# yoozzeek/zk-lisp

Measured on AMD Instinct MI355X. Metric: segment-proofs/sec at 65536 rows, blowup=16; proof bytes bit-exact vs CPU ref, higher is better.
Workload: dtype f128 (u128 mod 2^128-45*2^40+1)

## Files before the change

### zk-lisp_amd/csrc/kernels.h

```cpp
#pragma once
#include <hip/hip_runtime.h>
#include <stdint.h>

#include <stdexcept>
#include <string>
#include "air_host.h"
#include "field.h"

namespace zkl {

struct DeviceError : std::runtime_error { using std::runtime_error::runtime_error; };
#define ZKL_HIPCHECK(x)                                                                       \
  do {                                                                                        \
    hipError_t e_ = (x);                                                                      \
    if (e_ != hipSuccess) throw ::zkl::DeviceError(std::string(#x) + ": " + hipGetErrorString(e_)); \
  } while (0)
inline void check_launch(const char* what) {
  const hipError_t e = hipGetLastError();
  if (e != hipSuccess) throw DeviceError(std::string("kernel launch failed (") + what + "): " + hipGetErrorString(e));
}

struct HasherConsts {
  fe mds[144];
  fe rc[27 * 12];
  fe dom[2];
  fe dom_elems, dom_merge, dom_many, dom_int;
};

struct HasherMont {
  uint32_t mds[12][12][5];
  uint32_t rc[27][12][5];
  uint32_t dom[2][5];
  uint32_t r2[5];
  uint32_t dfe[4][5];
  uint32_t dom130[2][5];
  uint32_t r2_130[5];
  uint32_t dfe130[4][5];
  uint32_t mdsl[12][12][5][5];
  uint32_t rc130[27][12][5];
  uint32_t pmk0[5];
  uint32_t pmkt[2][5];
};
HasherMont make_hasher_mont(const HasherConsts& h);
void upload_hasher_mont(const HasherMont& m, hipStream_t s);
void upload_pm_tables(const HasherConsts& h, hipStream_t s);
int hash_engine();
void set_hash_policy(int engine, size_t min_items);
void set_row_digest_rule(int rule);
int row_digest_rule();
void set_ntt_lazy(bool on);
const char* poseidon_build_config();
const char* kernels_build_config();
void launch_permute(fe* d_states, size_t n, int engine, hipStream_t s);
struct CeParams;
struct DerivedConsts;
struct ProofConsts;
void upload_air_consts(ProofConsts* dK, const AirDevice& a, hipStream_t s);
void upload_alphas_from_device(ProofConsts* dK, const fe* d_alphas, int n, hipStream_t s);
void launch_pose_k(const ProofConsts* dK, DerivedConsts* dD, int n_tc, bool pose, hipStream_t s);
void launch_deep_coeffs(const fe* d_gam, uint32_t W, uint32_t C, const fe* d_frame, DerivedConsts* dD, hipStream_t s);

void launch_hash_rows(const fe* d_mat, uint32_t n_cols, size_t n_rows, uint32_t num_partitions,
                      uint32_t hash_rate, fe* d_tmp, fe* d_out, hipStream_t s, int tag = 0, int split = 0);
constexpr uint32_t COL_GENERAL = 0xFFFFFFFFu;
constexpr uint32_t COL_P_MAX = 128;
bool column_structure_enabled();
void set_column_structure(bool on);
void launch_scan_columns(const fe* d_mat, uint32_t n_cols, size_t n_rows, uint32_t* d_bits, hipStream_t s,
                         bool clear = true);
void decode_column_scan(const uint32_t* bits, uint32_t n_cols, size_t n_rows, uint32_t* period);
struct RowPrefixPlan {
  uint32_t np = 0;
  uint32_t lead[16] = {0};
  uint32_t q[16] = {0};
  bool any() const {
    for (uint32_t p = 0; p < np; p++)
      if (lead[p]) return true;
    return false;
  }
};
RowPrefixPlan plan_row_prefix(const uint32_t* period, uint32_t n_cols, size_t n_rows, uint32_t blowup,
                              uint32_t num_partitions, uint32_t hash_rate, size_t rows_per_entry = 64);
size_t row_prefix_table_bytes(const RowPrefixPlan& plan);
bool launch_hash_rows_prefix(const fe* d_mat, uint32_t n_cols, size_t n_rows, uint32_t num_partitions,
                             uint32_t hash_rate, const RowPrefixPlan& plan, uint32_t* d_table, fe* d_tmp, fe* d_out,
                             hipStream_t s, int split = 0);
void launch_merkle(fe* d_nodes, size_t n_leaves, hipStream_t s, fe* d_coin = nullptr, fe* d_root_out = nullptr,
                   int coin_mode = 0);
void launch_draws(fe seed, uint64_t base, size_t k, fe* d_out, hipStream_t s, const fe* d_seed = nullptr);
void launch_grind(fe seed, uint64_t base, uint32_t count, uint32_t bits, unsigned long long* d_best, hipStream_t s,
                  const fe* d_seed = nullptr);
void launch_fri_remainder(const fe* d_ev, uint32_t Nr, uint32_t rlen, const fe* wk, const fe* sk, fe* d_coin,
                          fe* d_rem, hipStream_t s);
void launch_query_seed(fe* d_coin, const unsigned long long* d_best, hipStream_t s);

struct MontTab {
  const uint4* l4;
  const uint32_t* l1;
};
void build_mont_table(const fe* h_w, size_t N, void* d_buf, hipStream_t s);
inline MontTab mont_tab(const void* d_buf, size_t N) {
  return MontTab{(const uint4*)d_buf, (const uint32_t*)((const char*)d_buf + N * 16)};
}
void launch_ntt_stages(fe* d_data, size_t n_cols, size_t N, bool dif, int lo_log, int hi_log,
                       MontTab roots, size_t Ntab, hipStream_t s);
void launch_intt_scaled(const fe* d_src, fe* d_data, size_t n_cols, size_t n, MontTab iroots, size_t Ntab,
                        const fe* d_scale, hipStream_t s);
int launch_lde_from_coeffs(const fe* d_coef, size_t n_cols, size_t n, size_t N, MontTab roots, size_t Ntab, fe* d_out,
                           hipStream_t s, bool want_split = false);
__host__ __device__ inline size_t lde_pos(size_t r, size_t N, int split) {
  if (!split) return r;
  const int logS = __builtin_ctzll((unsigned long long)N) - 8;
  const size_t S = (size_t)1 << logS;
  const size_t L = r & (S - 1), t = r >> logS, l = L & 7;
  return (L - l) + (l >> 1) + ((t & 1) << 2) + (((t >> 1) + ((l & 1) << 7)) << logS);
}
__host__ __device__ inline size_t lde_row(size_t q, size_t N, int split) {
  if (!split) return q;
  const int logS = __builtin_ctzll((unsigned long long)N) - 8;
  const size_t S = (size_t)1 << logS;
  const size_t Lp = q & (S - 1), tp = q >> logS, m = Lp & 7;
  const size_t l = ((m & 3) << 1) | (tp >> 7), t = ((tp & 127) << 1) | (m >> 2);
  return (Lp - m) + l + (t << logS);
}
void launch_broadcast(const fe* d_in, size_t in_col_stride, size_t in_elem_stride, size_t in_offset,
                      size_t n_cols, size_t n, size_t N, const fe* d_scale, fe mult, bool reverse, fe* d_out, hipStream_t s);
void launch_scale_bitrev(fe* d_data, size_t n_cols, size_t n, const fe* d_scale, hipStream_t s);

struct CeParams {
  size_t n, N, ce;
  uint32_t blowup;
  fe gl;
  fe inv_n;
  fe xn_inv[64];
  fe xn_m1[64];
  fe lagr;
  uint32_t n_bcols;
  uint32_t bcol[64];
};
struct ProofConsts {
  AirDevice air;
  CeParams ce;
  fe alpha[1024];
};
struct DerivedConsts {
  fe pose_k[27];
  fe apre[1025];
  fe deep[512];
  uint32_t deep_m[512][5];
  fe deep_sz[2];
};
void launch_constraint_eval(const fe* d_lde, const fe* d_roots, size_t Ntab, const fe* d_pertab,
                            const fe* d_bm , const CeParams& p, ProofConsts* dK,
                            const DerivedConsts* dD, bool pose_block, bool ram_merkle,
                            fe* d_xinv , bool xinv_ready, fe* d_out,
                            hipStream_t s, int split = 0, fe* d_pose_part  = nullptr);
void launch_boundary_scatter(const uint32_t* d_slot, const uint32_t* d_step, const fe* d_beta, size_t n_assert,
                             size_t n, fe* d_vecs, hipStream_t s);
void launch_boundary_w(const uint32_t* d_row_start, const fe* d_beta, const fe* d_val, size_t n, fe* d_w, hipStream_t s);
void launch_check_zero_range_bitrev(const fe* d_data, size_t N, size_t lo, size_t hi, unsigned* d_flag, hipStream_t s);

struct OodArgs {
  const fe* coef;
  size_t col_stride, elem_stride, n;
  const fe* pw1;
  const fe* pw2;
  uint32_t ncols, chunks, use_off;
  uint32_t off[16];
};
void launch_ood(const OodArgs& a, fe* d_partial, hipStream_t s);
void launch_ood_frame(const fe* d_partial_trace, const fe* d_partial_comp, uint32_t W, uint32_t C, uint32_t chunks,
                      const fe* mult , fe* d_frame, hipStream_t s);
struct DeepParams {
  size_t N;
  uint32_t W, C;
  fe z, zg;
};
void launch_deep_denoms(const fe* d_roots, size_t Ntab, size_t N, fe z, fe zg, fe* d_dinv, hipStream_t s);
void launch_deep(const fe* d_lde, const fe* d_clde, const fe* d_roots, size_t Ntab, const DeepParams& p,
                 const DerivedConsts* dD, const fe* d_dinv , fe* d_out, hipStream_t s,
                 int split = 0);
void launch_fri_leaves(const fe* d_ev, size_t Nd, fe* d_leaves, hipStream_t s);
void launch_fri_fold(const fe* d_ev, size_t Nd, const fe* d_alpha, const fe* d_iroots, size_t Ntab, fe* d_out,
                     hipStream_t s);
void launch_gather(const uint64_t* d_addrs, size_t k, fe* d_out, hipStream_t s);

}
```

### zk-lisp_amd/csrc/kernels.hip

```cpp
#include <hip/hip_runtime.h>

#include <algorithm>
#include <atomic>
#include <cstdlib>
#include <cstring>
#include <map>
#include <mutex>
#include <set>
#include <stdexcept>
#include <vector>

#include "kernels.h"
#include "air_eval.h"
#include "mont26.h"

namespace zkl {


void upload_air_consts(ProofConsts* dK, const AirDevice& a, hipStream_t s) {
  ZKL_HIPCHECK(hipMemcpyAsync(&dK->air, &a, sizeof a, hipMemcpyHostToDevice, s));
}
void upload_alphas_from_device(ProofConsts* dK, const fe* d, int n, hipStream_t s) {
  if (n > 1024) throw std::invalid_argument("more than 1024 transition constraints");
  ZKL_HIPCHECK(hipMemcpyAsync(dK->alpha, d, sizeof(fe) * n, hipMemcpyDeviceToDevice, s));
}
__global__ __launch_bounds__(1024) void pose_k_kernel(const ProofConsts* K, DerivedConsts* D, int n_tc, int pose) {
  const int j = (int)threadIdx.x;
  if (pose && j < 27) {
    uint32_t acc[9] = {0, 0, 0, 0, 0, 0, 0, 0, 0};
    for (int i = 0; i < 12; i++) mul_acc(K->alpha[12 * j + i], K->air.pose_rc[j][i], acc);
    D->pose_k[j] = reduce288(acc);
  }
  __shared__ fe sc[1024];
  sc[j] = j < n_tc ? K->alpha[j] : fe_zero();
  __syncthreads();
  for (int d = 1; d < 1024; d <<= 1) {
    const fe add = j >= d ? sc[j - d] : fe_zero();
    __syncthreads();
    sc[j] = fe_add(sc[j], add);
    __syncthreads();
  }
  D->apre[j + 1] = sc[j];
  if (j == 0) D->apre[0] = fe_zero();
}
void launch_pose_k(const ProofConsts* dK, DerivedConsts* dD, int n_tc, bool pose, hipStream_t s) {
  if (n_tc < 0 || n_tc > 1024) throw std::invalid_argument("launch_pose_k: more than 1024 transition constraints");
  pose_k_kernel<<<1, 1024, 0, s>>>(dK, dD, n_tc, pose ? 1 : 0);
}

#ifndef NTT_ELEMS_CFG
#define NTT_ELEMS_CFG 1024
#endif
#ifndef NTT_THREADS_CFG
#define NTT_THREADS_CFG 256
#endif
constexpr int NTT_ELEMS = NTT_ELEMS_CFG;
constexpr int NTT_THREADS = NTT_THREADS_CFG;

__device__ __forceinline__ uint32_t bitrev(uint32_t x, int logn) { return logn ? (__brev(x) >> (32 - logn)) : 0; }

__host__ __device__ __forceinline__ fe mul_tw(fe a, MontTab t, size_t e) {
  const uint4 q = t.l4[e];
  const uint32_t wm[5] = {q.x, q.y, q.z, q.w, t.l1[e]};
  uint32_t l[5], o[5];
  to26(a, l);
  mont_mul(l, wm, o);
  typedef unsigned __int128 u128;
  const u128 v = (u128)o[0] + ((u128)o[1] << 26) + ((u128)o[2] << 52) + ((u128)o[3] << 78) + ((u128)o[4] << 104);
  const u128 P = ((u128)P_HI << 64) | P_LO;
  const u128 r = (o[4] >> 24) ? v + C_RED : (v >= P ? v - P : v);
#ifdef NTT_CHECK
  {
    uint64_t cc[10] = {wm[0], wm[1], wm[2], wm[3], wm[4], 0, 0, 0, 0, 0};
    uint32_t wl[5];
    redc(cc, wl);
    u128 wv = (u128)wl[0] + ((u128)wl[1] << 26) + ((u128)wl[2] << 52) + ((u128)wl[3] << 78) + ((u128)wl[4] << 104);
    if (wv >= P) wv -= P;
    fe want = fe_mul(a, fe{(uint64_t)wv, (uint64_t)(wv >> 64)});
    if (want.lo != (uint64_t)r || want.hi != (uint64_t)(r >> 64))
      printf("mul_tw mismatch e=%lu a=%016lx%016lx got=%016lx%016lx want=%016lx%016lx o=%x %x %x %x %x\n", (unsigned long)e,
             (unsigned long)a.hi, (unsigned long)a.lo, (unsigned long)(uint64_t)(r >> 64), (unsigned long)(uint64_t)r,
             (unsigned long)want.hi, (unsigned long)want.lo, o[0], o[1], o[2], o[3], o[4]);
  }
#endif
  return fe{(uint64_t)r, (uint64_t)(r >> 64)};
}

void build_mont_table(const fe* w, size_t N, void* d_buf, hipStream_t s) {
  const fe R = fe_pow64(fe{2, 0}, 156);
  std::vector<uint32_t> l4(4 * N, 0), l1(N, 0);
  for (size_t H = 1; H < N; H *= 2) {
    const size_t step = N / (2 * H);
    for (size_t j = 0; j < H; j++) {
      uint32_t l[5];
      limbs26(fe_mul(w[j * step], R), l);
      for (int t = 0; t < 4; t++) l4[4 * (H + j) + t] = l[t];
      l1[H + j] = l[4];
    }
  }
  ZKL_HIPCHECK(hipMemcpyAsync(d_buf, l4.data(), N * 16, hipMemcpyHostToDevice, s));
  ZKL_HIPCHECK(hipMemcpyAsync((char*)d_buf + N * 16, l1.data(), N * 4, hipMemcpyHostToDevice, s));
  ZKL_HIPCHECK(hipStreamSynchronize(s));
}

template <bool DIF>
__global__ __launch_bounds__(NTT_THREADS) void ntt_pass_kernel(fe* __restrict__ data, size_t ncols, int logN, int r,
                                                       int logS, MontTab roots, int logTab, const fe* __restrict__ src,
                                                       int src_logb, const fe* __restrict__ scale = nullptr) {
  __shared__ fe buf[NTT_ELEMS + NTT_ELEMS / 16];
  const int R = 1 << r;
  const int G = NTT_ELEMS >> r;
  const size_t S = (size_t)1 << logS;
  const int log_gpc = logN - r;
  const size_t gpc = (size_t)1 << log_gpc;
  const bool gfast = S >= (size_t)G;
  const int pitch = R >= 16 ? R + 1 : R;
  size_t col_fixed = 0, qbase = 0;
  const bool whole = gpc >= (size_t)G;
  if (whole) {
    col_fixed = blockIdx.x % (unsigned)ncols;
    qbase = (size_t)(blockIdx.x / (unsigned)ncols) * G;
  }
  auto locate = [&](int g, size_t& col, size_t& q) -> bool {
    if (whole) {
      col = col_fixed;
      q = qbase + g;
      return true;
    }
    const size_t qg = (size_t)blockIdx.x * G + g;
    col = qg >> log_gpc;
    q = qg & (gpc - 1);
    return col < ncols;
  };
  auto addr = [&](int g, int t, bool& ok) -> size_t {
    size_t col, q;
    ok = locate(g, col, q);
    const size_t L = q & (S - 1), Hb = q >> logS;
    return (col << logN) + ((Hb << logS) << r) + (size_t)t * S + L;
  };
  const size_t Nmask = ((size_t)1 << logN) - 1;
  for (int e = threadIdx.x; e < NTT_ELEMS; e += NTT_THREADS) {
    int g = gfast ? (e % G) : (e >> r);
    int t = gfast ? (e / G) : (e & (R - 1));
    bool ok;
    size_t a = addr(g, t, ok);
    fe v = fe_zero();
    if (ok) v = src ? src[((a >> logN) << (logN - src_logb)) + ((a & Nmask) >> src_logb)] : data[a];
    buf[g * pitch + t] = v;
  }
  __syncthreads();
  for (int st = 0; st < r; st++) {
    const int lh = DIF ? (r - 1 - st) : st;
    const int h = 1 << lh;
    const size_t Hs = (size_t)h << logS;
    constexpr int BPT = NTT_ELEMS / 2 / NTT_THREADS;
    fe x0[BPT], x1[BPT];
    size_t te[BPT];
    int o0[BPT];
#pragma unroll
    for (int i = 0; i < BPT; i++) {
      const int u = threadIdx.x + NTT_THREADS * i;
      const int g = u % G;
      const int w = u / G;
      const int k = w & (h - 1);
      const int t0 = ((w >> lh) << (lh + 1)) + k;
      size_t colx, q;
      locate(g, colx, q);
      const size_t L = q & (S - 1);
      te[i] = Hs + ((size_t)k << logS) + L;
      o0[i] = g * pitch + t0;
      x0[i] = buf[o0[i]];
      x1[i] = buf[o0[i] + h];
    }
#pragma unroll
    for (int i = 0; i < BPT; i++) {
      if (DIF) {
        buf[o0[i]] = fe_add(x0[i], x1[i]);
        buf[o0[i] + h] = mul_tw(fe_sub(x0[i], x1[i]), roots, te[i]);
      } else {
        const fe v = mul_tw(x1[i], roots, te[i]);
        buf[o0[i]] = fe_add(x0[i], v);
        buf[o0[i] + h] = fe_sub(x0[i], v);
      }
    }
    __syncthreads();
  }
  for (int e = threadIdx.x; e < NTT_ELEMS; e += NTT_THREADS) {
    int g = gfast ? (e % G) : (e >> r);
    int t = gfast ? (e / G) : (e & (R - 1));
    bool ok;
    size_t a = addr(g, t, ok);
    if (ok) data[a] = scale ? fe_mul(buf[g * pitch + t], scale[bitrev((uint32_t)(a & Nmask), logN)]) : buf[g * pitch + t];
  }
}

constexpr uint32_t NTT_Q[5] = {67108872u, 128319487u, 134217726u, 134217726u, 134217726u};

__device__ __forceinline__ fe ntt_canon(const uint32_t l[5]) {
  typedef unsigned __int128 u128;
  const u128 lo = (u128)l[0] + ((u128)l[1] << 26) + ((u128)l[2] << 52) + ((u128)l[3] << 78);
  const u128 v = lo + ((u128)(l[4] & 0xFFFFFFu) << 104);
  const uint32_t t = (l[4] >> 24) + (v < lo ? 1u : 0u);
  const u128 P = ((u128)P_HI << 64) | P_LO;
  u128 r = v + (u128)t * C_RED;
  if (r < v) r += C_RED;
  if (r >= P) r -= P;
  return fe{(uint64_t)r, (uint64_t)(r >> 64)};
}

template <int ELEMS, int THREADS>
__global__ __launch_bounds__(THREADS) void ntt_dit_lazy_kernel(fe* __restrict__ data, size_t ncols, int logN, int r,
                                                                  int logS, MontTab roots, const fe* __restrict__ src,
                                                                  int src_logb) {
  constexpr int PITCHED = ELEMS + ELEMS / 16;
  __shared__ uint4 bufA[PITCHED];
  __shared__ uint32_t bufB[PITCHED];
  const int R = 1 << r;
  const int G = ELEMS >> r;
  const size_t S = (size_t)1 << logS;
  const int log_gpc = logN - r;
  const size_t gpc = (size_t)1 << log_gpc;
  const bool gfast = S >= (size_t)G;
  const int pitch = R >= 16 ? R + 1 : R;
  size_t col_fixed = 0, qbase = 0;
  const bool whole = gpc >= (size_t)G;
  if (whole) {
    col_fixed = blockIdx.x % (unsigned)ncols;
    qbase = (size_t)(blockIdx.x / (unsigned)ncols) * G;
  }
  auto locate = [&](int g, size_t& col, size_t& q) -> bool {
    if (whole) {
      col = col_fixed;
      q = qbase + g;
      return true;
    }
    const size_t qg = (size_t)blockIdx.x * G + g;
    col = qg >> log_gpc;
    q = qg & (gpc - 1);
    return col < ncols;
  };
  auto addr = [&](int g, int t, bool& ok) -> size_t {
    size_t col, q;
    ok = locate(g, col, q);
    const size_t L = q & (S - 1), Hb = q >> logS;
    return (col << logN) + ((Hb << logS) << r) + (size_t)t * S + L;
  };
  const size_t Nmask = ((size_t)1 << logN) - 1;
  for (int e = threadIdx.x; e < ELEMS; e += THREADS) {
    const int g = gfast ? (e % G) : (e >> r);
    const int t = gfast ? (e / G) : (e & (R - 1));
    bool ok;
    const size_t a = addr(g, t, ok);
    fe v = fe_zero();
    if (ok) v = src ? src[((a >> logN) << (logN - src_logb)) + ((a & Nmask) >> src_logb)] : data[a];
    uint32_t l[5];
    to26(v, l);
    bufA[g * pitch + t] = make_uint4(l[0], l[1], l[2], l[3]);
    bufB[g * pitch + t] = l[4];
  }
  __syncthreads();
  auto ld = [&](int o, uint32_t x[5]) {
    const uint4 a = bufA[o];
    x[0] = a.x; x[1] = a.y; x[2] = a.z; x[3] = a.w; x[4] = bufB[o];
  };
  auto st = [&](int o, const uint32_t x[5]) {
    bufA[o] = make_uint4(x[0], x[1], x[2], x[3]);
    bufB[o] = x[4];
  };
  auto tw = [&](size_t e, uint32_t wm[5]) {
    const uint4 q4 = roots.l4[e];
    wm[0] = q4.x; wm[1] = q4.y; wm[2] = q4.z; wm[3] = q4.w; wm[4] = roots.l1[e];
  };
  auto bfly = [&](uint32_t x0[5], uint32_t x1[5], const uint32_t wm[5]) {
    uint32_t v[5];
    mont_mul(x1, wm, v);
#pragma unroll
    for (int l = 0; l < 5; l++) {
      x1[l] = x0[l] + NTT_Q[l] - v[l];
      x0[l] = x0[l] + v[l];
    }
  };
  int lh = 0;
  for (; lh + 1 < r; lh += 2) {
    const int h = 1 << lh;
    constexpr int QPT = ELEMS / 4 / THREADS;
#pragma unroll
    for (int i = 0; i < QPT; i++) {
      const int u = threadIdx.x + THREADS * i;
      const int g = u % G;
      const int w = u / G;
      const int k = w & (h - 1);
      const int t0 = ((w >> lh) << (lh + 2)) + k;
      size_t colx, q;
      locate(g, colx, q);
      const size_t L = q & (S - 1);
      const int o = g * pitch + t0;
      uint32_t a0[5], a1[5], a2[5], a3[5], w1[5], w2[5], w3[5];
      ld(o, a0); ld(o + h, a1); ld(o + 2 * h, a2); ld(o + 3 * h, a3);
      tw(((size_t)h << logS) + ((size_t)k << logS) + L, w1);
      tw(((size_t)(2 * h) << logS) + ((size_t)k << logS) + L, w2);
      tw(((size_t)(2 * h) << logS) + ((size_t)(k + h) << logS) + L, w3);
      bfly(a0, a1, w1);
      bfly(a2, a3, w1);
      bfly(a0, a2, w2);
      bfly(a1, a3, w3);
      st(o, a0); st(o + h, a1); st(o + 2 * h, a2); st(o + 3 * h, a3);
    }
    __syncthreads();
  }
  if (lh < r) {
    const int h = 1 << lh;
    constexpr int BPT = ELEMS / 2 / THREADS;
#pragma unroll
    for (int i = 0; i < BPT; i++) {
      const int u = threadIdx.x + THREADS * i;
      const int g = u % G;
      const int w = u / G;
      const int k = w & (h - 1);
      const int t0 = ((w >> lh) << (lh + 1)) + k;
      size_t colx, q;
      locate(g, colx, q);
      const int o = g * pitch + t0;
      uint32_t x0[5], x1[5], wm[5];
      ld(o, x0); ld(o + h, x1);
      tw(((size_t)h << logS) + ((size_t)k << logS) + (q & (S - 1)), wm);
      bfly(x0, x1, wm);
      st(o, x0); st(o + h, x1);
    }
    __syncthreads();
  }
  for (int e = threadIdx.x; e < ELEMS; e += THREADS) {
    const int g = gfast ? (e % G) : (e >> r);
    const int t = gfast ? (e / G) : (e & (R - 1));
    bool ok;
    const size_t a = addr(g, t, ok);
    const uint4 a4 = bufA[g * pitch + t];
    const uint32_t l[5] = {a4.x, a4.y, a4.z, a4.w, bufB[g * pitch + t]};
    if (ok) data[a] = ntt_canon(l);
  }
}

template <int ELEMS, int THREADS>
__global__ __launch_bounds__(THREADS) void ntt_ct_lazy_kernel(fe* __restrict__ data, size_t ncols, int logN, int r,
                                                                 int logS, MontTab roots, const fe* __restrict__ src,
                                                                 int src_logb, const fe* __restrict__ scale) {
  constexpr int PITCHED = ELEMS + ELEMS / 16;
  __shared__ uint4 bufA[PITCHED];
  __shared__ uint32_t bufB[PITCHED];
  const int R = 1 << r;
  const int G = ELEMS >> r;
  const size_t S = (size_t)1 << logS;
  const int log_gpc = logN - r;
  const size_t gpc = (size_t)1 << log_gpc;
  const bool gfast = S >= (size_t)G;
  const int pitch = R >= 16 ? R + 1 : R;
  size_t col_fixed = 0, qbase = 0;
  const bool whole = gpc >= (size_t)G;
  if (whole) {
    col_fixed = blockIdx.x % (unsigned)ncols;
    qbase = (size_t)(blockIdx.x / (unsigned)ncols) * G;
  }
  auto locate = [&](int g, size_t& col, size_t& q) -> bool {
    if (whole) {
      col = col_fixed;
      q = qbase + g;
      return true;
    }
    const size_t qg = (size_t)blockIdx.x * G + g;
    col = qg >> log_gpc;
    q = qg & (gpc - 1);
    return col < ncols;
  };
  auto addr = [&](int g, int t, bool& ok) -> size_t {
    size_t col, q;
    ok = locate(g, col, q);
    const size_t L = q & (S - 1), Hb = q >> logS;
    return (col << logN) + ((Hb << logS) << r) + (size_t)t * S + L;
  };
  const size_t Nmask = ((size_t)1 << logN) - 1;
  for (int e = threadIdx.x; e < ELEMS; e += THREADS) {
    const int g = gfast ? (e % G) : (e >> r);
    const int t = gfast ? (e / G) : (e & (R - 1));
    bool ok;
    const size_t a = addr(g, t, ok);
    fe v = fe_zero();
    if (ok) v = src ? src[((a >> logN) << (logN - src_logb)) + ((a & Nmask) >> src_logb)] : data[a];
    uint32_t l[5];
    to26(v, l);
    bufA[g * pitch + t] = make_uint4(l[0], l[1], l[2], l[3]);
    bufB[g * pitch + t] = l[4];
  }
  __syncthreads();
  auto ld = [&](int o, uint32_t x[5]) {
    const uint4 a = bufA[o];
    x[0] = a.x; x[1] = a.y; x[2] = a.z; x[3] = a.w; x[4] = bufB[o];
  };
  auto st = [&](int o, const uint32_t x[5]) {
    bufA[o] = make_uint4(x[0], x[1], x[2], x[3]);
    bufB[o] = x[4];
  };
  auto tw = [&](int lh, size_t q, int t0, uint32_t wm[5]) {
    const int logm = logN - 1 - lh - logS;
    const size_t b = (q >> logS) * ((size_t)R >> (lh + 1)) + (size_t)(t0 >> (lh + 1));
    const size_t e = ((size_t)1 << logm) + (logm ? (size_t)(__brevll((unsigned long long)b) >> (64 - logm)) : 0);
    const uint4 q4 = roots.l4[e];
    wm[0] = q4.x; wm[1] = q4.y; wm[2] = q4.z; wm[3] = q4.w; wm[4] = roots.l1[e];
  };
  auto bfly = [&](uint32_t x0[5], uint32_t x1[5], const uint32_t wm[5]) {
    uint32_t v[5];
    mont_mul(x1, wm, v);
#pragma unroll
    for (int l = 0; l < 5; l++) {
      x1[l] = x0[l] + NTT_Q[l] - v[l];
      x0[l] = x0[l] + v[l];
    }
  };
  int lh = r - 1;
  for (; lh >= 1; lh -= 2) {
    const int hl = 1 << (lh - 1);
    constexpr int QPT = ELEMS / 4 / THREADS;
#pragma unroll
    for (int i = 0; i < QPT; i++) {
      const int u = threadIdx.x + THREADS * i;
      const int g = u % G;
      const int w = u / G;
      const int k = w & (hl - 1);
      const int t0 = ((w >> (lh - 1)) << (lh + 1)) + k;
      size_t colx, q;
      locate(g, colx, q);
      const int o = g * pitch + t0;
      uint32_t a0[5], a1[5], a2[5], a3[5], w1[5], w2[5], w3[5];
      ld(o, a0); ld(o + hl, a1); ld(o + 2 * hl, a2); ld(o + 3 * hl, a3);
      tw(lh, q, t0, w1);
      tw(lh - 1, q, t0, w2);
      tw(lh - 1, q, t0 + 2 * hl, w3);
      bfly(a0, a2, w1);
      bfly(a1, a3, w1);
      bfly(a0, a1, w2);
      bfly(a2, a3, w3);
      st(o, a0); st(o + hl, a1); st(o + 2 * hl, a2); st(o + 3 * hl, a3);
    }
    __syncthreads();
  }
  if (lh == 0) {
    constexpr int BPT = ELEMS / 2 / THREADS;
#pragma unroll
    for (int i = 0; i < BPT; i++) {
      const int u = threadIdx.x + THREADS * i;
      const int g = u % G;
      const int t0 = (u / G) << 1;
      size_t colx, q;
      locate(g, colx, q);
      const int o = g * pitch + t0;
      uint32_t x0[5], x1[5], wm[5];
      ld(o, x0); ld(o + 1, x1);
      tw(0, q, t0, wm);
      bfly(x0, x1, wm);
      st(o, x0); st(o + 1, x1);
    }
    __syncthreads();
  }
  for (int e = threadIdx.x; e < ELEMS; e += THREADS) {
    const int g = gfast ? (e % G) : (e >> r);
    const int t = gfast ? (e / G) : (e & (R - 1));
    bool ok;
    const size_t a = addr(g, t, ok);
    const uint4 a4 = bufA[g * pitch + t];
    const uint32_t l[5] = {a4.x, a4.y, a4.z, a4.w, bufB[g * pitch + t]};
    if (ok) {
      const fe v = ntt_canon(l);
      data[a] = scale ? fe_mul(v, scale[bitrev((uint32_t)(a & Nmask), logN)]) : v;
    }
  }
}

constexpr int NTT8_G = 8;
constexpr int NTT8_THREADS = 256;
constexpr int NTT8_PITCH = 257;
__global__ __launch_bounds__(NTT8_THREADS) __global__ __launch_bounds__(NTT8_THREADS) void ntt_dit8_kernel(fe* __restrict__ data, size_t ncols, int logN, int logS,
                                                                 MontTab roots, const fe* __restrict__ src, int src_logb,
                                                                 int lfast, int split) {
  __shared__ uint4 bufA[NTT8_G * NTT8_PITCH];
  __shared__ uint32_t bufB[NTT8_G * NTT8_PITCH];
  const int tid = (int)threadIdx.x;
  const int g = tid & (NTT8_G - 1), j = tid >> 3;
  size_t col, q;
  if (lfast) {
    const unsigned gpb = (1u << (logN - 8)) / NTT8_G;
    col = blockIdx.x / gpb;
    q = (size_t)(blockIdx.x % gpb) * NTT8_G + g;
  } else {
    col = blockIdx.x % (unsigned)ncols;
    q = (size_t)(blockIdx.x / (unsigned)ncols) * NTT8_G + g;
  }
  const size_t S = (size_t)1 << logS;
  const size_t L = q & (S - 1), Hb = q >> logS;
  const size_t base = (col << logN) + ((Hb << logS) << 8) + L;
  auto tw = [&](size_t h, size_t k, uint32_t wm[5]) {
    const size_t e = ((h + k) << logS) + L;
    const uint4 q4 = roots.l4[e];
    wm[0] = q4.x; wm[1] = q4.y; wm[2] = q4.z; wm[3] = q4.w; wm[4] = roots.l1[e];
  };
  auto bfly = [&](uint32_t x0[5], uint32_t x1[5], const uint32_t wm[5]) {
    uint32_t v[5];
    mont_mul(x1, wm, v);
#pragma unroll
    for (int l = 0; l < 5; l++) {
      x1[l] = x0[l] + NTT_Q[l] - v[l];
      x0[l] = x0[l] + v[l];
    }
  };
  auto lds_st = [&](int t, const uint32_t x[5]) {
    bufA[g * NTT8_PITCH + t] = make_uint4(x[0], x[1], x[2], x[3]);
    bufB[g * NTT8_PITCH + t] = x[4];
  };
  auto lds_ld = [&](int t, uint32_t x[5]) {
    const uint4 a = bufA[g * NTT8_PITCH + t];
    x[0] = a.x; x[1] = a.y; x[2] = a.z; x[3] = a.w; x[4] = bufB[g * NTT8_PITCH + t];
  };
  uint32_t x[8][5];
  uint32_t w[7][5];
  tw(1, 0, w[0]);
  tw(2, 0, w[1]); tw(2, 1, w[2]);
#pragma unroll
  for (int k = 0; k < 4; k++) tw(4, k, w[3 + k]);
  {
    const size_t Nmask = ((size_t)1 << logN) - 1;
#pragma unroll
    for (int u = 0; u < 8; u++) {
      const size_t a = base + (size_t)(8 * j + u) * S;
      const fe v = src ? src[((a >> logN) << (logN - src_logb)) + ((a & Nmask) >> src_logb)] : data[a];
      to26(v, x[u]);
    }
  }
#pragma unroll
  for (int u = 0; u < 8; u += 2) bfly(x[u], x[u + 1], w[0]);
#pragma unroll
  for (int u = 0; u < 8; u += 4) { bfly(x[u], x[u + 2], w[1]); bfly(x[u + 1], x[u + 3], w[2]); }
#pragma unroll
  for (int k = 0; k < 4; k++) bfly(x[k], x[k + 4], w[3 + k]);
#pragma unroll
  for (int u = 0; u < 8; u++) lds_st(8 * j + u, x[u]);
  const int a = j & 7, c = j >> 3;
  tw(8, a, w[0]);
  tw(16, a, w[1]); tw(16, a + 8, w[2]);
#pragma unroll
  for (int k = 0; k < 4; k++) tw(32, a + 8 * k, w[3 + k]);
  __syncthreads();
#pragma unroll
  for (int u = 0; u < 8; u++) lds_ld(a + 8 * u + 64 * c, x[u]);
#pragma unroll
  for (int u = 0; u < 8; u += 2) bfly(x[u], x[u + 1], w[0]);
#pragma unroll
  for (int u = 0; u < 8; u += 4) { bfly(x[u], x[u + 2], w[1]); bfly(x[u + 1], x[u + 3], w[2]); }
#pragma unroll
  for (int k = 0; k < 4; k++) bfly(x[k], x[k + 4], w[3 + k]);
#pragma unroll
  for (int u = 0; u < 8; u++) lds_st(a + 8 * u + 64 * c, x[u]);
  tw(64, j, w[0]); tw(128, j, w[1]); tw(128, j + 64, w[2]);
  tw(64, j + 32, w[3]); tw(128, j + 32, w[4]); tw(128, j + 96, w[5]);
  __syncthreads();
#pragma unroll
  for (int qd = 0; qd < 2; qd++) {
    const int a2 = j + 32 * qd;
#pragma unroll
    for (int u = 0; u < 4; u++) lds_ld(a2 + 64 * u, x[4 * qd + u]);
    uint32_t* y0 = x[4 * qd];
    uint32_t* y1 = x[4 * qd + 1];
    uint32_t* y2 = x[4 * qd + 2];
    uint32_t* y3 = x[4 * qd + 3];
    bfly(y0, y1, w[3 * qd]);
    bfly(y2, y3, w[3 * qd]);
    bfly(y0, y2, w[3 * qd + 1]);
    bfly(y1, y3, w[3 * qd + 2]);
    const size_t at0 = split ? (col << logN) + (L - g) + (g >> 1) + 4 * (a2 & 1) +
                                   ((size_t)((a2 >> 1) + ((g & 1) << 7)) << logS)
                             : base + (size_t)a2 * S;
    const size_t du = split ? 32 * S : 64 * S;
#pragma unroll
    for (int u = 0; u < 4; u++) data[at0 + u * du] = ntt_canon(x[4 * qd + u]);
  }
}

static std::atomic<int> g_ntt_lazy{-1};
static bool ntt_lazy_enabled() {
  int v = g_ntt_lazy.load(std::memory_order_relaxed);
  if (v < 0) {
    const char* e = getenv("ZKL_NTT");
    v = (e && !strcmp(e, "classic")) ? 0 : 1;
    g_ntt_lazy.store(v);
  }
  return v != 0;
}
void set_ntt_lazy(bool on) { g_ntt_lazy.store(on ? 1 : 0); }
static int ntt_wide_mode() {
  static const int m = [] {
    const char* e = getenv("ZKL_NTT_WIDE");
    return e ? atoi(e) : 2;
  }();
  return m;
}

static bool ntt8_enabled() {
  static const bool on = [] {
    const char* e = getenv("ZKL_NTT8");
    return !(e && !strcmp(e, "0"));
  }();
  return on;
}

static int ntt8_lfast(int logS) {
  static const int m = [] {
    const char* e = getenv("ZKL_NTT8_MAP");
    return e ? atoi(e) : 0;
  }();
  return m == 1 || (m == 2 && logS >= 11) ? 1 : 0;
}

static bool ntt_ct_enabled() {
  static const bool on = [] {
    const char* e = getenv("ZKL_NTT_CT");
    return !(e && !strcmp(e, "0"));
  }();
  return on;
}

static int ilog2s(size_t n) { int k = 0; while (((size_t)1 << k) < n) k++; return k; }

#ifndef NTT_TOP_R
#define NTT_TOP_R 6
#endif
#ifndef NTT_SPLIT_MODE
#define NTT_SPLIT_MODE 0
#endif
static std::vector<int> ntt_split(int K) {
  std::vector<int> rs;
  if (K <= 0) return rs;
  if (NTT_SPLIT_MODE == 0) {
    for (int left = K; left > 0; left -= std::min(8, left)) rs.push_back(std::min(8, left));
    return rs;
  }
  if (K <= 10) { rs.push_back(K); return rs; }
  int rest = K - NTT_TOP_R;
  const int np = (rest + 9) / 10;
  for (int i = 0; i < np; i++) {
    int r = (rest + (np - i) - 1) / (np - i);
    if ((r & 1) && r < rest && r < 10) r++;
    rs.push_back(r);
    rest -= r;
  }
  rs.push_back(NTT_TOP_R);
  return rs;
}

static bool dit_split_ok(size_t N, int lo, int hi) {
  if (hi < lo || !ntt_lazy_enabled() || !ntt8_enabled()) return false;
  const std::vector<int> rs = ntt_split(hi - lo + 1);
  int cur = lo;
  for (size_t k = 0; k + 1 < rs.size(); k++) cur += rs[k];
  return rs.back() == 8 && ((size_t)1 << cur) >= (size_t)NTT8_G && (N >> 8) >= (size_t)NTT8_G;
}

static void ntt_passes(fe* d, size_t ncols, size_t N, bool dif, int lo, int hi, MontTab roots, size_t Ntab,
                       const fe* src, int src_logb, hipStream_t s, int split = 0, const fe* scale = nullptr) {
  int logN = ilog2s(N), logTab = ilog2s(Ntab);
  if (hi < lo) return;
  const std::vector<int> rs = ntt_split(hi - lo + 1);
  if (dif) {
    int cur = hi;
    for (size_t k = rs.size(); k-- > 0;) {
      const int r = rs[k];
      int logS = cur - r + 1;
      size_t groups = (N >> r) * ncols;
      size_t G = NTT_ELEMS >> r;
      const fe* sp = k + 1 == rs.size() ? src : nullptr;
      const fe* sc = k == 0 ? scale : nullptr;
      if (ntt_lazy_enabled() && ntt_ct_enabled()) {
        const int wm = ntt_wide_mode();
        const bool wide = wm > 0 && G < 8 && ((size_t)1 << logS) >= G;
        const size_t Gw = wide ? 2 * G : G;
        const unsigned grid = (unsigned)((groups + Gw - 1) / Gw);
        if (wide && wm == 2)
          ntt_ct_lazy_kernel<2 * NTT_ELEMS, 2 * NTT_THREADS><<<grid, 2 * NTT_THREADS, 0, s>>>(d, ncols, logN, r, logS, roots, sp, 0, sc);
        else if (wide)
          ntt_ct_lazy_kernel<2 * NTT_ELEMS, NTT_THREADS><<<grid, NTT_THREADS, 0, s>>>(d, ncols, logN, r, logS, roots, sp, 0, sc);
        else
          ntt_ct_lazy_kernel<NTT_ELEMS, NTT_THREADS><<<grid, NTT_THREADS, 0, s>>>(d, ncols, logN, r, logS, roots, sp, 0, sc);
      } else {
        ntt_pass_kernel<true><<<(unsigned)((groups + G - 1) / G), NTT_THREADS, 0, s>>>(d, ncols, logN, r, logS, roots,
                                                                                      logTab, sp, 0, sc);
      }
      cur -= r;
    }
  } else {
    int cur = lo;
    for (size_t ri = 0; ri < rs.size(); ri++) {
      const int r = rs[ri];
      const int split_here = split && ri + 1 == rs.size();
      size_t groups = (N >> r) * ncols;
      size_t G = NTT_ELEMS >> r;
      if (ntt_lazy_enabled()) {
        const int wm = ntt_wide_mode();
        const bool wide = wm > 0 && G < 8 && ((size_t)1 << cur) >= G;
        const size_t Gw = wide ? 2 * G : G;
        const unsigned grid = (unsigned)((groups + Gw - 1) / Gw);
        const fe* sp = cur == lo ? src : nullptr;
        if (r == 8 && ntt8_enabled() && ((size_t)1 << cur) >= (size_t)NTT8_G && (N >> 8) >= (size_t)NTT8_G)
          ntt_dit8_kernel<<<(unsigned)(groups / NTT8_G), NTT8_THREADS, 0, s>>>(d, ncols, logN, cur, roots, sp, src_logb,
                                                                              ntt8_lfast(cur), split_here);
        else if (wide && wm == 2)
          ntt_dit_lazy_kernel<2 * NTT_ELEMS, 2 * NTT_THREADS><<<grid, 2 * NTT_THREADS, 0, s>>>(d, ncols, logN, r, cur, roots, sp, src_logb);
        else if (wide)
          ntt_dit_lazy_kernel<2 * NTT_ELEMS, NTT_THREADS><<<grid, NTT_THREADS, 0, s>>>(d, ncols, logN, r, cur, roots, sp, src_logb);
        else
          ntt_dit_lazy_kernel<NTT_ELEMS, NTT_THREADS><<<grid, NTT_THREADS, 0, s>>>(d, ncols, logN, r, cur, roots, sp, src_logb);
      } else
        ntt_pass_kernel<false><<<(unsigned)((groups + G - 1) / G), NTT_THREADS, 0, s>>>(
            d, ncols, logN, r, cur, roots, logTab, cur == lo ? src : nullptr, src_logb);
      cur += r;
    }
  }
}

void launch_ntt_stages(fe* d, size_t ncols, size_t N, bool dif, int lo, int hi, MontTab roots, size_t Ntab,
                       hipStream_t s) {
  ntt_passes(d, ncols, N, dif, lo, hi, roots, Ntab, nullptr, 0, s);
}

void launch_intt_scaled(const fe* src, fe* d, size_t ncols, size_t n, MontTab iroots, size_t Ntab, const fe* scale,
                        hipStream_t s) {
  const int logn = ilog2s(n);
  if (logn == 0) throw std::invalid_argument("launch_intt_scaled: n must be at least 2");
  ntt_passes(d, ncols, n, true, 0, logn - 1, iroots, Ntab, src, 0, s, 0, scale);
}

int launch_lde_from_coeffs(const fe* d_coef, size_t ncols, size_t n, size_t N, MontTab roots, size_t Ntab, fe* d_out,
                           hipStream_t s, bool want_split) {
  const int logB = ilog2s(N / n);
  if (logB == 0) {
    ZKL_HIPCHECK(hipMemcpyAsync(d_out, d_coef, ncols * n * sizeof(fe), hipMemcpyDeviceToDevice, s));
    ntt_passes(d_out, ncols, N, false, 0, ilog2s(N) - 1, roots, Ntab, nullptr, 0, s);
    return 0;
  }
  const int split = want_split && dit_split_ok(N, logB, ilog2s(N) - 1) ? 1 : 0;
  ntt_passes(d_out, ncols, N, false, logB, ilog2s(N) - 1, roots, Ntab, d_coef, logB, s, split);
  return split;
}

__global__ void broadcast_kernel(const fe* __restrict__ in, size_t in_col_stride, size_t in_elem_stride,
                                 size_t in_offset, size_t ncols, size_t n, int logn, int logB, const fe* __restrict__ scale,
                                 fe mult, bool reverse, fe* __restrict__ out) {
  size_t N = n << logB;
  size_t i = (size_t)blockIdx.x * blockDim.x + threadIdx.x;
  if (i >= N * ncols) return;
  size_t col = i / N, pos = i % N;
  size_t j = pos >> logB;
  size_t src = reverse ? (n - 1 - j) : j;
  fe v = in[col * in_col_stride + in_offset + src * in_elem_stride];
  if (scale) v = fe_mul(v, scale[bitrev((uint32_t)j, logn)]);
  if (!(mult.lo == 1 && mult.hi == 0)) v = fe_mul(v, mult);
  out[i] = v;
}

void launch_broadcast(const fe* d_in, size_t in_col_stride, size_t in_elem_stride, size_t in_offset, size_t ncols,
                      size_t n, size_t N, const fe* d_scale, fe mult, bool reverse, fe* d_out, hipStream_t s) {
  size_t tot = N * ncols;
  broadcast_kernel<<<(unsigned)((tot + 255) / 256), 256, 0, s>>>(d_in, in_col_stride, in_elem_stride, in_offset, ncols,
                                                                 n, ilog2s(n), ilog2s(N / n), d_scale, mult, reverse, d_out);
}

__global__ void scale_bitrev_kernel(fe* d, size_t ncols, size_t n, int logn, const fe* scale) {
  size_t i = (size_t)blockIdx.x * blockDim.x + threadIdx.x;
  if (i >= n * ncols) return;
  d[i] = fe_mul(d[i], scale[bitrev((uint32_t)(i % n), logn)]);
}
void launch_scale_bitrev(fe* d, size_t ncols, size_t n, const fe* scale, hipStream_t s) {
  scale_bitrev_kernel<<<(unsigned)((n * ncols + 255) / 256), 256, 0, s>>>(d, ncols, n, ilog2s(n), scale);
}

constexpr int SCAN_THREADS = 256;
constexpr size_t SCAN_CHUNK = 4096;
constexpr uint32_t SCAN_GENERAL = 1u << 31, SCAN_NONZERO = 1u << 8;
static_assert(SCAN_THREADS % COL_P_MAX == 0 && SCAN_CHUNK % SCAN_THREADS == 0 && COL_P_MAX <= 128, "scan shape");

__global__ __launch_bounds__(SCAN_THREADS) void scan_columns_kernel(const fe* __restrict__ M, size_t n, uint32_t R,
                                                                   uint32_t* __restrict__ bits) {
  const fe* col = M + (size_t)blockIdx.y * n;
  const size_t chunk = n < SCAN_CHUNK ? n : SCAN_CHUNK, i0 = (size_t)blockIdx.x * chunk;
  const uint32_t t = threadIdx.x;
  const fe ref = col[t & (R - 1)];
  uint32_t w = 0;
  for (size_t i = t; i < chunk; i += SCAN_THREADS) {
    const fe v = col[i0 + i];
    if (v.lo != ref.lo || v.hi != ref.hi) w = SCAN_GENERAL;
  }
  if (blockIdx.x == 0 && t < R) {
    if (ref.lo | ref.hi) w |= SCAN_NONZERO;
    for (uint32_t k = 0; (1u << k) < R; k++)
      if (t >= (1u << k)) {
        const fe v = col[t - (1u << k)];
        if (v.lo != ref.lo || v.hi != ref.hi) w |= 1u << k;
      }
  }
  if (__any(w != 0)) {
    for (int o = 32; o > 0; o >>= 1) w |= (uint32_t)__shfl_xor((int)w, o);
    if ((t & 63) == 0) atomicOr(&bits[blockIdx.y], w);
  }
}

void launch_scan_columns(const fe* d_mat, uint32_t ncols, size_t n, uint32_t* d_bits, hipStream_t s, bool clear) {
  if (n == 0 || (n & (n - 1)) || ncols == 0 || ncols > 65535)
    throw std::invalid_argument("launch_scan_columns: rows must be a power of two, 1..65535 columns");
  if (clear) ZKL_HIPCHECK(hipMemsetAsync(d_bits, 0, (size_t)ncols * sizeof(uint32_t), s));
  const uint32_t R = (uint32_t)std::min<size_t>(COL_P_MAX, n);
  const size_t chunk = std::min(n, SCAN_CHUNK);
  scan_columns_kernel<<<dim3((unsigned)(n / chunk), ncols), SCAN_THREADS, 0, s>>>(d_mat, n, R, d_bits);
}

void decode_column_scan(const uint32_t* bits, uint32_t ncols, size_t n, uint32_t* period) {
  const uint32_t R = (uint32_t)std::min<size_t>(COL_P_MAX, n);
  for (uint32_t c = 0; c < ncols; c++) {
    const uint32_t w = bits[c];
    uint32_t P = COL_GENERAL;
    if (!(w & SCAN_GENERAL)) {
      if (!(w & SCAN_NONZERO)) P = 0;
      else {
        P = R;
        for (uint32_t k = 0; (1u << k) < R; k++)
          if (!(w & (1u << k))) { P = 1u << k; break; }
      }
    }
    period[c] = P;
  }
}



#ifndef CE_WAVES_CFG
#define CE_WAVES_CFG 3
#endif
#if CE_WAVES_CFG
#define CE_OCC __attribute__((amdgpu_waves_per_eu(CE_WAVES_CFG, CE_WAVES_CFG)))
#else
#define CE_OCC
#endif
template <bool POSE, bool RM, int PART = 0>
__device__ __forceinline__ void constraint_eval_body(const fe* __restrict__ lde, const fe* __restrict__ roots,
                                                     int roots_shift, const fe* __restrict__ pertab,
                                                     const fe* __restrict__ bm, const ProofConsts* __restrict__ K,
                                                     const DerivedConsts* __restrict__ D, const fe* __restrict__ xinv,
                                                     fe* __restrict__ out, int split,
                                                     const fe* __restrict__ pose_part = nullptr) {
  const AirDevice& c_air = K->air;
  const CeParams& c_ce = K->ce;
  const size_t ce = c_ce.ce, N = c_ce.N;
  const size_t k = (size_t)blockIdx.x * blockDim.x + threadIdx.x;
  if (k >= ce) return;
  const bool by_pos = split && N <= 2 * ce;
  const size_t i = by_pos ? lde_row(k, N, 1) / (N / ce) : k;
  const size_t r0 = by_pos ? k : lde_pos(i * (N / ce), N, split);
  const size_t r1 = lde_pos((i * (N / ce) + c_ce.blowup) & (N - 1), N, split);
  auto cur = [&](int c) { return lde[(size_t)c * N + r0]; };
  auto nxt = [&](int c) { return lde[(size_t)c * N + r1]; };
  fe x = fe_mul(fe{3, 0}, roots[i << roots_shift]);
  const size_t per_period = ce / (c_ce.n / 32);
  const fe* per = pertab + (i % per_period) * 31;
  if (PART == 1) {
    out[i] = air_transition_sum<POSE, RM, 1>(c_air, cur, nxt, per, fe_zero(), K->alpha, D->pose_k, D->apre);
    return;
  }
  const size_t blow = ce / c_ce.n;
  const fe xn_inv = c_ce.xn_inv[i % blow];
  fe x_gl = fe_sub_sel(x, c_ce.gl);
  fe xn_m1 = c_ce.xn_m1[i % blow];
  fe p_last = fe_mul(fe_mul(c_ce.lagr, xn_m1), xinv[i]);
  fe tsum = air_transition_sum<POSE, RM, PART>(c_air, cur, nxt, per, p_last, K->alpha, D->pose_k, D->apre);
  if (PART == 2) tsum = fe_add(tsum, pose_part[i]);
  uint32_t bacc[9] = {0, 0, 0, 0, 0, 0, 0, 0, 0};
  const uint32_t nb = c_ce.n_bcols;
  for (uint32_t u = 0; u < nb; u++) mul_acc(cur((int)c_ce.bcol[u]), bm[(size_t)u * ce + i], bacc);
  fe bsum2 = fe_sub_sel(reduce288(bacc), bm[(size_t)nb * ce + i]);
  fe v = fe_add_sel(fe_mul(tsum, x_gl), bsum2);
  out[i] = fe_mul(v, xn_inv);
}

#ifndef CE_POSE_WAVES_CFG
#define CE_POSE_WAVES_CFG 3
#endif
#if CE_POSE_WAVES_CFG
#define CE_POSE_OCC __attribute__((amdgpu_waves_per_eu(CE_POSE_WAVES_CFG, CE_POSE_WAVES_CFG)))
#else
#define CE_POSE_OCC
#endif
template <bool RM>
__global__ __launch_bounds__(256) CE_OCC void constraint_eval_kernel(const fe* __restrict__ lde, const fe* __restrict__ roots,
                                                                    int roots_shift, const fe* __restrict__ pertab,
                                                                    const fe* __restrict__ bm,
                                                                    const ProofConsts* __restrict__ K,
                                                                    const DerivedConsts* __restrict__ D,
                                                                    const fe* __restrict__ xinv, fe* __restrict__ out,
                                                                    int split) {
  constraint_eval_body<false, RM>(lde, roots, roots_shift, pertab, bm, K, D, xinv, out, split);
}
__global__ __launch_bounds__(256) CE_POSE_OCC void constraint_eval_pose_part_kernel(
    const fe* __restrict__ lde, const fe* __restrict__ roots, int roots_shift, const fe* __restrict__ pertab,
    const fe* __restrict__ bm, const ProofConsts* __restrict__ K, const DerivedConsts* __restrict__ D,
    const fe* __restrict__ xinv, fe* __restrict__ pose_part, int split) {
  constraint_eval_body<true, false, 1>(lde, roots, roots_shift, pertab, bm, K, D, xinv, pose_part, split);
}
template <bool RM>
__global__ __launch_bounds__(256) CE_OCC void constraint_eval_pose_kernel(const fe* __restrict__ lde, const fe* __restrict__ roots,
                                                                  int roots_shift, const fe* __restrict__ pertab,
                                                                  const fe* __restrict__ bm,
                                                                  const ProofConsts* __restrict__ K,
                                                                  const DerivedConsts* __restrict__ D,
                                                                  const fe* __restrict__ xinv, fe* __restrict__ out,
                                                                  int split, const fe* __restrict__ pose_part) {
  constraint_eval_body<true, RM, 2>(lde, roots, roots_shift, pertab, bm, K, D, xinv, out, split, pose_part);
}

constexpr int INV_PTS = 16;
__device__ inline fe coset_den(const fe* __restrict__ roots, size_t i, int shift, fe a1, fe a2, int two) {
  const fe x = fe_mul(fe{3, 0}, roots[i << shift]);
  fe d = fe_sub(x, a1);
  if (two) d = fe_mul(d, fe_sub(x, a2));
  return d;
}
__global__ __launch_bounds__(256) void coset_inv_kernel(const fe* __restrict__ roots, int shift, fe a1, fe a2, int two,
                                                        fe* __restrict__ out) {
  const size_t T = (size_t)gridDim.x * blockDim.x;
  const size_t i0 = (size_t)blockIdx.x * blockDim.x + threadIdx.x;
  fe pre = coset_den(roots, i0, shift, a1, a2, two);
  for (int k = 1; k < INV_PTS; k++) {
    out[i0 + k * T] = pre;
    pre = fe_mul(pre, coset_den(roots, i0 + k * T, shift, a1, a2, two));
  }
  fe inv = fe_inv(pre);
  for (int k = INV_PTS - 1; k > 0; k--) {
    const fe p = out[i0 + k * T];
    out[i0 + k * T] = fe_mul(inv, p);
    inv = fe_mul(inv, coset_den(roots, i0 + k * T, shift, a1, a2, two));
  }
  out[i0] = inv;
}
static void launch_coset_inv(const fe* d_roots, int shift, size_t M, fe a1, fe a2, int two, fe* d_out, hipStream_t s) {
  const size_t threads = std::min<size_t>(256, M / INV_PTS);
  coset_inv_kernel<<<(unsigned)(M / (threads * INV_PTS)), (unsigned)threads, 0, s>>>(d_roots, shift, a1, a2, two, d_out);
}

void launch_constraint_eval(const fe* d_lde, const fe* d_roots, size_t Ntab, const fe* d_pertab, const fe* d_bm,
                            const CeParams& p, ProofConsts* dK, const DerivedConsts* dD, bool pose_block,
                            bool ram_merkle, fe* d_xinv,
                            bool xinv_ready, fe* d_out, hipStream_t s, int split, fe* d_pose_part) {
  ZKL_HIPCHECK(hipMemcpyAsync(&dK->ce, &p, sizeof p, hipMemcpyHostToDevice, s));
  int shift = ilog2s(Ntab) - ilog2s(p.ce);
  if (!xinv_ready) launch_coset_inv(d_roots, shift, p.ce, p.gl, fe_zero(), 0, d_xinv, s);
  const unsigned grid = (unsigned)((p.ce + 255) / 256);
  if (pose_block) {
    if (!d_pose_part) throw std::invalid_argument("constraint evaluation: Poseidon layout needs the pose_part buffer");
    constraint_eval_pose_part_kernel<<<grid, 256, 0, s>>>(d_lde, d_roots, shift, d_pertab, d_bm, dK, dD, d_xinv,
                                                           d_pose_part, split);
  }
  if (pose_block && ram_merkle)
    constraint_eval_pose_kernel<true><<<grid, 256, 0, s>>>(d_lde, d_roots, shift, d_pertab, d_bm, dK, dD, d_xinv, d_out,
                                                           split, d_pose_part);
  else if (pose_block)
    constraint_eval_pose_kernel<false><<<grid, 256, 0, s>>>(d_lde, d_roots, shift, d_pertab, d_bm, dK, dD, d_xinv, d_out,
                                                            split, d_pose_part);
  else if (ram_merkle)
    constraint_eval_kernel<true><<<grid, 256, 0, s>>>(d_lde, d_roots, shift, d_pertab, d_bm, dK, dD, d_xinv, d_out, split);
  else
    constraint_eval_kernel<false><<<grid, 256, 0, s>>>(d_lde, d_roots, shift, d_pertab, d_bm, dK, dD, d_xinv, d_out, split);
}

__global__ void boundary_scatter_kernel(const uint32_t* slot, const uint32_t* step, const fe* beta, size_t na, size_t n,
                                        fe* vecs) {
  size_t a = (size_t)blockIdx.x * blockDim.x + threadIdx.x;
  if (a >= na) return;
  vecs[(size_t)slot[a] * n + step[a]] = beta[a];
}
void launch_boundary_scatter(const uint32_t* d_slot, const uint32_t* d_step, const fe* d_beta, size_t na, size_t n,
                             fe* d_vecs, hipStream_t s) {
  boundary_scatter_kernel<<<(unsigned)((na + 255) / 256), 256, 0, s>>>(d_slot, d_step, d_beta, na, n, d_vecs);
}
__global__ void boundary_w_kernel(const uint32_t* rs, const fe* beta, const fe* val, size_t n, fe* w) {
  size_t row = (size_t)blockIdx.x * blockDim.x + threadIdx.x;
  if (row >= n) return;
  uint32_t acc[9] = {0, 0, 0, 0, 0, 0, 0, 0, 0};
  for (uint32_t a = rs[row]; a < rs[row + 1]; a++) mul_acc(beta[a], val[a], acc);
  w[row] = reduce288(acc);
}
void launch_boundary_w(const uint32_t* d_rs, const fe* d_beta, const fe* d_val, size_t n, fe* d_w, hipStream_t s) {
  boundary_w_kernel<<<(unsigned)((n + 255) / 256), 256, 0, s>>>(d_rs, d_beta, d_val, n, d_w);
}

__global__ void check_zero_kernel(const fe* d, size_t N, int logN, size_t lo, size_t hi, unsigned* flag) {
  size_t k = lo + (size_t)blockIdx.x * blockDim.x + threadIdx.x;
  if (k >= hi) return;
  fe v = d[bitrev((uint32_t)k, logN)];
  if (!fe_is_zero(v)) atomicOr(flag, 1u);
}
void launch_check_zero_range_bitrev(const fe* d, size_t N, size_t lo, size_t hi, unsigned* flag, hipStream_t s) {
  if (hi > lo) check_zero_kernel<<<(unsigned)((hi - lo + 255) / 256), 256, 0, s>>>(d, N, ilog2s(N), lo, hi, flag);
}

__global__ __launch_bounds__(256) void ood_kernel(OodArgs A, fe* partial) {
  const uint32_t c = blockIdx.x, k = blockIdx.z;
  const fe* col = A.coef + (A.use_off ? (size_t)A.off[c] : (size_t)c * A.col_stride);
  const size_t len = A.n / A.chunks, j0 = (size_t)k * len;
  uint32_t acc1[9] = {0, 0, 0, 0, 0, 0, 0, 0, 0}, acc2[9] = {0, 0, 0, 0, 0, 0, 0, 0, 0};
  for (size_t j = j0 + threadIdx.x; j < j0 + len; j += 256) {
    const fe v = col[j * A.elem_stride];
    mul_acc(v, A.pw1[j], acc1);
    mul_acc(v, A.pw2[j], acc2);
  }
  __shared__ fe red[2][256];
  red[0][threadIdx.x] = reduce288(acc1);
  red[1][threadIdx.x] = reduce288(acc2);
  __syncthreads();
  for (int w = 128; w > 0; w >>= 1) {
    if ((int)threadIdx.x < w) {
      red[0][threadIdx.x] = fe_add(red[0][threadIdx.x], red[0][threadIdx.x + w]);
      red[1][threadIdx.x] = fe_add(red[1][threadIdx.x], red[1][threadIdx.x + w]);
    }
    __syncthreads();
  }
  if (threadIdx.x < 2) partial[((size_t)threadIdx.x * A.ncols + c) * A.chunks + k] = red[threadIdx.x][0];
}
void launch_ood(const OodArgs& A, fe* d_partial, hipStream_t s) {
  ood_kernel<<<dim3(A.ncols, 1, A.chunks), 256, 0, s>>>(A, d_partial);
}

#ifndef DEEP_PTS_CFG
#define DEEP_PTS_CFG 2
#endif
#ifndef DEEP_COLS_CFG
#define DEEP_COLS_CFG 4
#endif
constexpr int DEEP_PTS = DEEP_PTS_CFG, DEEP_COLS = DEEP_COLS_CFG;

__device__ __forceinline__ fe limbs_canon(const uint32_t l[5]) {
  typedef unsigned __int128 u128;
  const u128 v = (u128)l[0] | ((u128)l[1] << 26) | ((u128)l[2] << 52) | ((u128)l[3] << 78) | ((u128)(l[4] & 0xFFFFFFu) << 104);
  const u128 P = ((u128)P_HI << 64) | P_LO;
  u128 r = v + (u128)(l[4] >> 24) * C_RED;
  if (r < v) r += C_RED;
  if (r >= P) r -= P;
  return fe{(uint64_t)r, (uint64_t)(r >> 64)};
}

__global__ __launch_bounds__(256) void deep_kernel(const fe* __restrict__ lde, const fe* __restrict__ clde,
                                                   const fe* __restrict__ roots, int shift, DeepParams p,
                                                   const DerivedConsts* __restrict__ K, const fe* __restrict__ dinv,
                                                   fe* out, int split) {
  const size_t T = (size_t)gridDim.x * blockDim.x;
  const size_t i0 = (size_t)blockIdx.x * blockDim.x + threadIdx.x;
  uint64_t col[DEEP_PTS][10];
#pragma unroll
  for (int k = 0; k < DEEP_PTS; k++)
#pragma unroll
    for (int u = 0; u < 10; u++) col[k][u] = 0;
  const uint32_t ncol = p.W + p.C;
  for (uint32_t c0 = 0; c0 < ncol; c0 += DEEP_COLS) {
    fe v[DEEP_COLS][DEEP_PTS];
#pragma unroll
    for (int cc = 0; cc < DEEP_COLS; cc++) {
      const uint32_t c = c0 + cc;
      const bool tr = c < p.W;
      const fe* src = tr ? lde + (size_t)c * p.N : clde + (size_t)(c - p.W) * p.N;
#pragma unroll
      for (int k = 0; k < DEEP_PTS; k++)
        v[cc][k] = c < ncol ? src[tr ? i0 + k * T : lde_row(i0 + k * T, p.N, split)] : fe_zero();
    }
#pragma unroll
    for (int cc = 0; cc < DEEP_COLS; cc++) {
      const uint32_t c = min(c0 + cc, ncol - 1);
      const uint32_t* g = K->deep_m[c];
      const uint32_t gm[5] = {g[0], g[1], g[2], g[3], g[4]};
#pragma unroll
      for (int k = 0; k < DEEP_PTS; k++) {
        uint32_t l[5];
        to26(v[cc][k], l);
        mac5(l, gm, col[k]);
      }
    }
  }
#pragma unroll
  for (int k = 0; k < DEEP_PTS; k++) {
    uint32_t l[5];
    redc(col[k], l);
    const fe sv = limbs_canon(l);
    const size_t i = lde_row(i0 + k * T, p.N, split);
    const fe x = fe_mul(fe{3, 0}, roots[i << shift]);
    const fe d1 = fe_sub(x, p.z), d2 = fe_sub(x, p.zg);
    const fe num = fe_add(fe_mul(fe_sub(sv, K->deep_sz[0]), d2), fe_mul(fe_sub(sv, K->deep_sz[1]), d1));
    out[i] = fe_mul(num, dinv[i]);
  }
}
__global__ __launch_bounds__(256) void deep_coeffs_kernel(const fe* __restrict__ gam, uint32_t W, uint32_t C,
                                                          const fe* __restrict__ frame, fe R156, DerivedConsts* K) {
  __shared__ fe red[2][256];
  const uint32_t i = threadIdx.x, n = W + C;
  fe a = fe_zero(), b = fe_zero();
  if (i < n) {
    const fe g = gam[i];
    K->deep[i] = g;
    uint32_t l[5];
    to26(fe_mul(g, R156), l);
#pragma unroll
    for (int t = 0; t < 5; t++) K->deep_m[i][t] = l[t];
    a = fe_mul(g, frame[i]);
    b = fe_mul(g, frame[n + i]);
  }
  red[0][i] = a;
  red[1][i] = b;
  __syncthreads();
  for (uint32_t h = 128; h > 0; h >>= 1) {
    if (i < h) {
      red[0][i] = fe_add(red[0][i], red[0][i + h]);
      red[1][i] = fe_add(red[1][i], red[1][i + h]);
    }
    __syncthreads();
  }
  if (i == 0) {
    K->deep_sz[0] = red[0][0];
    K->deep_sz[1] = red[1][0];
  }
}
void launch_deep_coeffs(const fe* d_gam, uint32_t W, uint32_t C, const fe* d_frame, DerivedConsts* dK, hipStream_t s) {
  if (W + C > 256) throw std::invalid_argument("more than 256 DEEP coefficients (W + C)");
  deep_coeffs_kernel<<<1, 256, 0, s>>>(d_gam, W, C, d_frame, fe_pow64(fe{2, 0}, 156), dK);
}

struct OodMult {
  fe m[16];
};
__global__ void ood_frame_kernel(const fe* __restrict__ pt, const fe* __restrict__ pc, uint32_t W, uint32_t C,
                                 uint32_t chunks, OodMult mult, fe* __restrict__ frame) {
  const uint32_t o = blockIdx.x * blockDim.x + threadIdx.x;
  const uint32_t n = W + C;
  if (o >= 2 * n) return;
  const uint32_t pt_ = o / n, r = o % n;
  const bool tr = r < W;
  const fe* src = tr ? pt + ((size_t)pt_ * W + r) * chunks : pc + ((size_t)pt_ * C + (r - W)) * chunks;
  fe acc = fe_zero();
  for (uint32_t k = 0; k < chunks; k++) acc = fe_add(acc, src[k]);
  frame[o] = tr ? acc : fe_mul(acc, mult.m[r - W]);
}
void launch_ood_frame(const fe* d_pt, const fe* d_pc, uint32_t W, uint32_t C, uint32_t chunks, const fe* mult,
                      fe* d_frame, hipStream_t s) {
  if (C > 16) throw std::invalid_argument("more than 16 composition columns");
  OodMult m{};
  for (uint32_t j = 0; j < C; j++) m.m[j] = mult[j];
  const uint32_t outs = 2 * (W + C);
  ood_frame_kernel<<<(outs + 127) / 128, 128, 0, s>>>(d_pt, d_pc, W, C, chunks, m, d_frame);
}

void launch_deep_denoms(const fe* d_roots, size_t Ntab, size_t N, fe z, fe zg, fe* d_dinv, hipStream_t s) {
  launch_coset_inv(d_roots, ilog2s(Ntab) - ilog2s(N), N, z, zg, 1, d_dinv, s);
}

void launch_deep(const fe* d_lde, const fe* d_clde, const fe* d_roots, size_t Ntab, const DeepParams& p,
                 const DerivedConsts* dK, const fe* d_dinv, fe* d_out, hipStream_t s, int split) {
  const size_t threads = std::min<size_t>(256, p.N / DEEP_PTS);
  deep_kernel<<<(unsigned)(p.N / (threads * DEEP_PTS)), (unsigned)threads, 0, s>>>(
      d_lde, d_clde, d_roots, ilog2s(Ntab) - ilog2s(p.N), p, dK, d_dinv, d_out, split);
}

__global__ void fri_fold_kernel(const fe* ev, size_t half, const fe* alpha_p, const fe* iroots, int shift, fe inv3,
                                fe inv2, fe* out) {
  size_t i = (size_t)blockIdx.x * blockDim.x + threadIdx.x;
  if (i >= half) return;
  const fe alpha = *alpha_p;
  fe v0 = ev[i], v1 = ev[i + half];
  fe ix = fe_mul(inv3, iroots[i << shift]);
  out[i] = fe_mul(fe_add(fe_add(v0, v1), fe_mul(alpha, fe_mul(fe_sub(v0, v1), ix))), inv2);
}
void launch_fri_fold(const fe* d_ev, size_t Nd, const fe* d_alpha, const fe* d_iroots, size_t Ntab, fe* d_out,
                     hipStream_t s) {
  size_t h = Nd / 2;
  fe inv3 = fe_inv(fe{3, 0}), inv2 = fe_inv(fe{2, 0});
  fri_fold_kernel<<<(unsigned)((h + 255) / 256), 256, 0, s>>>(d_ev, h, d_alpha, d_iroots, ilog2s(Ntab) - ilog2s(Nd),
                                                               inv3, inv2, d_out);
}

__global__ void gather_kernel(const uint64_t* addrs, size_t k, fe* out) {
  size_t i = (size_t)blockIdx.x * blockDim.x + threadIdx.x;
  if (i >= k) return;
  out[i] = *reinterpret_cast<const fe*>(addrs[i]);
}
void launch_gather(const uint64_t* d_addrs, size_t k, fe* d_out, hipStream_t s) {
  if (k) gather_kernel<<<(unsigned)((k + 255) / 256), 256, 0, s>>>(d_addrs, k, d_out);
}

}

#define ZKL_STR2(x) #x
#define ZKL_STR(x) ZKL_STR2(x)
namespace zkl {
const char* kernels_build_config() {
  return "NTT_ELEMS=" ZKL_STR(NTT_ELEMS_CFG) ";NTT_THREADS=" ZKL_STR(NTT_THREADS_CFG) ";CE_WAVES=" ZKL_STR(
      CE_WAVES_CFG) ";CE_POSE_WAVES=" ZKL_STR(CE_POSE_WAVES_CFG) ";DEEP_PTS=" ZKL_STR(DEEP_PTS_CFG) ";DEEP_COLS=" ZKL_STR(
      DEEP_COLS_CFG) ";CE_GROUPS=" ZKL_STR(CE_GROUPS_CFG) ";CE_DOT=" ZKL_STR(CE_DOT_CFG) ";CE_BRANCHFREE=" ZKL_STR(
      CE_BRANCHFREE_CFG);
}
}
```

### zk-lisp_amd/csrc/prover.cpp

```cpp
#include <hip/hip_runtime.h>
#include <malloc.h>
#include <stdio.h>
#include <string.h>

#include <atomic>
#include <algorithm>
#include <chrono>
#include <functional>
#include <map>
#include <memory>
#include <mutex>
#include <set>
#include <thread>
#include <stdexcept>
#include <string>
#include <vector>

#include "../../include/zkl_hip.h"
#include "air_host.h"
#include "host_hash.h"
#include "kernels.h"
#include "host_proof.h"
#include "proof_view.h"

using namespace zkl;

namespace zkl {
std::vector<uint8_t> step_encode(const zkl_air_public_inputs& pi, const zkl_step_info& s, const uint8_t* inner,
                                 size_t inner_len);
void step_digest(const uint8_t* p, size_t n, uint8_t digest[32], uint8_t rt[32]);
void children_root(const uint8_t suite[32], const uint8_t* digests, const uint8_t* roots, size_t n, uint8_t out[32]);
}

namespace {

#define HIPCHECK(x) ZKL_HIPCHECK(x)

struct InvalidArg : std::runtime_error { using std::runtime_error::runtime_error; };

uint32_t bitrev_u(uint32_t x, int logn) { uint32_t r = 0; for (int i = 0; i < logn; i++) r |= ((x >> i) & 1u) << (logn - 1 - i); return r; }

struct DBuf {
  void* p = nullptr;
  size_t bytes = 0;
  void ensure(size_t b) {
    if (b <= bytes) return;
    if (p) (void)hipFree(p);
    p = nullptr;
    bytes = 0;
    HIPCHECK(hipMalloc(&p, b));
    bytes = b;
  }
  fe* f() const { return (fe*)p; }
  ~DBuf() { if (p) (void)hipFree(p); }
};

std::atomic<uint64_t> g_pin_cur{0}, g_pin_peak{0};
void pin_alloc(void** p, size_t b) {
  HIPCHECK(hipHostMalloc(p, b, hipHostMallocDefault));
  const uint64_t c = g_pin_cur.fetch_add(b) + b;
  uint64_t pk = g_pin_peak.load();
  while (c > pk && !g_pin_peak.compare_exchange_weak(pk, c)) {
  }
}
hipError_t pin_free(void* p, size_t b) {
  if (!p) return hipSuccess;
  g_pin_cur.fetch_sub(b);
  return hipHostFree(p);
}

struct HBuf {
  void* p = nullptr;
  size_t bytes = 0;
  void ensure(size_t b) {
    if (b <= bytes) return;
    (void)release();
    b += b / 4;
    pin_alloc(&p, b);
    bytes = b;
  }
  hipError_t release() {
    const hipError_t e = pin_free(p, bytes);
    p = nullptr;
    bytes = 0;
    return e;
  }
  template <class T>
  T* at(size_t off = 0) const { return (T*)((char*)p + off); }
  ~HBuf() { (void)release(); }
};

}

constexpr size_t TX_CS = 48, TX_CS_MAX = 32, TX_QD = 80, TX_QD_MAX = 256, TX_FRI_SEED = 336, TX_WORDS = 344;

struct zkl_ctx {
  int device = 0;
  hipStream_t stream = nullptr;
  std::mutex mu;
  std::string err;
  double stage_ms[ZKL_NUM_STAGES] = {0};
  double host_ms[3] = {0, 0, 0};
  size_t tab_n = 0, tab_N = 0;
  DBuf roots, iroots, mroots, miroots, opow, opow_n, pertab;
  DBuf trace, coef, lde, parts, tree, ce, bvec, bm, clde, ctree, deep, draws, pw, oodv, oodf, txs, asl, ast, asv, ars;
  DBuf lcoef;
  DBuf fri_ev, fri_tree, best, gaddr, gout, flag;
  DBuf xinv;
  DBuf posep;
  DBuf cexinv;
  size_t cexinv_key_n = 0, cexinv_key_ce = 0, cexinv_key_tab = 0;
  const void* cexinv_key_roots = nullptr;
  DBuf scanbits, pfxtab;
  HBuf h_scan;
  std::vector<uint8_t> zero_known;
  struct { const void* coef = nullptr; const void* lde = nullptr; size_t n = 0, N = 0, W = 0; } zero_key;
  DBuf kconst;
  DBuf dconst;
  DBuf fri_coin;
  HBuf h_asrt, h_ood, h_addr, h_gv, h_tx, h_air;
  hipStream_t aux = nullptr;
  hipEvent_t aux_ev = nullptr, hev = nullptr;
  hipStream_t up = nullptr;
  std::vector<void*> up_slot;
  std::vector<hipEvent_t> up_ev;
  size_t up_slot_bytes = 0;
  double up_ms = 0;
  hipEvent_t stage_ev[ZKL_NUM_STAGES + 1] = {};
  bool stage_ev_ready = false;
  size_t pert_key_n = 0, pert_key_ce = 0;
  std::vector<hipEvent_t> evpool;
  std::vector<std::pair<int, size_t>> kmarks;
  size_t evnext = 0;
  int ktiming = 1;
  double kfam_ms[ZKL_NUM_KFAMILIES] = {0};
  int kfam_n[ZKL_NUM_KFAMILIES] = {0};
  std::vector<uint8_t> proof_s;
  Plan tplan_s;
  std::vector<Plan> fplan_s;
  std::vector<std::vector<size_t>> fpos_s;
  AirInstance air;
  HBuf tbuf[ZKL_TRACE_BUFFERS];
};

static const char* kFamilyNames =
    "ntt\ntrace_hash_rows\nmerkle\nconstraint_eval\ncomp_hash_rows\ndeep\nfri\ngrind\nmisc";
enum { KF_NTT = 0, KF_TRACE_HASH, KF_MERKLE, KF_CEVAL, KF_COMP_HASH, KF_DEEP, KF_FRI, KF_GRIND, KF_MISC };

namespace {

struct KScope {
  zkl_ctx* C;
  size_t i;
  KScope(zkl_ctx* c, int fam) : C(c), i(SIZE_MAX) {
    if (!(C->ktiming == 2 || (C->ktiming == 1 && fam == KF_TRACE_HASH))) return;
    if (C->evnext + 2 > C->evpool.size()) {
      size_t old = C->evpool.size();
      C->evpool.resize(old + 256);
      for (size_t k = old; k < C->evpool.size(); k++) HIPCHECK(hipEventCreate(&C->evpool[k]));
    }
    i = C->evnext;
    C->evnext += 2;
    C->kmarks.push_back({fam, i});
    HIPCHECK(hipEventRecord(C->evpool[i], C->stream));
  }
  ~KScope() {
    if (i != SIZE_MAX) (void)hipEventRecord(C->evpool[i + 1], C->stream);
  }
};

void resolve_kernel_times(zkl_ctx* C) {
  for (int f = 0; f < ZKL_NUM_KFAMILIES; f++) { C->kfam_ms[f] = 0; C->kfam_n[f] = 0; }
  for (auto& m : C->kmarks) {
    float ms = 0;
    HIPCHECK(hipEventElapsedTime(&ms, C->evpool[m.second], C->evpool[m.second + 1]));
    C->kfam_ms[m.first] += ms;
    C->kfam_n[m.first]++;
  }
  C->kmarks.clear();
  C->evnext = 0;
}

const char* g_global_err = "";
thread_local std::string g_tls_err;

void set_err(zkl_ctx* c, const std::string& m) {
  if (c) c->err = m;
  g_tls_err = m;
  g_global_err = g_tls_err.c_str();
}

void upload_hasher(hipStream_t s) {
  static HasherConsts hc;
  static HasherMont hm;
  static std::once_flag once;
  std::call_once(once, [] {
    const Hasher& H = hasher();
    for (int i = 0; i < 144; i++) hc.mds[i] = H.suite.mds[i / 12][i % 12];
    for (int r = 0; r < 27; r++) for (int l = 0; l < 12; l++) hc.rc[r * 12 + l] = H.suite.rc[r][l];
    hc.dom[0] = H.suite.dom[0]; hc.dom[1] = H.suite.dom[1];
    hc.dom_elems = H.dom_elems; hc.dom_merge = H.dom_merge; hc.dom_many = H.dom_many; hc.dom_int = H.dom_int;
    hm = make_hasher_mont(hc);
  });
  static std::mutex mu;
  static std::set<int> done;
  int dev = 0;
  HIPCHECK(hipGetDevice(&dev));
  std::lock_guard<std::mutex> lk(mu);
  if (done.count(dev)) return;
  upload_hasher_mont(hm, s);
  upload_pm_tables(hc, s);
  HIPCHECK(hipStreamSynchronize(s));
  done.insert(dev);
}

void ensure_tables(zkl_ctx* C, size_t n, size_t N) {
  hipStream_t s = C->stream;
  if (C->tab_N < N) {
    std::vector<fe> w(N), wi(N);
    fe g = root_of_unity(ilog2(N)), gi = fe_inv(g);
    w[0] = wi[0] = fe_one();
    for (size_t i = 1; i < N; i++) { w[i] = fe_mul(w[i - 1], g); wi[i] = fe_mul(wi[i - 1], gi); }
    C->roots.ensure(N * sizeof(fe));
    C->iroots.ensure(N * sizeof(fe));
    HIPCHECK(hipMemcpyAsync(C->roots.p, w.data(), N * sizeof(fe), hipMemcpyHostToDevice, s));
    HIPCHECK(hipMemcpyAsync(C->iroots.p, wi.data(), N * sizeof(fe), hipMemcpyHostToDevice, s));
    C->mroots.ensure(N * 20);
    C->miroots.ensure(N * 20);
    build_mont_table(w.data(), N, C->mroots.p, s);
    build_mont_table(wi.data(), N, C->miroots.p, s);
    HIPCHECK(hipStreamSynchronize(s));
    C->tab_N = N;
  }
  if (C->tab_n != n) {
    std::vector<fe> o(n), on(n);
    fe inv_n = fe_inv(fe{n, 0}), p = fe_one();
    for (size_t k = 0; k < n; k++) { o[k] = p; on[k] = fe_mul(p, inv_n); p = fe_mul(p, fe{3, 0}); }
    C->opow.ensure(n * sizeof(fe));
    C->opow_n.ensure(n * sizeof(fe));
    HIPCHECK(hipMemcpyAsync(C->opow.p, o.data(), n * sizeof(fe), hipMemcpyHostToDevice, s));
    HIPCHECK(hipMemcpyAsync(C->opow_n.p, on.data(), n * sizeof(fe), hipMemcpyHostToDevice, s));
    HIPCHECK(hipStreamSynchronize(s));
    C->tab_n = n;
  }
}

struct StageTimer {
  zkl_ctx* C;
  hipEvent_t* ev;
  bool inner;
  explicit StageTimer(zkl_ctx* c) : C(c), ev(c->stage_ev), inner(c->ktiming == 2) {
    if (!C->stage_ev_ready) {
      for (int i = 0; i <= ZKL_NUM_STAGES; i++) HIPCHECK(hipEventCreate(&C->stage_ev[i]));
      C->stage_ev_ready = true;
    }
  }
  void mark(int i) {
    if (inner || i == 0 || i == ZKL_NUM_STAGES) HIPCHECK(hipEventRecord(ev[i], C->stream));
  }
  void finish() {
    HIPCHECK(hipEventSynchronize(ev[ZKL_NUM_STAGES]));
    for (int i = 0; i < ZKL_NUM_STAGES; i++) {
      float ms = 0;
      if (inner) HIPCHECK(hipEventElapsedTime(&ms, ev[i], ev[i + 1]));
      C->stage_ms[i] = ms;
    }
  }
};

static const bool g_host_trace = getenv("ZKL_HOST_TRACE") != nullptr;
static const bool g_lde_split = [] {
  const char* e = getenv("ZKL_LDE_SPLIT");
  return !(e && !strcmp(e, "0"));
}();
#define HT(label)                                                                                   \
  do {                                                                                              \
    if (g_host_trace)                                                                               \
      fprintf(stderr, "[ht] %-24s %9.1f\n", label,                                                  \
              std::chrono::duration<double, std::micro>(std::chrono::steady_clock::now() - t_call0).count()); \
  } while (0)

template <class T>
void d2h(zkl_ctx* C, T* dst, const void* src, size_t bytes) {
  HIPCHECK(hipMemcpyAsync(dst, src, bytes, hipMemcpyDeviceToHost, C->stream));
  HIPCHECK(hipStreamSynchronize(C->stream));
}

__global__ void powers_kernel(fe base, fe mult, size_t n, int logn, fe* out) {
  size_t j = (size_t)blockIdx.x * blockDim.x + threadIdx.x;
  if (j >= n) return;
  uint32_t k = logn ? (__brev((uint32_t)j) >> (32 - logn)) : 0;
  out[j] = fe_mul(mult, fe_pow64(base, k));
}

void validate_request(uint32_t W, uint32_t n32, const zkl_air_public_inputs& pi, const zkl_proof_options& o) {
  const size_t n = n32;
  if (n < 32 || (n & (n - 1))) throw InvalidArg("trace length must be a power of two >= 32");
  if (o.field_extension != 1) throw InvalidArg("only FieldExtension::None is supported for segment proofs");
  if (o.fri_folding_factor != 2) throw InvalidArg("only FRI folding factor 2 is supported");
  if (o.batching_constraints != 0 || o.batching_deep != 0) throw InvalidArg("only BatchingMethod::Linear is supported");
  if (o.blowup_factor < 2 || (o.blowup_factor & (o.blowup_factor - 1))) throw InvalidArg("blowup must be a power of two");
  if (o.blowup_factor > 128) throw InvalidArg("blowup must be at most 128");
  if (o.grinding_factor > 32) throw InvalidArg("grinding_factor must be at most 32");
  if (o.num_queries == 0 || o.num_queries > 255) throw InvalidArg("num_queries must be in 1..255");
  if (o.num_partitions < 1 || o.num_partitions > 16) throw InvalidArg("num_partitions must be in 1..16");
  if (o.hash_rate < 1 || o.hash_rate > 255) throw InvalidArg("hash_rate must be in 1..255 (a u8 in the proof context)");
  if (o.fri_remainder_max_degree > 15 || ((o.fri_remainder_max_degree + 1) & o.fri_remainder_max_degree))
    throw InvalidArg("fri_remainder_max_degree must be one less than a power of two, at most 15");
  {
    const std::string e = check_proof_options(o);
    if (!e.empty()) throw InvalidArg(e);
  }
  if (pi.n_main_slots > ZKL_MAX_MAIN_SLOTS) throw InvalidArg("n_main_slots exceeds ZKL_MAX_MAIN_SLOTS");
  if (W == 0 || W > 4096) throw InvalidArg("trace width must be in 1..4096");
}

constexpr int UP_SLOTS = 4;
constexpr size_t UP_SLOT_BYTES = (size_t)16 << 20;

static unsigned up_threads() {
  static const unsigned t = [] {
    const char* e = getenv("ZKL_UP_THREADS");
    const unsigned d = std::max(1u, std::min(8u, std::thread::hardware_concurrency() / 2));
    return e ? std::max(1, atoi(e)) : (int)d;
  }();
  return t;
}
static bool up_direct() {
  static const bool d = [] {
    const char* e = getenv("ZKL_UP_MODE");
    return e && !strcmp(e, "direct");
  }();
  return d;
}

void parallel_copy(void* dst, const void* src, size_t bytes, unsigned nt) {
  if (nt <= 1 || bytes < ((size_t)1 << 20)) { memcpy(dst, src, bytes); return; }
  const size_t per = ((bytes + nt - 1) / nt + 63) & ~(size_t)63;
  std::vector<std::thread> th;
  for (unsigned t = 1; t < nt && t * per < bytes; t++)
    th.emplace_back([=] { memcpy((char*)dst + t * per, (const char*)src + t * per, std::min(per, bytes - t * per)); });
  memcpy(dst, src, std::min(per, bytes));
  for (auto& x : th) x.join();
}

template <class F>
void upload_trace_chunked(zkl_ctx* C, const void* h_trace, uint32_t W, size_t n, hipStream_t s, F&& on_chunk) {
  if (!C->up) {
    HIPCHECK(hipStreamCreateWithFlags(&C->up, hipStreamNonBlocking));
    C->up_slot.assign(UP_SLOTS, nullptr);
    C->up_ev.assign(UP_SLOTS, nullptr);
    for (int k = 0; k < UP_SLOTS; k++) {
      pin_alloc(&C->up_slot[k], UP_SLOT_BYTES);
      HIPCHECK(hipEventCreateWithFlags(&C->up_ev[k], hipEventDisableTiming));
    }
    C->up_slot_bytes = UP_SLOT_BYTES;
  }
  const auto t0 = std::chrono::steady_clock::now();
  const size_t col_bytes = n * sizeof(fe);
  const uint32_t per = (uint32_t)std::max<size_t>(1, C->up_slot_bytes / col_bytes);
  const unsigned nt = up_threads();
  bool in_tbuf = false;
  for (const HBuf& b : C->tbuf)
    in_tbuf |= b.p && (const char*)h_trace >= (const char*)b.p &&
               (const char*)h_trace + (size_t)W * col_bytes <= (const char*)b.p + b.bytes;
  const bool direct = in_tbuf || up_direct();
  bool used[UP_SLOTS] = {false, false, false, false};
  double copy_ms = 0, wait_ms = 0;
  auto ms_since = [](std::chrono::steady_clock::time_point a) {
    return std::chrono::duration<double, std::milli>(std::chrono::steady_clock::now() - a).count();
  };
  int k = 0;
  for (uint32_t c0 = 0; c0 < W; c0 += per, k = (k + 1) % UP_SLOTS) {
    const uint32_t nc = std::min(per, W - c0);
    if (direct || col_bytes * nc > C->up_slot_bytes) {
      HIPCHECK(hipMemcpyAsync(C->coef.f() + (size_t)c0 * n, (const char*)h_trace + c0 * col_bytes, col_bytes * nc,
                              hipMemcpyHostToDevice, direct ? C->up : s));
      if (direct) {
        HIPCHECK(hipEventRecord(C->up_ev[k], C->up));
        HIPCHECK(hipStreamWaitEvent(s, C->up_ev[k], 0));
      }
      on_chunk(c0, nc);
      continue;
    }
    auto tw = std::chrono::steady_clock::now();
    if (used[k]) HIPCHECK(hipEventSynchronize(C->up_ev[k]));
    wait_ms += ms_since(tw);
    auto tc = std::chrono::steady_clock::now();
    parallel_copy(C->up_slot[k], (const char*)h_trace + c0 * col_bytes, col_bytes * nc, nt);
    copy_ms += ms_since(tc);
    HIPCHECK(hipMemcpyAsync(C->coef.f() + (size_t)c0 * n, C->up_slot[k], col_bytes * nc, hipMemcpyHostToDevice, C->up));
    HIPCHECK(hipEventRecord(C->up_ev[k], C->up));
    used[k] = true;
    HIPCHECK(hipStreamWaitEvent(s, C->up_ev[k], 0));
    on_chunk(c0, nc);
  }
  C->up_ms = ms_since(t0);
  if (getenv("ZKL_UP_DEBUG"))
    fprintf(stderr, "[zkl upload] %u cols x %zu rows: loop %.2f ms (host copy %.2f ms on %u threads, slot waits %.2f ms)%s\n",
            W, n, C->up_ms, copy_ms, nt, wait_ms, in_tbuf ? " pinned trace buffer" : direct ? " direct" : "");
}

std::atomic<int> g_proofs_in_flight{0};
struct InFlight {
  InFlight() { g_proofs_in_flight.fetch_add(1); }
  ~InFlight() { g_proofs_in_flight.fetch_sub(1); }
};

void prove_impl(zkl_ctx* C, const void* d_trace_in, bool trace_on_host, uint32_t W, uint32_t n32,
                const zkl_air_public_inputs& pi, const zkl_proof_options& o) {
  const InFlight in_flight;
  const auto t_call0 = std::chrono::steady_clock::now();
  hipStream_t s = C->stream;
  const size_t n = n32;
  validate_request(W, n32, pi, o);
  const size_t N = n * o.blowup_factor;
  const int logn = ilog2(n), logN = ilog2(N);
  const uint32_t B = o.blowup_factor;
  const fe g = root_of_unity(logn), three{3, 0};
  const Hasher& H = hasher();

  upload_hasher(s);
  ensure_tables(C, n, N);
  const fe* roots = C->roots.f();
  const fe* iroots = C->iroots.f();
  const MontTab mroots = mont_tab(C->mroots.p, C->tab_N), miroots = mont_tab(C->miroots.p, C->tab_N);
  const size_t Ntab = C->tab_N;

  StageTimer T(C);
  T.mark(0);
  C->host_ms[0] = std::chrono::duration<double, std::milli>(std::chrono::steady_clock::now() - t_call0).count();
  C->coef.ensure((size_t)W * n * sizeof(fe));
  C->lde.ensure((size_t)W * N * sizeof(fe));
  int split = -1;
  auto lde_cols = [&](uint32_t c0, uint32_t nc, const fe* src) {
    fe* cf = C->coef.f() + (size_t)c0 * n;
    launch_intt_scaled(src ? src + (size_t)c0 * n : nullptr, cf, nc, n, miroots, Ntab, C->opow_n.f(), s);
    const int sp = launch_lde_from_coeffs(cf, nc, n, N, mroots, Ntab, C->lde.f() + (size_t)c0 * N, s, g_lde_split);
    if (split >= 0 && sp != split) throw std::runtime_error("internal: trace LDE chunks in different layouts");
    split = sp;
  };
  const bool colstruct = column_structure_enabled();
  const bool zkey_ok = C->zero_key.coef == C->coef.p && C->zero_key.lde == C->lde.p && C->zero_key.n == n &&
                       C->zero_key.N == N && C->zero_key.W == W && C->zero_known.size() == W;
  if (!zkey_ok) C->zero_known.assign(W, 0);
  C->zero_key.coef = nullptr;
  std::vector<uint32_t> period;
  uint32_t* hbits = nullptr;
  if (colstruct) {
    C->scanbits.ensure((size_t)W * sizeof(uint32_t));
    C->h_scan.ensure((size_t)W * sizeof(uint32_t));
    hbits = C->h_scan.at<uint32_t>();
  }
  auto read_scan = [&] {
    HIPCHECK(hipMemcpyAsync(hbits, C->scanbits.p, (size_t)W * sizeof(uint32_t), hipMemcpyDeviceToHost, s));
    HIPCHECK(hipStreamSynchronize(s));
    period.resize(W);
    decode_column_scan(hbits, W, n, period.data());
  };
  if (trace_on_host) {
    KScope k(C, KF_NTT);
    std::fill(C->zero_known.begin(), C->zero_known.end(), 0);
    if (colstruct) HIPCHECK(hipMemsetAsync(C->scanbits.p, 0, (size_t)W * sizeof(uint32_t), s));
    upload_trace_chunked(C, d_trace_in, W, n, s, [&](uint32_t c0, uint32_t nc) {
      if (colstruct) launch_scan_columns(C->coef.f() + (size_t)c0 * n, nc, n, (uint32_t*)C->scanbits.p + c0, s, false);
      lde_cols(c0, nc, nullptr);
    });
  } else if (!colstruct) {
    C->up_ms = 0;
    KScope k(C, KF_NTT);
    std::fill(C->zero_known.begin(), C->zero_known.end(), 0);
    lde_cols(0, W, (const fe*)d_trace_in);
  } else {
    C->up_ms = 0;
    {
      KScope k(C, KF_MISC);
      launch_scan_columns((const fe*)d_trace_in, W, n, (uint32_t*)C->scanbits.p, s);
      check_launch("column scan");
      read_scan();
    }
    KScope k(C, KF_NTT);
    for (uint32_t c0 = 0; c0 < W;) {
      uint32_t c1 = c0;
      const bool zero = period[c0] == 0;
      while (c1 < W && (period[c1] == 0) == zero) c1++;
      if (!zero) {
        lde_cols(c0, c1 - c0, (const fe*)d_trace_in);
        std::fill(C->zero_known.begin() + c0, C->zero_known.begin() + c1, 0);
      } else {
        for (uint32_t a = c0; a < c1;) {
          if (C->zero_known[a]) { a++; continue; }
          uint32_t b = a;
          while (b < c1 && !C->zero_known[b]) b++;
          HIPCHECK(hipMemsetAsync(C->coef.f() + (size_t)a * n, 0, (size_t)(b - a) * n * sizeof(fe), s));
          HIPCHECK(hipMemsetAsync(C->lde.f() + (size_t)a * N, 0, (size_t)(b - a) * N * sizeof(fe), s));
          std::fill(C->zero_known.begin() + a, C->zero_known.begin() + b, 1);
          a = b;
        }
      }
      c0 = c1;
    }
  }
  check_launch("trace LDE");
  if (split < 0) split = 0;
  C->zero_key.coef = C->coef.p; C->zero_key.lde = C->lde.p; C->zero_key.n = n; C->zero_key.N = N; C->zero_key.W = W;
  T.mark(1);
  C->parts.ensure((size_t)o.num_partitions * N * sizeof(fe) + N * sizeof(fe));
  C->tree.ensure(2 * N * sizeof(fe));
  if (colstruct && trace_on_host) read_scan();
  {
    RowPrefixPlan plan;
    if (colstruct) plan = plan_row_prefix(period.data(), W, N, B, o.num_partitions, o.hash_rate);
    if (plan.any()) C->pfxtab.ensure(row_prefix_table_bytes(plan));
    KScope k(C, KF_TRACE_HASH);
    launch_hash_rows_prefix(C->lde.f(), W, N, o.num_partitions, o.hash_rate, plan, (uint32_t*)C->pfxtab.p, C->parts.f(),
                            C->tree.f() + N, s, split);
  }
  check_launch("trace row hash");
  std::vector<fe> seed_el = context_elements(W, n, o);
  auto pie = pi_elements(pi);
  seed_el.insert(seed_el.end(), pie.begin(), pie.end());
  Coin coin{H.hash_elements(seed_el.data(), seed_el.size()), 0};
  C->txs.ensure(64 * sizeof(fe));
  C->h_tx.ensure(TX_WORDS * sizeof(fe));
  fe* tx = C->txs.f();
  fe* htx = C->h_tx.at<fe>();
  htx[32] = coin.seed;
  HIPCHECK(hipMemcpyAsync(tx, htx + 32, sizeof(fe), hipMemcpyHostToDevice, s));
  {
    KScope k(C, KF_MERKLE);
    launch_merkle(C->tree.f(), N, s, tx, tx + 2, 1);
  }
  check_launch("trace Merkle tree and trace-root reseed");
  coin.counter = 0;
  AirInstance& air = C->air;
  {
    std::string e = build_air(pi, W, n, air);
    if (e.empty() && o.blowup_factor < (uint32_t)air.ce_blowup) e = "blowup factor below constraint-evaluation blowup";
    if (!e.empty()) {
      (void)hipStreamSynchronize(s);
      throw InvalidArg(e);
    }
  }
  const size_t ce = n * air.ce_blowup;
  const int logce = ilog2(ce);
  const int Cc = air.num_comp_cols;
  C->kconst.ensure(sizeof(ProofConsts));
  ProofConsts* dK = (ProofConsts*)C->kconst.p;
  C->dconst.ensure(sizeof(DerivedConsts));
  DerivedConsts* dD = (DerivedConsts*)C->dconst.p;
  C->h_air.ensure(sizeof(AirDevice));
  memcpy(C->h_air.p, &air.dev, sizeof(AirDevice));
  upload_air_consts(dK, *C->h_air.at<AirDevice>(), s);
  const size_t na = air.assertions.size();
  std::map<uint32_t, uint32_t> slot_of;
  std::vector<uint32_t> bcols;
  for (auto& a : air.assertions)
    if (!slot_of.count(a.col)) { slot_of[a.col] = (uint32_t)bcols.size(); bcols.push_back(a.col); }
  if (bcols.size() > 64) throw InvalidArg("too many asserted columns");
  const uint32_t nb = (uint32_t)bcols.size();
  const size_t off_st = na * 4, off_sv = (na * 8 + 15) & ~(size_t)15, off_rs = off_sv + na * sizeof(fe);
  C->h_asrt.ensure(off_rs + (n + 1) * 4);
  uint32_t* hslot = C->h_asrt.at<uint32_t>(0);
  uint32_t* hstep = C->h_asrt.at<uint32_t>(off_st);
  fe* hval = C->h_asrt.at<fe>(off_sv);
  uint32_t* rowstart = C->h_asrt.at<uint32_t>(off_rs);
  memset(rowstart, 0, (n + 1) * 4);
  for (size_t k = 0; k < na; k++) {
    hslot[k] = slot_of[air.assertions[k].col];
    hstep[k] = air.assertions[k].step;
    hval[k] = air.assertions[k].value;
    rowstart[hstep[k] + 1]++;
  }
  for (size_t r = 0; r < n; r++) rowstart[r + 1] += rowstart[r];
  C->asl.ensure(na * 4); C->ast.ensure(na * 4); C->asv.ensure(na * sizeof(fe)); C->ars.ensure((n + 1) * 4);
  if (!C->aux) {
    HIPCHECK(hipStreamCreateWithFlags(&C->aux, hipStreamNonBlocking));
    HIPCHECK(hipEventCreateWithFlags(&C->aux_ev, hipEventDisableTiming));
    HIPCHECK(hipEventCreateWithFlags(&C->hev, hipEventDisableTiming));
  }
  HIPCHECK(hipMemcpyAsync(C->asl.p, hslot, na * 4, hipMemcpyHostToDevice, C->aux));
  HIPCHECK(hipMemcpyAsync(C->ast.p, hstep, na * 4, hipMemcpyHostToDevice, C->aux));
  HIPCHECK(hipMemcpyAsync(C->asv.p, hval, na * sizeof(fe), hipMemcpyHostToDevice, C->aux));
  HIPCHECK(hipMemcpyAsync(C->ars.p, rowstart, (n + 1) * 4, hipMemcpyHostToDevice, C->aux));
  HIPCHECK(hipEventRecord(C->aux_ev, C->aux));
  HIPCHECK(hipStreamWaitEvent(s, C->aux_ev, 0));
  C->bvec.ensure((size_t)(nb + 1) * n * sizeof(fe));
  C->bm.ensure((size_t)(nb + 1) * ce * sizeof(fe));
  HT("air_built");
  T.mark(2);

  const size_t ndraw = (size_t)air.n_tc + na;
  C->draws.ensure((ndraw + 1024) * sizeof(fe));
  {
    KScope k(C, KF_MISC);
    launch_draws(fe_zero(), coin.counter, ndraw, C->draws.f(), s, tx);
  }
  check_launch("composition coefficient draws");
  coin.counter += ndraw;
  upload_alphas_from_device(dK, C->draws.f(), air.n_tc, s);
  launch_pose_k(dK, dD, air.n_tc, air.dev.pose_block != 0, s);

  HIPCHECK(hipMemsetAsync(C->bvec.p, 0, (size_t)(nb + 1) * n * sizeof(fe), s));
  const fe* betas = C->draws.f() + air.n_tc;
  {
    KScope k(C, KF_CEVAL);
    launch_boundary_scatter((const uint32_t*)C->asl.p, (const uint32_t*)C->ast.p, betas, na, n, C->bvec.f(), s);
    launch_boundary_w((const uint32_t*)C->ars.p, betas, C->asv.f(), n, C->bvec.f() + (size_t)nb * n, s);
  }
  {
    KScope k(C, KF_NTT);
    launch_ntt_stages(C->bvec.f(), nb + 1, n, true, 0, logn - 1, mroots, Ntab, s);
    C->lcoef.ensure((size_t)std::max<uint32_t>(nb + 1, Cc) * n * sizeof(fe));
    launch_broadcast(C->bvec.f(), n, 1, 0, nb + 1, n, n, C->opow.f(), fe_one(), true, C->lcoef.f(), s);
    launch_lde_from_coeffs(C->lcoef.f(), nb + 1, n, ce, mroots, Ntab, C->bm.f(), s, false);
  }
  check_launch("boundary tables");

  if (C->pert_key_n != n || C->pert_key_ce != ce) {
    auto tab = periodic_table(n, ce, three);
    C->pertab.ensure(tab.size() * sizeof(fe));
    HIPCHECK(hipMemcpyAsync(C->pertab.p, tab.data(), tab.size() * sizeof(fe), hipMemcpyHostToDevice, s));
    HIPCHECK(hipStreamSynchronize(s));
    C->pert_key_n = n; C->pert_key_ce = ce;
  }
  CeParams cp{};
  cp.n = n; cp.N = N; cp.ce = ce; cp.blowup = B;
  cp.gl = fe_pow64(g, n - 1);
  cp.inv_n = fe_inv(fe{n, 0});
  cp.lagr = fe_mul(cp.gl, cp.inv_n);
  {
    size_t blow = ce / n;
    fe wb = root_of_unity(ilog2(blow)), on = fe_pow64(three, n), p = fe_one();
    for (size_t j = 0; j < blow; j++) {
      cp.xn_m1[j] = fe_sub(fe_mul(on, p), fe_one());
      cp.xn_inv[j] = fe_inv(cp.xn_m1[j]);
      p = fe_mul(p, wb);
    }
  }
  cp.n_bcols = nb;
  for (uint32_t u = 0; u < nb; u++) cp.bcol[u] = bcols[u];
  C->ce.ensure(ce * sizeof(fe));
  {
    KScope k(C, KF_CEVAL);
    const bool ready = C->cexinv_key_n == n && C->cexinv_key_ce == ce && C->cexinv_key_tab == Ntab &&
                       C->cexinv_key_roots == (const void*)roots && C->cexinv.bytes >= ce * sizeof(fe);
    if (!ready) {
      C->cexinv_key_n = 0;
      C->cexinv.ensure(ce * sizeof(fe));
    }
    if (air.dev.pose_block) C->posep.ensure(ce * sizeof(fe));
    launch_constraint_eval(C->lde.f(), roots, Ntab, C->pertab.f(), C->bm.f(), cp, dK, dD, air.dev.pose_block != 0,
                           (air.dev.ram_block | air.dev.merkle_block) != 0, C->cexinv.f(), ready, C->ce.f(), s, split,
                           air.dev.pose_block ? C->posep.f() : nullptr);
    C->cexinv_key_n = n; C->cexinv_key_ce = ce; C->cexinv_key_tab = Ntab; C->cexinv_key_roots = roots;
  }
  check_launch("constraint evaluation");
  T.mark(3);

  C->flag.ensure(16);
  C->clde.ensure((size_t)Cc * N * sizeof(fe));
  const int loge = ilog2(ce / n);
  const fe inv3 = fe_inv(three), inv_ce = fe_inv(fe{ce, 0});
  {
    KScope k(C, KF_NTT);
    launch_ntt_stages(C->ce.f(), 1, ce, true, 0, logce - 1, miroots, Ntab, s);
    HIPCHECK(hipMemsetAsync(C->flag.p, 0, 4, s));
    launch_check_zero_range_bitrev(C->ce.f(), ce, (size_t)Cc * n, ce, (unsigned*)C->flag.p, s);
    for (int j = 0; j < Cc; j++) {
      fe mult = fe_mul(fe_pow64(inv3, (uint64_t)j * n), inv_ce);
      launch_broadcast(C->ce.f(), 0, ce / n, bitrev_u((uint32_t)j, loge), 1, n, n, nullptr, mult, false,
                       C->lcoef.f() + (size_t)j * n, s);
    }
    launch_lde_from_coeffs(C->lcoef.f(), Cc, n, N, mroots, Ntab, C->clde.f(), s, false);
  }
  check_launch("composition polynomial LDE");
  C->ctree.ensure(2 * N * sizeof(fe));
  {
    KScope k(C, KF_COMP_HASH);
    launch_hash_rows(C->clde.f(), Cc, N, o.num_partitions, o.hash_rate, C->parts.f(), C->ctree.f() + N, s, 1);
  }
  {
    KScope k(C, KF_MERKLE);
    launch_merkle(C->ctree.f(), N, s, tx, tx + 3, 1);
  }
  check_launch("composition commitment");
  HIPCHECK(hipMemcpyAsync(htx, tx, 4 * sizeof(fe), hipMemcpyDeviceToHost, s));
  HIPCHECK(hipMemcpyAsync(htx + 4, C->flag.p, 4, hipMemcpyDeviceToHost, s));
  HIPCHECK(hipStreamSynchronize(s));
  HT("croot");
  unsigned bad = 0;
  memcpy(&bad, htx + 4, 4);
  if (bad) throw InvalidArg("constraint composition polynomial degree too large: trace does not satisfy the AIR");
  const fe troot = htx[2], croot = htx[3];
  coin.seed = htx[0];
  coin.counter = 0;
  T.mark(4);

  fe z = coin.draw(), zg = fe_mul(z, g);
  C->pw.ensure(4 * n * sizeof(fe));
  fe* pw = C->pw.f();
  powers_kernel<<<(unsigned)((n + 255) / 256), 256, 0, s>>>(fe_mul(z, inv3), fe_one(), n, logn, pw + 2 * n);
  powers_kernel<<<(unsigned)((n + 255) / 256), 256, 0, s>>>(fe_mul(zg, inv3), fe_one(), n, logn, pw + 3 * n);
  const uint32_t chunks = n >= 8192 ? 32 : 1;
  const size_t n_otr = 2 * (size_t)W * chunks, n_ocp = 2 * (size_t)Cc * chunks;
  C->oodv.ensure((n_otr + n_ocp) * sizeof(fe));
  fe* dood = C->oodv.f();
  if (Cc > 16) throw std::runtime_error("internal: more than 16 composition columns");
  {
    KScope k(C, KF_MISC);
    OodArgs a{};
    a.coef = C->coef.f(); a.col_stride = n; a.elem_stride = 1; a.n = n;
    a.pw1 = pw + 2 * n; a.pw2 = pw + 3 * n; a.ncols = W; a.chunks = chunks; a.use_off = 0;
    launch_ood(a, dood, s);
    OodArgs b{};
    b.coef = C->ce.f(); b.col_stride = 0; b.elem_stride = ce / n; b.n = n;
    b.pw1 = pw + 2 * n; b.pw2 = pw + 3 * n; b.ncols = (uint32_t)Cc; b.chunks = chunks; b.use_off = 1;
    for (int j = 0; j < Cc; j++) b.off[j] = bitrev_u((uint32_t)j, loge);
    launch_ood(b, dood + n_otr, s);
  }
  std::vector<fe> cmult(Cc);
  for (int j = 0; j < Cc; j++) cmult[j] = fe_mul(fe_pow64(inv3, (uint64_t)j * n), inv_ce);
  C->oodf.ensure(2 * ((size_t)W + Cc) * sizeof(fe));
  fe* dframe = C->oodf.f();
  launch_ood_frame(dood, dood + n_otr, W, (uint32_t)Cc, chunks, cmult.data(), dframe, s);
  check_launch("OOD evaluation");
  const size_t nfr = 2 * ((size_t)W + Cc);
  C->h_ood.ensure(nfr * sizeof(fe));
  const fe* frame = C->h_ood.at<fe>();
  HIPCHECK(hipMemcpyAsync(C->h_ood.p, dframe, nfr * sizeof(fe), hipMemcpyDeviceToHost, s));
  HIPCHECK(hipEventRecord(C->hev, s));
  C->xinv.ensure(std::max(ce, N) * sizeof(fe));
  {
    KScope k(C, KF_DEEP);
    launch_deep_denoms(roots, Ntab, N, z, zg, C->xinv.f(), s);
  }
  check_launch("DEEP denominators");
  HT("ood_enqueued");
  HIPCHECK(hipEventSynchronize(C->hev));
  std::vector<fe> tz(frame, frame + W), hz(frame + W, frame + W + Cc);
  std::vector<fe> tzg(frame + W + Cc, frame + 2 * W + Cc), hzg(frame + 2 * W + Cc, frame + nfr);
  coin.reseed(H.hash_elements(frame, nfr));
  T.mark(5);

  HT("ood_hashed");
  launch_draws(coin.seed, coin.counter, W + Cc, C->draws.f(), s);
  check_launch("DEEP coefficient draws");
  coin.counter += W + Cc;
  launch_deep_coeffs(C->draws.f(), W, (uint32_t)Cc, dframe, dD, s);
  check_launch("DEEP coefficients");
  HT("gam");
  DeepParams dp{};
  dp.N = N; dp.W = W; dp.C = Cc; dp.z = z; dp.zg = zg;
  C->deep.ensure(N * sizeof(fe));
  {
    KScope k(C, KF_DEEP);
    launch_deep(C->lde.f(), C->clde.f(), roots, Ntab, dp, dD, C->xinv.f(), C->deep.f(), s, split);
  }
  check_launch("DEEP composition");
  T.mark(6);

  const size_t rem_max = (size_t)(o.fri_remainder_max_degree + 1) * B;
  int nl = 0;
  for (size_t d = N; d > rem_max; d /= 2) nl++;
  std::vector<size_t> ev_off(nl + 1), tr_off(nl);
  size_t ev_tot = 0, tr_tot = 0;
  for (int d = 0; d <= nl; d++) {
    ev_off[d] = ev_tot;
    if (d >= 1) ev_tot += N >> d;
    if (d < nl) { tr_off[d] = tr_tot; tr_tot += N >> d; }
  }
  C->fri_ev.ensure((ev_tot + 1) * sizeof(fe));
  C->fri_tree.ensure((tr_tot + 1) * sizeof(fe));
  auto layer_ev = [&](int d) -> fe* { return d == 0 ? C->deep.f() : C->fri_ev.f() + ev_off[d]; };
  std::vector<fe> fri_roots(nl);
  C->fri_coin.ensure((2 + (size_t)nl) * sizeof(fe));
  fe* d_coin = C->fri_coin.f();
  htx[TX_FRI_SEED] = coin.seed;
  HIPCHECK(hipMemcpyAsync(d_coin, htx + TX_FRI_SEED, sizeof(fe), hipMemcpyHostToDevice, s));
  for (int d = 0; d < nl; d++) {
    size_t Nd = N >> d, h = Nd / 2;
    fe* tr = C->fri_tree.f() + tr_off[d];
    {
      KScope k(C, KF_FRI);
      launch_fri_leaves(layer_ev(d), Nd, tr + h, s);
    }
    {
      KScope k(C, KF_MERKLE);
      launch_merkle(tr, h, s, d_coin, d_coin + 2 + d, 2);
    }
    KScope k(C, KF_FRI);
    launch_fri_fold(layer_ev(d), Nd, d_coin + 1, iroots, Ntab, layer_ev(d + 1), s);
  }
  check_launch("FRI layers");
  HT("fri_enqueued");
  const size_t Nr = N >> nl;
  const uint32_t rlen = o.fri_remainder_max_degree + 1;
  {
    const fe w = root_of_unity(ilog2(Nr)), wi = fe_inv(w), inv_nr = fe_inv(fe{Nr, 0});
    fe wk[16], sk[16];
    for (uint32_t k = 0; k < rlen; k++) {
      wk[k] = fe_pow64(wi, k);
      sk[k] = fe_mul(inv_nr, fe_pow64(inv3, k));
    }
    KScope k(C, KF_FRI);
    launch_fri_remainder(layer_ev(nl), (uint32_t)Nr, rlen, wk, sk, d_coin, tx + 4, s);
  }
  check_launch("FRI remainder");
  T.mark(7);

  HT("grind_start");
  uint64_t nonce = 0;
  C->best.ensure(8);
  unsigned long long* hbest = (unsigned long long*)(htx + 40);
  uint32_t batch = 1u << std::min<uint32_t>(std::max<uint32_t>(o.grinding_factor, 14), 22);
  if (const char* e = getenv("ZKL_TEST_GRIND_FIRST")) {
    batch = (uint32_t)std::max(1L, std::min(atol(e), 1L << 22));
    static std::once_flag said;
    std::call_once(said, [&] { fprintf(stderr, "zkl_hip: test hook ZKL_TEST_GRIND_FIRST=%s active\n", e); });
  }
  uint64_t base = 1;
  auto queue_windows = [&](const fe* d_seed, fe h_seed) {
    *hbest = o.grinding_factor == 0 ? 1ull : ~0ull;
    HIPCHECK(hipMemcpyAsync(C->best.p, hbest, 8, hipMemcpyHostToDevice, s));
    if (o.grinding_factor == 0) return;
    KScope k(C, KF_GRIND);
    for (int w = 0; w < 4; w++) {
      launch_grind(h_seed, base, batch, o.grinding_factor, (unsigned long long*)C->best.p, s, d_seed);
      base += batch;
      if (w >= 1) batch = std::min<uint32_t>(batch * 2, 1u << 22);
    }
  };
  queue_windows(d_coin, fe_zero());
  launch_query_seed(d_coin, (const unsigned long long*)C->best.p, s);
  launch_draws(fe_zero(), 0, o.num_queries, C->draws.f(), s, d_coin + 1);
  check_launch("grinding and query draws");
  if (2 + (size_t)nl > TX_CS_MAX || o.num_queries > TX_QD_MAX) throw std::runtime_error("internal: transcript staging");
  HIPCHECK(hipMemcpyAsync(htx + TX_CS, d_coin, (2 + (size_t)nl) * sizeof(fe), hipMemcpyDeviceToHost, s));
  HIPCHECK(hipMemcpyAsync(htx + 4, tx + 4, (rlen + 1) * sizeof(fe), hipMemcpyDeviceToHost, s));
  HIPCHECK(hipMemcpyAsync(hbest, C->best.p, 8, hipMemcpyDeviceToHost, s));
  HIPCHECK(hipMemcpyAsync(htx + TX_QD, C->draws.p, o.num_queries * sizeof(fe), hipMemcpyDeviceToHost, s));
  HIPCHECK(hipStreamSynchronize(s));
  std::vector<fe> cs(htx + TX_CS, htx + TX_CS + 2 + nl), qd(htx + TX_QD, htx + TX_QD + o.num_queries);
  for (int d = 0; d < nl; d++) fri_roots[d] = cs[2 + d];
  std::vector<fe> rem(htx + 4, htx + 4 + rlen);
  const fe rem_commit = htx[4 + rlen];
  coin.seed = cs[0];
  coin.counter = 0;
  HT("rem");
  if (*hbest != ~0ull) {
    nonce = *hbest;
  } else {
    while (nonce == 0) {
      queue_windows(nullptr, coin.seed);
      check_launch("grinding");
      HIPCHECK(hipMemcpyAsync(hbest, C->best.p, 8, hipMemcpyDeviceToHost, s));
      HIPCHECK(hipStreamSynchronize(s));
      if (*hbest != ~0ull) nonce = *hbest;
    }
    launch_draws(H.merge_with_int(coin.seed, nonce), 0, o.num_queries, C->draws.f(), s);
    check_launch("query draws");
    HIPCHECK(hipMemcpyAsync(htx + TX_QD, C->draws.p, o.num_queries * sizeof(fe), hipMemcpyDeviceToHost, s));
    HIPCHECK(hipStreamSynchronize(s));
    qd.assign(htx + TX_QD, htx + TX_QD + o.num_queries);
  }
  T.mark(8);

  HT("q_start");
  HT("q_drawn");
  std::vector<size_t> pos;
  for (auto& v : qd) pos.push_back((size_t)(v.lo & (N - 1)));
  std::sort(pos.begin(), pos.end());
  pos.erase(std::unique(pos.begin(), pos.end()), pos.end());
  const size_t nq = pos.size();

  HT("q_sorted");
  const size_t na_max = nq * ((size_t)W + Cc) + 2 * nq * ((size_t)logN + 2) + (size_t)nl * nq * ((size_t)logN + 4);
  C->h_addr.ensure(na_max * 8);
  uint64_t* const abase = C->h_addr.at<uint64_t>();
  uint64_t* ap = abase;
  for (size_t k = 0; k < nq; k++) {
    const fe* rp = C->lde.f() + lde_pos(pos[k], N, split);
    for (uint32_t c = 0; c < W; c++) *ap++ = (uint64_t)(uintptr_t)(rp + (size_t)c * N);
  }
  for (size_t k = 0; k < nq; k++)
    for (int j = 0; j < Cc; j++) *ap++ = (uint64_t)(uintptr_t)(C->clde.f() + (size_t)j * N + pos[k]);
  auto room = [&](size_t k) {
    if ((size_t)(ap - abase) + k > na_max) throw std::runtime_error("internal: gather plan bound");
  };
  auto append_nodes = [&](const fe* tree, const Plan& plan) {
    room(plan.node.size());
    for (uint64_t ix : plan.node) *ap++ = (uint64_t)(uintptr_t)(tree + ix);
  };
  Plan& tplan = C->tplan_s;
  batch_plan_into(N, pos.data(), nq, tplan);
  append_nodes(C->tree.f(), tplan);
  append_nodes(C->ctree.f(), tplan);
  std::vector<std::vector<size_t>>& fpos = C->fpos_s;
  std::vector<Plan>& fplan = C->fplan_s;
  if (fpos.size() < (size_t)nl) fpos.resize(nl);
  if (fplan.size() < (size_t)nl) fplan.resize(nl);
  {
    size_t dsz = N;
    for (int d = 0; d < nl; d++) {
      const size_t h = dsz / 2;
      const std::vector<size_t>& p = d ? fpos[d - 1] : pos;
      std::vector<size_t>& f = fpos[d];
      f.clear();
      uint64_t seen_key[512];
      uint8_t seen[512] = {0};
      for (size_t x : p) {
        const size_t y = x & (h - 1);
        size_t k = (size_t)(((uint64_t)y * 0x9E3779B97F4A7C15ull) >> 55);
        while (seen[k] && seen_key[k] != y) k = (k + 1) & 511;
        if (!seen[k]) {
          seen[k] = 1;
          seen_key[k] = y;
          f.push_back(y);
        }
      }
      room(2 * f.size());
      for (size_t y : f) { *ap++ = (uint64_t)(uintptr_t)(layer_ev(d) + y); *ap++ = (uint64_t)(uintptr_t)(layer_ev(d) + y + h); }
      batch_plan_into(h, f.data(), f.size(), fplan[d]);
      append_nodes(C->fri_tree.f() + tr_off[d], fplan[d]);
      dsz = h;
    }
  }
  HT("q_planned");
  const size_t na_g = (size_t)(ap - abase);
  C->gaddr.ensure((na_g + na_g / 4) * 8);
  C->gout.ensure((na_g + na_g / 4) * sizeof(fe));
  C->h_gv.ensure(na_g * sizeof(fe));
  HIPCHECK(hipMemcpyAsync(C->gaddr.p, C->h_addr.p, na_g * 8, hipMemcpyHostToDevice, s));
  launch_gather((const uint64_t*)C->gaddr.p, na_g, C->gout.f(), s);
  check_launch("query gather");
  HIPCHECK(hipMemcpyAsync(C->h_gv.p, C->gout.p, na_g * sizeof(fe), hipMemcpyDeviceToHost, s));
  T.mark(9);
  T.mark(10);
  HIPCHECK(hipStreamSynchronize(s));
  HT("q_gathered");
  const fe* gv = C->h_gv.at<fe>();
  size_t gi = 0;

  Bytes P;
  P.v.swap(C->proof_s);
  P.v.clear();
  P.v.reserve(na_g * 32 + 4096);
  P.u8((uint8_t)W); P.u8(0); P.u8(0); P.u8((uint8_t)logn); P.u8(0); P.u8(0);
  P.u8(16); P.felem(fe{P_LO, P_HI});
  P.u8((uint8_t)o.num_queries); P.u8((uint8_t)o.blowup_factor); P.u8((uint8_t)o.grinding_factor);
  P.u8((uint8_t)o.field_extension); P.u8((uint8_t)o.fri_folding_factor); P.u8((uint8_t)o.fri_remainder_max_degree);
  P.u8((uint8_t)o.batching_constraints); P.u8((uint8_t)o.batching_deep);
  P.u8((uint8_t)o.num_partitions); P.u8((uint8_t)o.hash_rate);
  P.u8((uint8_t)nq);
  {
    Bytes cm;
    cm.digest(troot); cm.digest(croot);
    for (auto& r : fri_roots) cm.digest(r);
    cm.digest(rem_commit);
    P.vec(cm);
  }
  auto mp_len = [](const Plan& plan) {
    size_t n = 2 + plan.len.size();
    for (uint32_t l : plan.len) n += 32 * (size_t)l;
    return n;
  };
  auto emit_multiproof = [&](const Plan& plan, int depth, size_t g) {
    const size_t len = mp_len(plan);
    P.usize(len);
    const size_t o = P.v.size();
    P.v.resize(o + len);
    uint8_t* w = P.v.data() + o;
    *w++ = (uint8_t)depth;
    *w++ = (uint8_t)plan.len.size();
    for (uint32_t l : plan.len) {
      *w++ = (uint8_t)l;
      for (uint32_t k = 0; k < l; k++, w += 32) {
        memcpy(w, gv + g++, 16);
        memset(w + 16, 0, 16);
      }
    }
  };
  const size_t g_rows = 0, g_crows = nq * W, g_tnodes = nq * ((size_t)W + Cc), g_cnodes = g_tnodes + tplan.node.size();
  P.usize(1);
  P.usize(nq * W * sizeof(fe));
  P.raw(gv + g_rows, nq * W * sizeof(fe));
  emit_multiproof(tplan, logN, g_tnodes);
  P.usize(nq * Cc * sizeof(fe));
  P.raw(gv + g_crows, nq * Cc * sizeof(fe));
  emit_multiproof(tplan, logN, g_cnodes);
  gi = g_cnodes + tplan.node.size();
  {
    Bytes ts, es;
    for (auto& v : tz) ts.felem(v);
    for (auto& v : tzg) ts.felem(v);
    for (auto& v : hz) es.felem(v);
    for (auto& v : hzg) es.felem(v);
    P.vec(ts); P.vec(es);
  }
  P.usize((uint64_t)nl);
  for (int d = 0; d < nl; d++) {
    const size_t nv = 2 * fpos[d].size();
    P.usize(nv * sizeof(fe));
    P.raw(gv + gi, nv * sizeof(fe));
    gi += nv;
    emit_multiproof(fplan[d], ilog2((N >> d) / 2), gi);
    gi += fplan[d].node.size();
  }
  {
    Bytes rv;
    for (auto& v : rem) rv.felem(v);
    P.vec(rv);
  }
  P.u8(0);
  P.u64(nonce);
  if (gi != na_g) throw std::runtime_error("internal: gather plan mismatch");
  HT("serialised");
  T.finish();
  HT("stage_events");
  resolve_kernel_times(C);
  C->proof_s.swap(P.v);
  HT("returned");
  C->host_ms[2] = std::chrono::duration<double, std::milli>(std::chrono::steady_clock::now() - t_call0).count();
  {
    float gpu_ms = 0;
    HIPCHECK(hipEventElapsedTime(&gpu_ms, T.ev[0], T.ev[ZKL_NUM_STAGES]));
    C->host_ms[1] = C->host_ms[2] - C->host_ms[0] - gpu_ms;
  }
}

int run_guarded(zkl_ctx* ctx, const std::function<void()>& f) {
  try {
    f();
    return ZKL_OK;
  } catch (const InvalidArg& e) {
    set_err(ctx, e.what());
    return ZKL_E_INVALID;
  } catch (const std::invalid_argument& e) {
    set_err(ctx, e.what());
    return ZKL_E_INVALID;
  } catch (const DeviceError& e) {
    set_err(ctx, e.what());
    return ZKL_E_DEVICE;
  } catch (const std::bad_alloc&) {
    set_err(ctx, "host allocation failed");
    return ZKL_E_OOM;
  } catch (const std::exception& e) {
    set_err(ctx, e.what());
    return ZKL_E_INTERNAL;
  }
}

}

int zkl::guarded_call(const std::function<void()>& f) { return run_guarded(nullptr, f); }

extern "C" {

int zkl_hip_abi_version(void) { return ZKL_ABI_VERSION; }

const char* zkl_hip_build_config(void) {
  static const std::string cfg = std::string(poseidon_build_config()) + ";" + kernels_build_config();
  return cfg.c_str();
}

int zkl_hip_init(int device, zkl_ctx** out) {
  if (!out) return ZKL_E_INVALID;
  *out = nullptr;
  return run_guarded(nullptr, [&] {
    int cnt = 0;
    HIPCHECK(hipGetDeviceCount(&cnt));
    if (device < 0 || device >= cnt) throw InvalidArg("no such HIP device");
    HIPCHECK(hipSetDevice(device));
    auto* c = new zkl_ctx();
    c->device = device;
    hipError_t e = hipStreamCreateWithFlags(&c->stream, hipStreamNonBlocking);
    if (e != hipSuccess) { delete c; throw DeviceError(hipGetErrorString(e)); }
    *out = c;
  });
}

int zkl_hip_process_tuning(uint32_t flags, uint32_t* applied) {
  if (applied) *applied = 0;
  if (flags & ~(uint32_t)(ZKL_TUNE_SPIN | ZKL_TUNE_MALLOC)) return ZKL_E_INVALID;
  static std::mutex mu;
  std::lock_guard<std::mutex> lk(mu);
  uint32_t ok = 0;
  if (flags & ZKL_TUNE_SPIN) {
    int cnt = 0, cur = 0;
    bool all = hipGetDeviceCount(&cnt) == hipSuccess && cnt > 0 && hipGetDevice(&cur) == hipSuccess;
    for (int d = 0; all && d < cnt; d++)
      all = hipSetDevice(d) == hipSuccess && hipSetDeviceFlags(hipDeviceScheduleSpin) == hipSuccess;
    if (cnt > 0) (void)hipSetDevice(cur);
    (void)hipGetLastError();
    if (all) ok |= ZKL_TUNE_SPIN;
  }
  if (flags & ZKL_TUNE_MALLOC) {
    if (mallopt(M_MMAP_THRESHOLD, 32 << 20) == 1 && mallopt(M_TOP_PAD, 64 << 20) == 1 &&
        mallopt(M_TRIM_THRESHOLD, 0x7fffffff) == 1)
      ok |= ZKL_TUNE_MALLOC;
  }
  if (applied) *applied = ok;
  return ok == flags ? ZKL_OK : ZKL_E_DEVICE;
}

int zkl_hip_trace_buffer(zkl_ctx* c, uint32_t slot, size_t bytes, zkl_f128** out) {
  if (!c || !out || !bytes || slot >= ZKL_TRACE_BUFFERS) return ZKL_E_INVALID;
  std::lock_guard<std::mutex> lk(c->mu);
  *out = nullptr;
  return run_guarded(c, [&] {
    HIPCHECK(hipSetDevice(c->device));
    HBuf& b = c->tbuf[slot];
    if (bytes > b.bytes) {
      HIPCHECK(b.release());
      pin_alloc(&b.p, bytes);
      b.bytes = bytes;
    }
    *out = (zkl_f128*)b.p;
  });
}

int zkl_hip_pinned_bytes(uint64_t* current, uint64_t* peak) {
  if (current) *current = g_pin_cur.load();
  if (peak) *peak = g_pin_peak.load();
  return ZKL_OK;
}

void zkl_hip_destroy(zkl_ctx* c) {
  if (!c) return;
  (void)hipSetDevice(c->device);
  (void)hipStreamSynchronize(c->stream);
  (void)hipStreamDestroy(c->stream);
  if (c->stage_ev_ready)
    for (auto& e : c->stage_ev) (void)hipEventDestroy(e);
  if (c->up) {
    (void)hipStreamSynchronize(c->up);
    (void)hipStreamDestroy(c->up);
    for (void* p : c->up_slot) (void)pin_free(p, c->up_slot_bytes);
    for (hipEvent_t e : c->up_ev) (void)hipEventDestroy(e);
  }
  if (c->aux) {
    (void)hipStreamSynchronize(c->aux);
    (void)hipStreamDestroy(c->aux);
    (void)hipEventDestroy(c->aux_ev);
    (void)hipEventDestroy(c->hev);
  }
  delete c;
}

const char* zkl_hip_last_error(const zkl_ctx* c) { return c ? c->err.c_str() : g_global_err; }

void zkl_hip_free(uint8_t* p) { free(p); }

static int finish_proof(std::vector<uint8_t>& v, uint8_t** out, size_t* len) {
  uint8_t* b = (uint8_t*)malloc(v.size());
  if (!b) return ZKL_E_OOM;
  memcpy(b, v.data(), v.size());
  *out = b;
  *len = v.size();
  return ZKL_OK;
}

int zkl_hip_prove_segment(zkl_ctx* c, const zkl_f128* trace, uint32_t width, uint32_t n, const zkl_air_public_inputs* pi,
                          const zkl_proof_options* o, uint8_t** proof, size_t* len) {
  if (!c || !trace || !pi || !o || !proof || !len) return ZKL_E_INVALID;
  std::lock_guard<std::mutex> lk(c->mu);
  c->proof_s.clear();
  int rc = run_guarded(c, [&] {
    HIPCHECK(hipSetDevice(c->device));
    prove_impl(c, trace, true, width, n, *pi, *o);
  });
  return rc ? rc : finish_proof(c->proof_s, proof, len);
}

int zkl_hip_prove_segment_device(zkl_ctx* c, const void* d_trace, uint32_t width, uint32_t n,
                                 const zkl_air_public_inputs* pi, const zkl_proof_options* o, uint8_t** proof,
                                 size_t* len) {
  if (!c || !d_trace || !pi || !o || !proof || !len) return ZKL_E_INVALID;
  std::lock_guard<std::mutex> lk(c->mu);
  c->proof_s.clear();
  int rc = run_guarded(c, [&] {
    HIPCHECK(hipSetDevice(c->device));
    prove_impl(c, d_trace, false, width, n, *pi, *o);
  });
  return rc ? rc : finish_proof(c->proof_s, proof, len);
}

static int copy_last_proof(zkl_ctx* c, uint8_t* buf, size_t cap, size_t* len) {
  *len = c->proof_s.size();
  if (c->proof_s.empty()) {
    c->err = "no proof on this context (the last prove call failed or none was made)";
    return ZKL_E_INVALID;
  }
  if (!buf) return ZKL_OK;
  if (cap < c->proof_s.size()) {
    c->err = "proof buffer too small: " + std::to_string(c->proof_s.size()) + " bytes needed, " +
             std::to_string(cap) + " given (zkl_hip_last_proof still returns it)";
    return ZKL_E_INVALID;
  }
  memcpy(buf, c->proof_s.data(), c->proof_s.size());
  return ZKL_OK;
}

int zkl_hip_last_proof(zkl_ctx* c, uint8_t* buf, size_t cap, size_t* len) {
  if (!c || !len) return ZKL_E_INVALID;
  std::lock_guard<std::mutex> lk(c->mu);
  return copy_last_proof(c, buf, cap, len);
}

int zkl_hip_prove_segment_device_into(zkl_ctx* c, const void* d_trace, uint32_t width, uint32_t n,
                                      const zkl_air_public_inputs* pi, const zkl_proof_options* o, uint8_t* buf,
                                      size_t cap, size_t* len) {
  if (!c || !d_trace || !pi || !o || !len) return ZKL_E_INVALID;
  std::lock_guard<std::mutex> lk(c->mu);
  c->proof_s.clear();
  int rc = run_guarded(c, [&] {
    HIPCHECK(hipSetDevice(c->device));
    prove_impl(c, d_trace, false, width, n, *pi, *o);
  });
  return rc ? rc : copy_last_proof(c, buf, cap, len);
}

int zkl_hip_check_request(uint32_t width, uint32_t n_rows, const zkl_air_public_inputs* pi,
                          const zkl_proof_options* o) {
  if (!pi || !o) return ZKL_E_INVALID;
  return run_guarded(nullptr, [&] {
    validate_request(width, n_rows, *pi, *o);
    AirInstance air;
    std::string e = build_air(*pi, width, n_rows, air);
    if (e.empty() && o->blowup_factor < (uint32_t)air.ce_blowup) e = "blowup factor below constraint-evaluation blowup";
    if (!e.empty()) throw InvalidArg(e);
  });
}

int zkl_verify_segment(const uint8_t* proof, size_t len, const zkl_air_public_inputs* pi,
                       const zkl_proof_options* opts) {
  if (!proof || !pi || !opts) return ZKL_E_INVALID;
  return run_guarded(nullptr, [&] {
    const std::string e = verify_segment(proof, len, *pi, *opts, nullptr);
    if (!e.empty()) throw InvalidArg(e);
  });
}

int zkl_hip_host_times(const zkl_ctx* c, double* out_ms, int max_n) {
  if (!c || !out_ms) return ZKL_E_INVALID;
  const double v[4] = {c->host_ms[0], c->host_ms[1], c->host_ms[2], c->up_ms};
  const int k = std::min(max_n, 4);
  for (int i = 0; i < k; i++) out_ms[i] = v[i];
  return k;
}

int zkl_hip_stage_times(const zkl_ctx* c, double* out, int max_n) {
  if (!c || !out) return 0;
  int k = std::min(max_n, ZKL_NUM_STAGES);
  for (int i = 0; i < k; i++) out[i] = c->stage_ms[i];
  return k;
}

int zkl_hip_kernel_times(const zkl_ctx* c, double* out, int* launches, int max_n, const char** names) {
  if (names) *names = kFamilyNames;
  if (!c) return 0;
  int k = std::min(max_n, ZKL_NUM_KFAMILIES);
  for (int i = 0; i < k; i++) {
    if (out) out[i] = c->kfam_ms[i];
    if (launches) launches[i] = c->kfam_n[i];
  }
  return k;
}

int zkl_hip_set_kernel_timing(zkl_ctx* c, int mode) {
  if (!c || mode < 0 || mode > 2) return ZKL_E_INVALID;
  std::lock_guard<std::mutex> lk(c->mu);
  c->ktiming = mode;
  return 0;
}

int zkl_step_proof_encode(const zkl_air_public_inputs* pi, const zkl_step_info* info, const uint8_t* inner,
                          size_t inner_len, uint8_t** out, size_t* out_len) {
  if (!pi || !info || !inner || !out || !out_len) return ZKL_E_INVALID;
  std::vector<uint8_t> v;
  int rc = run_guarded(nullptr, [&] { v = step_encode(*pi, *info, inner, inner_len); });
  if (rc) return rc;
  return finish_proof(v, out, out_len);
}

int zkl_children_root(const uint8_t suite_id[32], const uint8_t* digests, const uint8_t* root_traces, uint32_t n,
                      uint8_t root_out[32]) {
  if (!suite_id || !root_out || (n && (!digests || !root_traces))) return ZKL_E_INVALID;
  return run_guarded(nullptr, [&] { children_root(suite_id, digests, root_traces, n, root_out); });
}

int zkl_step_proof_digest(const uint8_t* step, size_t len, uint8_t digest_out[32], uint8_t root_trace_out[32]) {
  if (!step) return ZKL_E_INVALID;
  return run_guarded(nullptr, [&] { step_digest(step, len, digest_out, root_trace_out); });
}

int zkl_hip_device_count(int* count) {
  if (!count) return ZKL_E_INVALID;
  return run_guarded(nullptr, [&] { HIPCHECK(hipGetDeviceCount(count)); });
}

int zkl_hip_device_alloc(zkl_ctx* c, size_t bytes, void** d) {
  if (!c || !d) return ZKL_E_INVALID;
  return run_guarded(c, [&] {
    HIPCHECK(hipSetDevice(c->device));
    hipError_t e = hipMalloc(d, bytes);
    if (e == hipErrorOutOfMemory) throw std::bad_alloc();
    HIPCHECK(e);
  });
}

int zkl_hip_device_free(zkl_ctx* c, void* d) {
  if (!c) return ZKL_E_INVALID;
  return run_guarded(c, [&] {
    HIPCHECK(hipSetDevice(c->device));
    HIPCHECK(hipFree(d));
  });
}

int zkl_hip_memcpy(zkl_ctx* c, void* dst, const void* src, size_t bytes, int kind) {
  if (!c || kind < 1 || kind > 3) return ZKL_E_INVALID;
  std::lock_guard<std::mutex> lk(c->mu);
  return run_guarded(c, [&] {
    HIPCHECK(hipSetDevice(c->device));
    hipMemcpyKind k = kind == 1 ? hipMemcpyHostToDevice : kind == 2 ? hipMemcpyDeviceToHost : hipMemcpyDeviceToDevice;
    HIPCHECK(hipMemcpyAsync(dst, src, bytes, k, c->stream));
    HIPCHECK(hipStreamSynchronize(c->stream));
  });
}

int zkl_hip_synchronize(zkl_ctx* c) {
  if (!c) return ZKL_E_INVALID;
  return run_guarded(c, [&] {
    HIPCHECK(hipSetDevice(c->device));
    HIPCHECK(hipStreamSynchronize(c->stream));
    HIPCHECK(hipDeviceSynchronize());
  });
}

void zkl_select_partitions(uint32_t w, uint32_t len, uint32_t* parts, uint32_t* rate) {
  if (rate) *rate = w <= 32 ? 8 : 16;
  if (parts) *parts = len >= (1u << 20) ? 16 : len >= (1u << 18) ? 8 : len >= (1u << 16) ? 4 : len >= (1u << 14) ? 2 : 1;
}

int zkl_hip_hash_rows(zkl_ctx* c, const void* d_m, uint32_t nc, uint32_t nr, uint32_t np, uint32_t rate, void* d_out) {
  if (!c || !d_m || !d_out || nc == 0 || np < 1 || np > 16 || rate < 1 || rate > 256) return ZKL_E_INVALID;
  std::lock_guard<std::mutex> lk(c->mu);
  return run_guarded(c, [&] {
    HIPCHECK(hipSetDevice(c->device));
    upload_hasher(c->stream);
    c->parts.ensure((size_t)std::max<uint32_t>(np, 1) * nr * sizeof(fe) + 16);
    launch_hash_rows((const fe*)d_m, nc, nr, np, rate, c->parts.f(), (fe*)d_out, c->stream);
    check_launch("stage entry point");
    HIPCHECK(hipStreamSynchronize(c->stream));
  });
}

int zkl_hip_set_column_structure(int on) {
  if (on < 0 || on > 1) return ZKL_E_INVALID;
  set_column_structure(on != 0);
  return 0;
}

int zkl_hip_column_structure(void) { return column_structure_enabled() ? 1 : 0; }

int zkl_hip_scan_columns(zkl_ctx* c, const void* d_m, uint32_t nc, uint32_t nr, uint32_t* period_out) {
  if (!c || !d_m || !period_out || nc == 0 || nc > 4096 || nr == 0 || (nr & (nr - 1))) return ZKL_E_INVALID;
  std::lock_guard<std::mutex> lk(c->mu);
  return run_guarded(c, [&] {
    HIPCHECK(hipSetDevice(c->device));
    c->scanbits.ensure((size_t)nc * sizeof(uint32_t));
    c->h_scan.ensure((size_t)nc * sizeof(uint32_t));
    launch_scan_columns((const fe*)d_m, nc, nr, (uint32_t*)c->scanbits.p, c->stream);
    check_launch("stage entry point");
    HIPCHECK(hipMemcpyAsync(c->h_scan.p, c->scanbits.p, (size_t)nc * sizeof(uint32_t), hipMemcpyDeviceToHost, c->stream));
    HIPCHECK(hipStreamSynchronize(c->stream));
    decode_column_scan(c->h_scan.at<uint32_t>(), nc, nr, period_out);
  });
}

int zkl_hip_plan_row_prefix(const uint32_t* period, uint32_t nc, uint64_t n_lde_rows, uint32_t blowup, uint32_t np,
                            uint32_t rate, uint32_t* lead_out, uint32_t* q_out, uint32_t* n_parts_out) {
  if (!period || !lead_out || !q_out || nc == 0 || np < 1 || np > 16 || rate < 1 || rate > 256 || blowup < 1 ||
      (blowup & (blowup - 1)))
    return ZKL_E_INVALID;
  return run_guarded(nullptr, [&] {
    const RowPrefixPlan pl = plan_row_prefix(period, nc, (size_t)n_lde_rows, blowup, np, rate);
    for (int p = 0; p < 16; p++) {
      lead_out[p] = pl.lead[p];
      q_out[p] = pl.lead[p] ? pl.q[p] : 0;
    }
    if (n_parts_out) *n_parts_out = pl.np;
  });
}

int zkl_hip_hash_rows_periodic(zkl_ctx* c, const void* d_m, uint32_t nc, uint32_t nr, uint32_t np, uint32_t rate,
                               const uint32_t* row_period, int split, void* d_out, uint32_t* resumed_out) {
  if (resumed_out) *resumed_out = 0;
  if (!c || !d_m || !d_out || !row_period || nc == 0 || np < 1 || np > 16 || rate < 1 || rate > 256 || split < 0 ||
      split > 1 || (split && (nr < 2048 || (nr & (nr - 1)))))
    return ZKL_E_INVALID;
  std::lock_guard<std::mutex> lk(c->mu);
  return run_guarded(c, [&] {
    HIPCHECK(hipSetDevice(c->device));
    upload_hasher(c->stream);
    c->parts.ensure((size_t)std::max<uint32_t>(np, 1) * nr * sizeof(fe) + 16);
    RowPrefixPlan plan;
    if (column_structure_enabled()) plan = plan_row_prefix(row_period, nc, nr, 1, np, rate, 1);
    if (plan.any()) c->pfxtab.ensure(row_prefix_table_bytes(plan));
    const bool used = launch_hash_rows_prefix((const fe*)d_m, nc, nr, np, rate, plan, (uint32_t*)c->pfxtab.p,
                                              c->parts.f(), (fe*)d_out, c->stream, split);
    if (used && resumed_out)
      for (uint32_t p = 0; p < plan.np; p++) *resumed_out += plan.lead[p] != 0;
    check_launch("stage entry point");
    HIPCHECK(hipStreamSynchronize(c->stream));
  });
}

int zkl_hip_lde_columns(zkl_ctx* c, const void* d_values, uint32_t nc, uint32_t n, uint32_t blowup,
                        const uint32_t* period, int want_split, void* d_coeffs, void* d_lde, int* split_out) {
  if (!c || !d_values || !d_coeffs || !d_lde || nc == 0 || nc > 4096 || n < 2 || (n & (n - 1)) || blowup < 2 ||
      (blowup & (blowup - 1)))
    return ZKL_E_INVALID;
  std::lock_guard<std::mutex> lk(c->mu);
  return run_guarded(c, [&] {
    HIPCHECK(hipSetDevice(c->device));
    const size_t N = (size_t)n * blowup;
    ensure_tables(c, n, N);
    hipStream_t s = c->stream;
    std::vector<uint32_t> per(nc, COL_GENERAL);
    if (column_structure_enabled()) {
      if (period) {
        per.assign(period, period + nc);
      } else {
        c->scanbits.ensure((size_t)nc * sizeof(uint32_t));
        c->h_scan.ensure((size_t)nc * sizeof(uint32_t));
        launch_scan_columns((const fe*)d_values, nc, n, (uint32_t*)c->scanbits.p, s);
        HIPCHECK(hipMemcpyAsync(c->h_scan.p, c->scanbits.p, (size_t)nc * sizeof(uint32_t), hipMemcpyDeviceToHost, s));
        HIPCHECK(hipStreamSynchronize(s));
        decode_column_scan(c->h_scan.at<uint32_t>(), nc, n, per.data());
      }
    }
    const MontTab mi = mont_tab(c->miroots.p, c->tab_N), mr = mont_tab(c->mroots.p, c->tab_N);
    int split = -1;
    for (uint32_t c0 = 0; c0 < nc;) {
      uint32_t c1 = c0;
      const bool zero = per[c0] == 0;
      while (c1 < nc && (per[c1] == 0) == zero) c1++;
      fe* cf = (fe*)d_coeffs + (size_t)c0 * n;
      fe* out = (fe*)d_lde + (size_t)c0 * N;
      if (zero) {
        HIPCHECK(hipMemsetAsync(cf, 0, (size_t)(c1 - c0) * n * sizeof(fe), s));
        HIPCHECK(hipMemsetAsync(out, 0, (size_t)(c1 - c0) * N * sizeof(fe), s));
      } else {
        launch_intt_scaled((const fe*)d_values + (size_t)c0 * n, cf, c1 - c0, n, mi, c->tab_N, c->opow_n.f(), s);
        const int sp = launch_lde_from_coeffs(cf, c1 - c0, n, N, mr, c->tab_N, out, s, want_split != 0);
        if (split >= 0 && sp != split) throw std::runtime_error("internal: LDE column runs in different layouts");
        split = sp;
      }
      c0 = c1;
    }
    check_launch("stage entry point");
    HIPCHECK(hipStreamSynchronize(s));
    if (split_out) *split_out = split < 0 ? 0 : split;
  });
}

int zkl_hip_set_ntt_mode(int mode) {
  if (mode < 0 || mode > 1) return ZKL_E_INVALID;
  if (g_proofs_in_flight.load() != 0) {
    set_err(nullptr, "the NTT mode cannot change while a proof is in flight");
    return ZKL_E_INVALID;
  }
  set_ntt_lazy(mode != 0);
  return 0;
}

int zkl_hip_set_row_digest_rule(int rule) {
  if (rule < 0 || rule > 1) return ZKL_E_INVALID;
  if (g_proofs_in_flight.load() != 0) {
    set_err(nullptr, "the row-digest rule cannot change while a proof is in flight");
    return ZKL_E_INVALID;
  }
  set_row_digest_rule(rule);
  return 0;
}

int zkl_hip_row_digest_rule(void) { return row_digest_rule(); }

int zkl_hip_set_hash_policy(int engine, uint32_t pm_min_items) {
  if (engine < 0 || engine > 1) return ZKL_E_INVALID;
  set_hash_policy(engine, pm_min_items);
  return 0;
}

int zkl_hip_poseidon_permute(zkl_ctx* c, void* d_states, uint32_t n_states, int engine) {
  if (!c || !d_states || engine < 0 || engine > 2) return ZKL_E_INVALID;
  std::lock_guard<std::mutex> lk(c->mu);
  return run_guarded(c, [&] {
    HIPCHECK(hipSetDevice(c->device));
    upload_hasher(c->stream);
    launch_permute((fe*)d_states, n_states, engine, c->stream);
    check_launch("stage entry point");
    HIPCHECK(hipStreamSynchronize(c->stream));
  });
}

int zkl_hip_merkle_tree(zkl_ctx* c, const void* d_leaves, uint32_t n, void* d_nodes) {
  if (!c || n < 2 || (n & (n - 1))) return ZKL_E_INVALID;
  std::lock_guard<std::mutex> lk(c->mu);
  return run_guarded(c, [&] {
    HIPCHECK(hipSetDevice(c->device));
    upload_hasher(c->stream);
    HIPCHECK(hipMemcpyAsync((fe*)d_nodes + n, d_leaves, (size_t)n * sizeof(fe), hipMemcpyDeviceToDevice, c->stream));
    HIPCHECK(hipMemsetAsync(d_nodes, 0, sizeof(fe), c->stream));
    launch_merkle((fe*)d_nodes, n, c->stream);
    check_launch("stage entry point");
    HIPCHECK(hipStreamSynchronize(c->stream));
  });
}

int zkl_hip_ntt(zkl_ctx* c, void* d_data, uint32_t nc, uint32_t n, int dif, int inverse) {
  if (!c || !d_data || n < 2 || (n & (n - 1))) return ZKL_E_INVALID;
  std::lock_guard<std::mutex> lk(c->mu);
  return run_guarded(c, [&] {
    HIPCHECK(hipSetDevice(c->device));
    ensure_tables(c, c->tab_n ? c->tab_n : n, std::max<size_t>(n, c->tab_N));
    const MontTab t = mont_tab(inverse ? c->miroots.p : c->mroots.p, c->tab_N);
    launch_ntt_stages((fe*)d_data, nc, n, dif != 0, 0, ilog2(n) - 1, t, c->tab_N, c->stream);
    check_launch("stage entry point");
    HIPCHECK(hipStreamSynchronize(c->stream));
  });
}

int zkl_hip_lde(zkl_ctx* c, const void* d_values, uint32_t nc, uint32_t n, uint32_t blowup, void* d_coeffs,
                void* d_lde) {
  if (!c || n < 2 || (n & (n - 1)) || blowup < 1 || (blowup & (blowup - 1))) return ZKL_E_INVALID;
  std::lock_guard<std::mutex> lk(c->mu);
  return run_guarded(c, [&] {
    HIPCHECK(hipSetDevice(c->device));
    size_t N = (size_t)n * blowup;
    ensure_tables(c, n, N);
    hipStream_t s = c->stream;
    fe* coef = (fe*)d_coeffs;
    HIPCHECK(hipMemcpyAsync(coef, d_values, (size_t)nc * n * sizeof(fe), hipMemcpyDeviceToDevice, s));
    launch_ntt_stages(coef, nc, n, true, 0, ilog2(n) - 1, mont_tab(c->miroots.p, c->tab_N), c->tab_N, s);
    launch_scale_bitrev(coef, nc, n, c->opow_n.f(), s);
    launch_lde_from_coeffs(coef, nc, n, N, mont_tab(c->mroots.p, c->tab_N), c->tab_N, (fe*)d_lde, s);
    check_launch("stage entry point");
    std::vector<fe> h((size_t)nc * n), r((size_t)nc * n);
    HIPCHECK(hipMemcpyAsync(h.data(), coef, h.size() * sizeof(fe), hipMemcpyDeviceToHost, s));
    HIPCHECK(hipStreamSynchronize(s));
    const fe inv3 = fe_inv(fe{3, 0});
    int logn = ilog2(n);
    std::vector<fe> i3k(n);
    i3k[0] = fe_one();
    for (uint32_t k = 1; k < n; k++) i3k[k] = fe_mul(i3k[k - 1], inv3);
    for (uint32_t col = 0; col < nc; col++)
      for (uint32_t j = 0; j < n; j++) {
        const uint32_t k = bitrev_u(j, logn);
        r[(size_t)col * n + k] = fe_mul(h[(size_t)col * n + j], i3k[k]);
      }
    HIPCHECK(hipMemcpyAsync(coef, r.data(), r.size() * sizeof(fe), hipMemcpyHostToDevice, s));
    HIPCHECK(hipStreamSynchronize(s));
  });
}

}
```

Before: 21.89.

## Exploit periodic and zero trace columns in LDE, OOD and DEEP

Adds a structured trace-LDE path. Columns with a small power-of-two period get their coefficients and blowup-times-period evaluations from a direct small DFT and are then tiled across the LDE. General columns go through the NTT through a column map, and zero columns are tracked in a ZeroBook so their buffers are not rewritten. OOD and DEEP receive lists of nonzero columns so they can skip zero columns. The goal is to avoid full NTT and memory traffic for degenerate columns, at the cost of extra bookkeeping, indirection in the NTT kernels, and correctness risk in the zero-tracking state across API calls.

After: 22.51 (median of 6 runs). 2.9% higher.

```diff
diff --git a/zk-lisp_amd/csrc/kernels.h b/zk-lisp_amd/csrc/kernels.h
--- a/zk-lisp_amd/csrc/kernels.h
+++ b/zk-lisp_amd/csrc/kernels.h
@@ -105,9 +105,14 @@
 void launch_ntt_stages(fe* d_data, size_t n_cols, size_t N, bool dif, int lo_log, int hi_log,
                        MontTab roots, size_t Ntab, hipStream_t s);
 void launch_intt_scaled(const fe* d_src, fe* d_data, size_t n_cols, size_t n, MontTab iroots, size_t Ntab,
-                        const fe* d_scale, hipStream_t s);
+                        const fe* d_scale, hipStream_t s, const uint32_t* d_cmap = nullptr);
 int launch_lde_from_coeffs(const fe* d_coef, size_t n_cols, size_t n, size_t N, MontTab roots, size_t Ntab, fe* d_out,
-                           hipStream_t s, bool want_split = false);
+                           hipStream_t s, bool want_split = false, const uint32_t* d_cmap = nullptr);
+void launch_periodic_lde(const fe* d_src, size_t n, size_t N, const uint32_t* d_cols, uint32_t n_cols, uint32_t P,
+                         const fe* d_roots, const fe* d_iroots, size_t Ntab, const fe* d_opow, fe* d_coef,
+                         fe* d_small, size_t small_stride, hipStream_t s);
+void launch_periodic_tile(const fe* d_small, size_t small_stride, const uint32_t* d_cols, const uint32_t* d_bp,
+                          uint32_t n_cols, size_t N, int split, fe* d_lde, hipStream_t s);
 __host__ __device__ inline size_t lde_pos(size_t r, size_t N, int split) {
   if (!split) return r;
   const int logS = __builtin_ctzll((unsigned long long)N) - 8;
@@ -167,6 +172,7 @@
   const fe* pw2;
   uint32_t ncols, chunks, use_off;
   uint32_t off[16];
+  const uint32_t* zero;
 };
 void launch_ood(const OodArgs& a, fe* d_partial, hipStream_t s);
 void launch_ood_frame(const fe* d_partial_trace, const fe* d_partial_comp, uint32_t W, uint32_t C, uint32_t chunks,
@@ -179,7 +185,7 @@
 void launch_deep_denoms(const fe* d_roots, size_t Ntab, size_t N, fe z, fe zg, fe* d_dinv, hipStream_t s);
 void launch_deep(const fe* d_lde, const fe* d_clde, const fe* d_roots, size_t Ntab, const DeepParams& p,
                  const DerivedConsts* dD, const fe* d_dinv , fe* d_out, hipStream_t s,
-                 int split = 0);
+                 int split = 0, const uint32_t* d_list = nullptr, uint32_t n_list = 0);
 void launch_fri_leaves(const fe* d_ev, size_t Nd, fe* d_leaves, hipStream_t s);
 void launch_fri_fold(const fe* d_ev, size_t Nd, const fe* d_alpha, const fe* d_iroots, size_t Ntab, fe* d_out,
                      hipStream_t s);
diff --git a/zk-lisp_amd/csrc/kernels.hip b/zk-lisp_amd/csrc/kernels.hip
--- a/zk-lisp_amd/csrc/kernels.hip
+++ b/zk-lisp_amd/csrc/kernels.hip
@@ -106,7 +106,8 @@
 template <bool DIF>
 __global__ __launch_bounds__(NTT_THREADS) void ntt_pass_kernel(fe* __restrict__ data, size_t ncols, int logN, int r,
                                                        int logS, MontTab roots, int logTab, const fe* __restrict__ src,
-                                                       int src_logb, const fe* __restrict__ scale = nullptr) {
+                                                       int src_logb, const fe* __restrict__ scale = nullptr,
+                                                       const uint32_t* __restrict__ cmap = nullptr) {
   __shared__ fe buf[NTT_ELEMS + NTT_ELEMS / 16];
   const int R = 1 << r;
   const int G = NTT_ELEMS >> r;
@@ -119,6 +120,7 @@
   const bool whole = gpc >= (size_t)G;
   if (whole) {
     col_fixed = blockIdx.x % (unsigned)ncols;
+    if (cmap) col_fixed = cmap[col_fixed];
     qbase = (size_t)(blockIdx.x / (unsigned)ncols) * G;
   }
   auto locate = [&](int g, size_t& col, size_t& q) -> bool {
@@ -130,7 +132,9 @@
     const size_t qg = (size_t)blockIdx.x * G + g;
     col = qg >> log_gpc;
     q = qg & (gpc - 1);
-    return col < ncols;
+    if (col >= ncols) return false;
+    if (cmap) col = cmap[col];
+    return true;
   };
   auto addr = [&](int g, int t, bool& ok) -> size_t {
     size_t col, q;
@@ -211,7 +215,7 @@
 template <int ELEMS, int THREADS>
 __global__ __launch_bounds__(THREADS) void ntt_dit_lazy_kernel(fe* __restrict__ data, size_t ncols, int logN, int r,
                                                                   int logS, MontTab roots, const fe* __restrict__ src,
-                                                                  int src_logb) {
+                                                                  int src_logb, const uint32_t* __restrict__ cmap) {
   constexpr int PITCHED = ELEMS + ELEMS / 16;
   __shared__ uint4 bufA[PITCHED];
   __shared__ uint32_t bufB[PITCHED];
@@ -226,6 +230,7 @@
   const bool whole = gpc >= (size_t)G;
   if (whole) {
     col_fixed = blockIdx.x % (unsigned)ncols;
+    if (cmap) col_fixed = cmap[col_fixed];
     qbase = (size_t)(blockIdx.x / (unsigned)ncols) * G;
   }
   auto locate = [&](int g, size_t& col, size_t& q) -> bool {
@@ -237,7 +242,9 @@
     const size_t qg = (size_t)blockIdx.x * G + g;
     col = qg >> log_gpc;
     q = qg & (gpc - 1);
-    return col < ncols;
+    if (col >= ncols) return false;
+    if (cmap) col = cmap[col];
+    return true;
   };
   auto addr = [&](int g, int t, bool& ok) -> size_t {
     size_t col, q;
@@ -343,7 +350,8 @@
 template <int ELEMS, int THREADS>
 __global__ __launch_bounds__(THREADS) void ntt_ct_lazy_kernel(fe* __restrict__ data, size_t ncols, int logN, int r,
                                                                  int logS, MontTab roots, const fe* __restrict__ src,
-                                                                 int src_logb, const fe* __restrict__ scale) {
+                                                                 int src_logb, const fe* __restrict__ scale,
+                                                                 const uint32_t* __restrict__ cmap) {
   constexpr int PITCHED = ELEMS + ELEMS / 16;
   __shared__ uint4 bufA[PITCHED];
   __shared__ uint32_t bufB[PITCHED];
@@ -358,6 +366,7 @@
   const bool whole = gpc >= (size_t)G;
   if (whole) {
     col_fixed = blockIdx.x % (unsigned)ncols;
+    if (cmap) col_fixed = cmap[col_fixed];
     qbase = (size_t)(blockIdx.x / (unsigned)ncols) * G;
   }
   auto locate = [&](int g, size_t& col, size_t& q) -> bool {
@@ -369,7 +378,9 @@
     const size_t qg = (size_t)blockIdx.x * G + g;
     col = qg >> log_gpc;
     q = qg & (gpc - 1);
-    return col < ncols;
+    if (col >= ncols) return false;
+    if (cmap) col = cmap[col];
+    return true;
   };
   auto addr = [&](int g, int t, bool& ok) -> size_t {
     size_t col, q;
@@ -479,7 +490,8 @@
 constexpr int NTT8_PITCH = 257;
 __global__ __launch_bounds__(NTT8_THREADS) __global__ __launch_bounds__(NTT8_THREADS) void ntt_dit8_kernel(fe* __restrict__ data, size_t ncols, int logN, int logS,
                                                                  MontTab roots, const fe* __restrict__ src, int src_logb,
-                                                                 int lfast, int split) {
+                                                                 int lfast, int split,
+                                                                 const uint32_t* __restrict__ cmap) {
   __shared__ uint4 bufA[NTT8_G * NTT8_PITCH];
   __shared__ uint32_t bufB[NTT8_G * NTT8_PITCH];
   const int tid = (int)threadIdx.x;
@@ -493,6 +505,7 @@
     col = blockIdx.x % (unsigned)ncols;
     q = (size_t)(blockIdx.x / (unsigned)ncols) * NTT8_G + g;
   }
+  if (cmap) col = cmap[col];
   const size_t S = (size_t)1 << logS;
   const size_t L = q & (S - 1), Hb = q >> logS;
   const size_t base = (col << logN) + ((Hb << logS) << 8) + L;
@@ -662,9 +675,10 @@
 }
 
 static void ntt_passes(fe* d, size_t ncols, size_t N, bool dif, int lo, int hi, MontTab roots, size_t Ntab,
-                       const fe* src, int src_logb, hipStream_t s, int split = 0, const fe* scale = nullptr) {
+                       const fe* src, int src_logb, hipStream_t s, int split = 0, const fe* scale = nullptr,
+                       const uint32_t* cmap = nullptr) {
   int logN = ilog2s(N), logTab = ilog2s(Ntab);
-  if (hi < lo) return;
+  if (hi < lo || ncols == 0) return;
   const std::vector<int> rs = ntt_split(hi - lo + 1);
   if (dif) {
     int cur = hi;
@@ -681,14 +695,14 @@
         const size_t Gw = wide ? 2 * G : G;
         const unsigned grid = (unsigned)((groups + Gw - 1) / Gw);
         if (wide && wm == 2)
-          ntt_ct_lazy_kernel<2 * NTT_ELEMS, 2 * NTT_THREADS><<<grid, 2 * NTT_THREADS, 0, s>>>(d, ncols, logN, r, logS, roots, sp, 0, sc);
+          ntt_ct_lazy_kernel<2 * NTT_ELEMS, 2 * NTT_THREADS><<<grid, 2 * NTT_THREADS, 0, s>>>(d, ncols, logN, r, logS, roots, sp, 0, sc, cmap);
         else if (wide)
-          ntt_ct_lazy_kernel<2 * NTT_ELEMS, NTT_THREADS><<<grid, NTT_THREADS, 0, s>>>(d, ncols, logN, r, logS, roots, sp, 0, sc);
+          ntt_ct_lazy_kernel<2 * NTT_ELEMS, NTT_THREADS><<<grid, NTT_THREADS, 0, s>>>(d, ncols, logN, r, logS, roots, sp, 0, sc, cmap);
         else
-          ntt_ct_lazy_kernel<NTT_ELEMS, NTT_THREADS><<<grid, NTT_THREADS, 0, s>>>(d, ncols, logN, r, logS, roots, sp, 0, sc);
+          ntt_ct_lazy_kernel<NTT_ELEMS, NTT_THREADS><<<grid, NTT_THREADS, 0, s>>>(d, ncols, logN, r, logS, roots, sp, 0, sc, cmap);
       } else {
         ntt_pass_kernel<true><<<(unsigned)((groups + G - 1) / G), NTT_THREADS, 0, s>>>(d, ncols, logN, r, logS, roots,
-                                                                                      logTab, sp, 0, sc);
+                                                                                      logTab, sp, 0, sc, cmap);
       }
       cur -= r;
     }
@@ -707,16 +721,16 @@
         const fe* sp = cur == lo ? src : nullptr;
         if (r == 8 && ntt8_enabled() && ((size_t)1 << cur) >= (size_t)NTT8_G && (N >> 8) >= (size_t)NTT8_G)
           ntt_dit8_kernel<<<(unsigned)(groups / NTT8_G), NTT8_THREADS, 0, s>>>(d, ncols, logN, cur, roots, sp, src_logb,
-                                                                              ntt8_lfast(cur), split_here);
+                                                                              ntt8_lfast(cur), split_here, cmap);
         else if (wide && wm == 2)
-          ntt_dit_lazy_kernel<2 * NTT_ELEMS, 2 * NTT_THREADS><<<grid, 2 * NTT_THREADS, 0, s>>>(d, ncols, logN, r, cur, roots, sp, src_logb);
+          ntt_dit_lazy_kernel<2 * NTT_ELEMS, 2 * NTT_THREADS><<<grid, 2 * NTT_THREADS, 0, s>>>(d, ncols, logN, r, cur, roots, sp, src_logb, cmap);
         else if (wide)
-          ntt_dit_lazy_kernel<2 * NTT_ELEMS, NTT_THREADS><<<grid, NTT_THREADS, 0, s>>>(d, ncols, logN, r, cur, roots, sp, src_logb);
+          ntt_dit_lazy_kernel<2 * NTT_ELEMS, NTT_THREADS><<<grid, NTT_THREADS, 0, s>>>(d, ncols, logN, r, cur, roots, sp, src_logb, cmap);
         else
-          ntt_dit_lazy_kernel<NTT_ELEMS, NTT_THREADS><<<grid, NTT_THREADS, 0, s>>>(d, ncols, logN, r, cur, roots, sp, src_logb);
+          ntt_dit_lazy_kernel<NTT_ELEMS, NTT_THREADS><<<grid, NTT_THREADS, 0, s>>>(d, ncols, logN, r, cur, roots, sp, src_logb, cmap);
       } else
         ntt_pass_kernel<false><<<(unsigned)((groups + G - 1) / G), NTT_THREADS, 0, s>>>(
-            d, ncols, logN, r, cur, roots, logTab, cur == lo ? src : nullptr, src_logb);
+            d, ncols, logN, r, cur, roots, logTab, cur == lo ? src : nullptr, src_logb, nullptr, cmap);
       cur += r;
     }
   }
@@ -728,22 +742,24 @@
 }
 
 void launch_intt_scaled(const fe* src, fe* d, size_t ncols, size_t n, MontTab iroots, size_t Ntab, const fe* scale,
-                        hipStream_t s) {
+                        hipStream_t s, const uint32_t* d_cmap) {
   const int logn = ilog2s(n);
   if (logn == 0) throw std::invalid_argument("launch_intt_scaled: n must be at least 2");
-  ntt_passes(d, ncols, n, true, 0, logn - 1, iroots, Ntab, src, 0, s, 0, scale);
+  ntt_passes(d, ncols, n, true, 0, logn - 1, iroots, Ntab, src, 0, s, 0, scale, d_cmap);
 }
 
 int launch_lde_from_coeffs(const fe* d_coef, size_t ncols, size_t n, size_t N, MontTab roots, size_t Ntab, fe* d_out,
-                           hipStream_t s, bool want_split) {
+                           hipStream_t s, bool want_split, const uint32_t* d_cmap) {
   const int logB = ilog2s(N / n);
   if (logB == 0) {
+    if (d_cmap) throw std::invalid_argument("launch_lde_from_coeffs: a column map needs a blowup of at least 2");
+    if (ncols == 0) return 0;
     ZKL_HIPCHECK(hipMemcpyAsync(d_out, d_coef, ncols * n * sizeof(fe), hipMemcpyDeviceToDevice, s));
     ntt_passes(d_out, ncols, N, false, 0, ilog2s(N) - 1, roots, Ntab, nullptr, 0, s);
     return 0;
   }
   const int split = want_split && dit_split_ok(N, logB, ilog2s(N) - 1) ? 1 : 0;
-  ntt_passes(d_out, ncols, N, false, logB, ilog2s(N) - 1, roots, Ntab, d_coef, logB, s, split);
+  ntt_passes(d_out, ncols, N, false, logB, ilog2s(N) - 1, roots, Ntab, d_coef, logB, s, split, nullptr, d_cmap);
   return split;
 }
 
@@ -832,6 +848,88 @@
     }
     period[c] = P;
   }
+}
+
+constexpr int PER_THREADS = 256, PER_EPARTS = 4, PER_ROWS = PER_THREADS / PER_EPARTS;
+__global__ __launch_bounds__(PER_THREADS) void periodic_lde_kernel(
+    const fe* __restrict__ src, size_t n, const uint32_t* __restrict__ cols, uint32_t logP, uint32_t logBP,
+    const fe* __restrict__ roots, const fe* __restrict__ iroots, int logTab, const fe* __restrict__ opow, fe invP,
+    uint32_t head, fe* __restrict__ coef, fe* __restrict__ small, size_t small_stride) {
+  __shared__ fe v[COL_P_MAX], c[COL_P_MAX], red[PER_THREADS];
+  const uint32_t P = 1u << logP, BP = 1u << logBP, t = threadIdx.x;
+  const size_t col = cols[blockIdx.y];
+  if (t < P) v[t] = src[col * n + t];
+  __syncthreads();
+  {
+    const uint32_t parts = min((uint32_t)PER_THREADS >> logP, P), len = P / parts;
+    const uint32_t j = t & (P - 1), part = t >> logP;
+    fe acc = fe_zero();
+    if (part < parts) {
+#pragma unroll 4
+      for (uint32_t i = part * len; i < (part + 1) * len; i++)
+        acc = fe_add(acc, fe_mul(v[i], iroots[(size_t)((i * j) & (P - 1)) << (logTab - logP)]));
+    }
+    red[t] = acc;
+    __syncthreads();
+    if (t < P) {
+      for (uint32_t k = 1; k < parts; k++) acc = fe_add(acc, red[k * P + t]);
+      c[t] = fe_mul(fe_mul(acc, invP), opow[(size_t)t * (n >> logP)]);
+    }
+    __syncthreads();
+  }
+  if (blockIdx.x == 0 && t < head) {
+    fe* cf = coef + col * n;
+    if (t < P) cf[bitrev(t, (int)logP)] = c[t];
+    else cf[t] = fe_zero();
+  }
+  const uint32_t eparts = min((uint32_t)PER_EPARTS, P), elen = P / eparts;
+  const uint32_t rl = t & (PER_ROWS - 1), epart = t / PER_ROWS;
+  const uint32_t r = blockIdx.x * PER_ROWS + rl;
+  fe acc = fe_zero();
+  if (r < BP && epart < eparts) {
+#pragma unroll 4
+    for (uint32_t j = epart * elen; j < (epart + 1) * elen; j++)
+      acc = fe_add(acc, fe_mul(c[j], roots[(size_t)((r * j) & (BP - 1)) << (logTab - logBP)]));
+  }
+  red[t] = acc;
+  __syncthreads();
+  if (t < PER_ROWS && r < BP) {
+    for (uint32_t k = 1; k < eparts; k++) acc = fe_add(acc, red[k * PER_ROWS + t]);
+    small[blockIdx.y * small_stride + r] = acc;
+  }
+}
+
+__global__ __launch_bounds__(256) void periodic_tile_kernel(const fe* __restrict__ small, size_t small_stride,
+                                                            const uint32_t* __restrict__ cols,
+                                                            const uint32_t* __restrict__ bp, size_t N, int split,
+                                                            fe* __restrict__ lde) {
+  const fe* sm = small + blockIdx.y * small_stride;
+  const size_t mask = (size_t)bp[blockIdx.y] - 1;
+  fe* out = lde + (size_t)cols[blockIdx.y] * N;
+  for (size_t pos = (size_t)blockIdx.x * blockDim.x + threadIdx.x; pos < N; pos += (size_t)gridDim.x * blockDim.x)
+    out[pos] = sm[lde_row(pos, N, split) & mask];
+}
+
+void launch_periodic_lde(const fe* d_src, size_t n, size_t N, const uint32_t* d_cols, uint32_t ncols, uint32_t P,
+                         const fe* d_roots, const fe* d_iroots, size_t Ntab, const fe* d_opow, fe* d_coef,
+                         fe* d_small, size_t small_stride, hipStream_t s) {
+  if (ncols == 0) return;
+  const size_t B = N / n;
+  if (P == 0 || (P & (P - 1)) || P > COL_P_MAX || P >= n || B * P > small_stride || B * P > Ntab || ncols > 65535)
+    throw std::invalid_argument("launch_periodic_lde: period must be a power of two <= 128 and below n");
+  const uint32_t BP = (uint32_t)(B * P), head = (uint32_t)std::min<size_t>(COL_P_MAX, n);
+  static_assert(COL_P_MAX <= PER_THREADS, "one thread per coefficient of the head");
+  periodic_lde_kernel<<<dim3((BP + PER_ROWS - 1) / PER_ROWS, ncols), PER_THREADS, 0, s>>>(
+      d_src, n, d_cols, (uint32_t)ilog2s(P), (uint32_t)ilog2s(BP), d_roots, d_iroots, ilog2s(Ntab), d_opow,
+      fe_inv(fe{P, 0}), head, d_coef, d_small, small_stride);
+}
+
+void launch_periodic_tile(const fe* d_small, size_t small_stride, const uint32_t* d_cols, const uint32_t* d_bp,
+                          uint32_t ncols, size_t N, int split, fe* d_lde, hipStream_t s) {
+  if (ncols == 0) return;
+  if (ncols > 65535) throw std::invalid_argument("launch_periodic_tile: at most 65535 columns");
+  const unsigned gx = (unsigned)std::max<size_t>(1, N / (256 * 16));
+  periodic_tile_kernel<<<dim3(gx, ncols), 256, 0, s>>>(d_small, small_stride, d_cols, d_bp, N, split, d_lde);
 }
 
 
@@ -1006,6 +1104,10 @@
 
 __global__ __launch_bounds__(256) void ood_kernel(OodArgs A, fe* partial) {
   const uint32_t c = blockIdx.x, k = blockIdx.z;
+  if (A.zero && A.zero[c]) {
+    if (threadIdx.x < 2) partial[((size_t)threadIdx.x * A.ncols + c) * A.chunks + k] = fe_zero();
+    return;
+  }
   const fe* col = A.coef + (A.use_off ? (size_t)A.off[c] : (size_t)c * A.col_stride);
   const size_t len = A.n / A.chunks, j0 = (size_t)k * len;
   uint32_t acc1[9] = {0, 0, 0, 0, 0, 0, 0, 0, 0}, acc2[9] = {0, 0, 0, 0, 0, 0, 0, 0, 0};
@@ -1052,7 +1154,8 @@
 __global__ __launch_bounds__(256) void deep_kernel(const fe* __restrict__ lde, const fe* __restrict__ clde,
                                                    const fe* __restrict__ roots, int shift, DeepParams p,
                                                    const DerivedConsts* __restrict__ K, const fe* __restrict__ dinv,
-                                                   fe* out, int split) {
+                                                   fe* out, int split, const uint32_t* __restrict__ list,
+                                                   uint32_t nlist) {
   const size_t T = (size_t)gridDim.x * blockDim.x;
   const size_t i0 = (size_t)blockIdx.x * blockDim.x + threadIdx.x;
   uint64_t col[DEEP_PTS][10];
@@ -1060,22 +1163,23 @@
   for (int k = 0; k < DEEP_PTS; k++)
 #pragma unroll
     for (int u = 0; u < 10; u++) col[k][u] = 0;
-  const uint32_t ncol = p.W + p.C;
+  const uint32_t ncol = list ? nlist : p.W + p.C;
   for (uint32_t c0 = 0; c0 < ncol; c0 += DEEP_COLS) {
     fe v[DEEP_COLS][DEEP_PTS];
 #pragma unroll
     for (int cc = 0; cc < DEEP_COLS; cc++) {
-      const uint32_t c = c0 + cc;
+      const uint32_t e = min(c0 + cc, ncol - 1);
+      const uint32_t c = list ? list[e] : e;
       const bool tr = c < p.W;
       const fe* src = tr ? lde + (size_t)c * p.N : clde + (size_t)(c - p.W) * p.N;
 #pragma unroll
       for (int k = 0; k < DEEP_PTS; k++)
-        v[cc][k] = c < ncol ? src[tr ? i0 + k * T : lde_row(i0 + k * T, p.N, split)] : fe_zero();
+        v[cc][k] = c0 + cc < ncol ? src[tr ? i0 + k * T : lde_row(i0 + k * T, p.N, split)] : fe_zero();
     }
 #pragma unroll
     for (int cc = 0; cc < DEEP_COLS; cc++) {
-      const uint32_t c = min(c0 + cc, ncol - 1);
-      const uint32_t* g = K->deep_m[c];
+      const uint32_t e = min(c0 + cc, ncol - 1);
+      const uint32_t* g = K->deep_m[list ? list[e] : e];
       const uint32_t gm[5] = {g[0], g[1], g[2], g[3], g[4]};
 #pragma unroll
       for (int k = 0; k < DEEP_PTS; k++) {
@@ -1161,10 +1265,12 @@
 }
 
 void launch_deep(const fe* d_lde, const fe* d_clde, const fe* d_roots, size_t Ntab, const DeepParams& p,
-                 const DerivedConsts* dK, const fe* d_dinv, fe* d_out, hipStream_t s, int split) {
+                 const DerivedConsts* dK, const fe* d_dinv, fe* d_out, hipStream_t s, int split,
+                 const uint32_t* d_list, uint32_t n_list) {
+  if (d_list && (n_list == 0 || n_list > p.W + p.C)) throw std::invalid_argument("launch_deep: bad column list");
   const size_t threads = std::min<size_t>(256, p.N / DEEP_PTS);
   deep_kernel<<<(unsigned)(p.N / (threads * DEEP_PTS)), (unsigned)threads, 0, s>>>(
-      d_lde, d_clde, d_roots, ilog2s(Ntab) - ilog2s(p.N), p, dK, d_dinv, d_out, split);
+      d_lde, d_clde, d_roots, ilog2s(Ntab) - ilog2s(p.N), p, dK, d_dinv, d_out, split, d_list, n_list);
 }
 
 __global__ void fri_fold_kernel(const fe* ev, size_t half, const fe* alpha_p, const fe* iroots, int shift, fe inv3,
diff --git a/zk-lisp_amd/csrc/lde_plan.h b/zk-lisp_amd/csrc/lde_plan.h
--- /dev/null
+++ b/zk-lisp_amd/csrc/lde_plan.h
@@ -0,0 +1,95 @@
+#pragma once
+#include <stddef.h>
+#include <stdint.h>
+
+#include <utility>
+#include <vector>
+
+namespace zkl {
+
+constexpr uint32_t LDE_COL_GENERAL = 0xFFFFFFFFu;
+constexpr uint32_t LDE_P_MAX = 128;
+
+struct ZeroBook {
+  enum : uint8_t {
+    UNKNOWN = 0,
+    ZERO = 1,
+    TAIL = 2,
+  };
+  std::vector<uint8_t> known;
+  const void* coef = nullptr;
+  const void* lde = nullptr;
+  size_t n = 0, N = 0, W = 0;
+
+  void forget() { coef = lde = nullptr; }
+  void wrote(const void* p, size_t bytes, size_t elem) {
+    if (!coef || !p) return;
+    const char* a = (const char*)p;
+    auto hits = [&](const void* buf, size_t len) {
+      const char* b = (const char*)buf;
+      return bytes == 0 ? (a < b + len) : (a < b + len && b < a + bytes);
+    };
+    if (hits(coef, W * n * elem) || hits(lde, W * N * elem)) forget();
+  }
+  void begin(const void* coef_, const void* lde_, size_t n_, size_t N_, size_t W_) {
+    const bool ok = coef_ && coef == coef_ && lde == lde_ && n == n_ && N == N_ && W == W_ && known.size() == W_;
+    if (!ok) known.assign(W_, UNKNOWN);
+    forget();
+  }
+  void all_unknown() { known.assign(known.size(), UNKNOWN); }
+  void commit(const void* coef_, const void* lde_, size_t n_, size_t N_, size_t W_) {
+    coef = coef_; lde = lde_; n = n_; N = N_; W = W_;
+  }
+};
+
+struct LdePlan {
+  std::vector<uint32_t> general;
+  std::vector<uint32_t> pcols, pper;
+  std::vector<uint32_t> nonzero;
+  std::vector<uint8_t> zero;
+  std::vector<std::pair<uint32_t, uint32_t>> clear_all, clear_tail;
+};
+
+inline bool lde_period_usable(uint32_t P, size_t n) {
+  return P != 0 && P != LDE_COL_GENERAL && P <= LDE_P_MAX && (P & (P - 1)) == 0 && (size_t)P < n;
+}
+
+inline LdePlan plan_structured_lde(const uint32_t* period, uint32_t W, size_t n, ZeroBook& book) {
+  LdePlan pl;
+  pl.zero.assign(W, 0);
+  if (book.known.size() != W) book.known.assign(W, ZeroBook::UNKNOWN);
+  std::vector<uint32_t> by_period[8];
+  auto extend = [](std::vector<std::pair<uint32_t, uint32_t>>& runs, uint32_t c) {
+    if (!runs.empty() && runs.back().second == c) runs.back().second = c + 1;
+    else runs.push_back({c, c + 1});
+  };
+  for (uint32_t c = 0; c < W; c++) {
+    const uint32_t P = period[c];
+    uint8_t& st = book.known[c];
+    if (P == 0) {
+      pl.zero[c] = 1;
+      if (st != ZeroBook::ZERO) extend(pl.clear_all, c);
+      st = ZeroBook::ZERO;
+      continue;
+    }
+    pl.nonzero.push_back(c);
+    if (lde_period_usable(P, n)) {
+      int lg = 0;
+      while ((1u << lg) < P) lg++;
+      by_period[lg].push_back(c);
+      if (st == ZeroBook::UNKNOWN && n > LDE_P_MAX) extend(pl.clear_tail, c);
+      st = ZeroBook::TAIL;
+    } else {
+      pl.general.push_back(c);
+      st = ZeroBook::UNKNOWN;
+    }
+  }
+  for (int lg = 0; lg < 8; lg++)
+    for (uint32_t c : by_period[lg]) {
+      pl.pcols.push_back(c);
+      pl.pper.push_back(1u << lg);
+    }
+  return pl;
+}
+
+}
diff --git a/zk-lisp_amd/csrc/prover.cpp b/zk-lisp_amd/csrc/prover.cpp
--- a/zk-lisp_amd/csrc/prover.cpp
+++ b/zk-lisp_amd/csrc/prover.cpp
@@ -20,6 +20,7 @@
 #include "air_host.h"
 #include "host_hash.h"
 #include "kernels.h"
+#include "lde_plan.h"
 #include "host_proof.h"
 #include "proof_view.h"
 
@@ -35,6 +36,8 @@
 namespace {
 
 #define HIPCHECK(x) ZKL_HIPCHECK(x)
+
+static_assert(LDE_COL_GENERAL == COL_GENERAL && LDE_P_MAX == COL_P_MAX, "lde_plan.h restates kernels.h");
 
 struct InvalidArg : std::runtime_error { using std::runtime_error::runtime_error; };
 
@@ -111,10 +114,9 @@
   DBuf cexinv;
   size_t cexinv_key_n = 0, cexinv_key_ce = 0, cexinv_key_tab = 0;
   const void* cexinv_key_roots = nullptr;
-  DBuf scanbits, pfxtab;
-  HBuf h_scan;
-  std::vector<uint8_t> zero_known;
-  struct { const void* coef = nullptr; const void* lde = nullptr; size_t n = 0, N = 0, W = 0; } zero_key;
+  DBuf scanbits, pfxtab, colmeta, psmall;
+  HBuf h_scan, h_meta;
+  ZeroBook zero_known, zero_stage;
   DBuf kconst;
   DBuf dconst;
   DBuf fri_coin;
@@ -407,6 +409,78 @@
   ~InFlight() { g_proofs_in_flight.fetch_sub(1); }
 };
 
+struct ColMeta {
+  const uint32_t* zero = nullptr;
+  const uint32_t* general = nullptr;
+  const uint32_t* pcols = nullptr;
+  const uint32_t* pbp = nullptr;
+  const uint32_t* deep = nullptr;
+  uint32_t n_nonzero = 0;
+};
+
+ColMeta upload_col_meta(zkl_ctx* C, const LdePlan& pl, uint32_t W, uint32_t B, hipStream_t s) {
+  const size_t words = 5 * (size_t)W + 16;
+  C->colmeta.ensure(words * sizeof(uint32_t));
+  C->h_meta.ensure(words * sizeof(uint32_t));
+  uint32_t* h = C->h_meta.at<uint32_t>();
+  memset(h, 0, words * sizeof(uint32_t));
+  for (uint32_t c = 0; c < W; c++) h[c] = pl.zero[c];
+  std::copy(pl.general.begin(), pl.general.end(), h + W);
+  std::copy(pl.pcols.begin(), pl.pcols.end(), h + 2 * (size_t)W);
+  for (size_t k = 0; k < pl.pper.size(); k++) h[3 * (size_t)W + k] = pl.pper[k] * B;
+  std::copy(pl.nonzero.begin(), pl.nonzero.end(), h + 4 * (size_t)W);
+  for (uint32_t j = 0; j < 16; j++) h[4 * (size_t)W + pl.nonzero.size() + j] = W + j;
+  HIPCHECK(hipMemcpyAsync(C->colmeta.p, h, words * sizeof(uint32_t), hipMemcpyHostToDevice, s));
+  const uint32_t* d = (const uint32_t*)C->colmeta.p;
+  ColMeta m;
+  m.zero = d; m.general = d + W; m.pcols = d + 2 * (size_t)W; m.pbp = d + 3 * (size_t)W; m.deep = d + 4 * (size_t)W;
+  m.n_nonzero = (uint32_t)pl.nonzero.size();
+  return m;
+}
+
+int trace_lde_columns(zkl_ctx* C, ZeroBook& book, const fe* d_src, uint32_t W, size_t n, size_t N,
+                      const uint32_t* period, fe* coef, fe* lde, bool want_split, ColMeta* meta_out, hipStream_t s) {
+  const MontTab mi = mont_tab(C->miroots.p, C->tab_N), mr = mont_tab(C->mroots.p, C->tab_N);
+  const size_t Ntab = C->tab_N;
+  book.begin(coef, lde, n, N, W);
+  int split;
+  if (!period) {
+    book.all_unknown();
+    launch_intt_scaled(d_src, coef, W, n, mi, Ntab, C->opow_n.f(), s);
+    split = launch_lde_from_coeffs(coef, W, n, N, mr, Ntab, lde, s, want_split);
+  } else {
+    const uint32_t B = (uint32_t)(N / n);
+    const LdePlan pl = plan_structured_lde(period, W, n, book);
+    const ColMeta m = upload_col_meta(C, pl, W, B, s);
+    if (meta_out) *meta_out = m;
+    const size_t head = std::min<size_t>(LDE_P_MAX, n);
+    for (auto& r : pl.clear_all) {
+      HIPCHECK(hipMemsetAsync(coef + (size_t)r.first * n, 0, (size_t)(r.second - r.first) * n * sizeof(fe), s));
+      HIPCHECK(hipMemsetAsync(lde + (size_t)r.first * N, 0, (size_t)(r.second - r.first) * N * sizeof(fe), s));
+    }
+    for (auto& r : pl.clear_tail)
+      for (uint32_t c = r.first; c < r.second; c++)
+        HIPCHECK(hipMemsetAsync(coef + (size_t)c * n + head, 0, (n - head) * sizeof(fe), s));
+    const uint32_t ng = (uint32_t)pl.general.size(), npc = (uint32_t)pl.pcols.size();
+    launch_intt_scaled(d_src, coef, ng, n, mi, Ntab, C->opow_n.f(), s, m.general);
+    split = launch_lde_from_coeffs(coef, ng, n, N, mr, Ntab, lde, s, want_split, m.general);
+    if (npc) {
+      const size_t stride = (size_t)B * LDE_P_MAX;
+      C->psmall.ensure((size_t)npc * stride * sizeof(fe));
+      for (uint32_t a = 0; a < npc;) {
+        uint32_t b = a;
+        while (b < npc && pl.pper[b] == pl.pper[a]) b++;
+        launch_periodic_lde(d_src, n, N, m.pcols + a, b - a, pl.pper[a], C->roots.f(), C->iroots.f(), Ntab,
+                            C->opow.f(), coef, C->psmall.f() + (size_t)a * stride, stride, s);
+        a = b;
+      }
+      launch_periodic_tile(C->psmall.f(), stride, m.pcols, m.pbp, npc, N, split, lde, s);
+    }
+  }
+  book.commit(coef, lde, n, N, W);
+  return split;
+}
+
 void prove_impl(zkl_ctx* C, const void* d_trace_in, bool trace_on_host, uint32_t W, uint32_t n32,
                 const zkl_air_public_inputs& pi, const zkl_proof_options& o) {
   const InFlight in_flight;
@@ -441,10 +515,8 @@
     split = sp;
   };
   const bool colstruct = column_structure_enabled();
-  const bool zkey_ok = C->zero_key.coef == C->coef.p && C->zero_key.lde == C->lde.p && C->zero_key.n == n &&
-                       C->zero_key.N == N && C->zero_key.W == W && C->zero_known.size() == W;
-  if (!zkey_ok) C->zero_known.assign(W, 0);
-  C->zero_key.coef = nullptr;
+  ZeroBook& book = C->zero_known;
+  ColMeta meta;
   std::vector<uint32_t> period;
   uint32_t* hbits = nullptr;
   if (colstruct) {
@@ -460,54 +532,36 @@
   };
   if (trace_on_host) {
     KScope k(C, KF_NTT);
-    std::fill(C->zero_known.begin(), C->zero_known.end(), 0);
+    book.begin(C->coef.p, C->lde.p, n, N, W);
+    book.all_unknown();
     if (colstruct) HIPCHECK(hipMemsetAsync(C->scanbits.p, 0, (size_t)W * sizeof(uint32_t), s));
     upload_trace_chunked(C, d_trace_in, W, n, s, [&](uint32_t c0, uint32_t nc) {
       if (colstruct) launch_scan_columns(C->coef.f() + (size_t)c0 * n, nc, n, (uint32_t*)C->scanbits.p + c0, s, false);
       lde_cols(c0, nc, nullptr);
     });
-  } else if (!colstruct) {
-    C->up_ms = 0;
-    KScope k(C, KF_NTT);
-    std::fill(C->zero_known.begin(), C->zero_known.end(), 0);
-    lde_cols(0, W, (const fe*)d_trace_in);
+    book.commit(C->coef.p, C->lde.p, n, N, W);
   } else {
     C->up_ms = 0;
-    {
+    if (colstruct) {
       KScope k(C, KF_MISC);
       launch_scan_columns((const fe*)d_trace_in, W, n, (uint32_t*)C->scanbits.p, s);
       check_launch("column scan");
       read_scan();
     }
     KScope k(C, KF_NTT);
-    for (uint32_t c0 = 0; c0 < W;) {
-      uint32_t c1 = c0;
-      const bool zero = period[c0] == 0;
-      while (c1 < W && (period[c1] == 0) == zero) c1++;
-      if (!zero) {
-        lde_cols(c0, c1 - c0, (const fe*)d_trace_in);
-        std::fill(C->zero_known.begin() + c0, C->zero_known.begin() + c1, 0);
-      } else {
-        for (uint32_t a = c0; a < c1;) {
-          if (C->zero_known[a]) { a++; continue; }
-          uint32_t b = a;
-          while (b < c1 && !C->zero_known[b]) b++;
-          HIPCHECK(hipMemsetAsync(C->coef.f() + (size_t)a * n, 0, (size_t)(b - a) * n * sizeof(fe), s));
-          HIPCHECK(hipMemsetAsync(C->lde.f() + (size_t)a * N, 0, (size_t)(b - a) * N * sizeof(fe), s));
-          std::fill(C->zero_known.begin() + a, C->zero_known.begin() + b, 1);
-          a = b;
-        }
-      }
-      c0 = c1;
-    }
+    split = trace_lde_columns(C, book, (const fe*)d_trace_in, W, n, N, colstruct ? period.data() : nullptr, C->coef.f(),
+                              C->lde.f(), g_lde_split, &meta, s);
   }
   check_launch("trace LDE");
   if (split < 0) split = 0;
-  C->zero_key.coef = C->coef.p; C->zero_key.lde = C->lde.p; C->zero_key.n = n; C->zero_key.N = N; C->zero_key.W = W;
   T.mark(1);
   C->parts.ensure((size_t)o.num_partitions * N * sizeof(fe) + N * sizeof(fe));
   C->tree.ensure(2 * N * sizeof(fe));
-  if (colstruct && trace_on_host) read_scan();
+  if (colstruct && trace_on_host) {
+    read_scan();
+    ZeroBook none;
+    meta = upload_col_meta(C, plan_structured_lde(period.data(), W, n, none), W, B, s);
+  }
   {
     RowPrefixPlan plan;
     if (colstruct) plan = plan_row_prefix(period.data(), W, N, B, o.num_partitions, o.hash_rate);
@@ -712,6 +766,7 @@
     OodArgs a{};
     a.coef = C->coef.f(); a.col_stride = n; a.elem_stride = 1; a.n = n;
     a.pw1 = pw + 2 * n; a.pw2 = pw + 3 * n; a.ncols = W; a.chunks = chunks; a.use_off = 0;
+    a.zero = meta.zero;
     launch_ood(a, dood, s);
     OodArgs b{};
     b.coef = C->ce.f(); b.col_stride = 0; b.elem_stride = ce / n; b.n = n;
@@ -755,7 +810,8 @@
   C->deep.ensure(N * sizeof(fe));
   {
     KScope k(C, KF_DEEP);
-    launch_deep(C->lde.f(), C->clde.f(), roots, Ntab, dp, dD, C->xinv.f(), C->deep.f(), s, split);
+    launch_deep(C->lde.f(), C->clde.f(), roots, Ntab, dp, dD, C->xinv.f(), C->deep.f(), s, split, meta.deep,
+                meta.n_nonzero + (uint32_t)Cc);
   }
   check_launch("DEEP composition");
   T.mark(6);
@@ -1313,6 +1369,7 @@
 int zkl_hip_device_free(zkl_ctx* c, void* d) {
   if (!c) return ZKL_E_INVALID;
   return run_guarded(c, [&] {
+    c->zero_stage.wrote(d, 0, sizeof(fe));
     HIPCHECK(hipSetDevice(c->device));
     HIPCHECK(hipFree(d));
   });
@@ -1322,6 +1379,7 @@
   if (!c || kind < 1 || kind > 3) return ZKL_E_INVALID;
   std::lock_guard<std::mutex> lk(c->mu);
   return run_guarded(c, [&] {
+    if (kind != 2 && bytes) c->zero_stage.wrote(dst, bytes, sizeof(fe));
     HIPCHECK(hipSetDevice(c->device));
     hipMemcpyKind k = kind == 1 ? hipMemcpyHostToDevice : kind == 2 ? hipMemcpyDeviceToHost : hipMemcpyDeviceToDevice;
     HIPCHECK(hipMemcpyAsync(dst, src, bytes, k, c->stream));
@@ -1347,6 +1405,7 @@
   if (!c || !d_m || !d_out || nc == 0 || np < 1 || np > 16 || rate < 1 || rate > 256) return ZKL_E_INVALID;
   std::lock_guard<std::mutex> lk(c->mu);
   return run_guarded(c, [&] {
+    c->zero_stage.forget();
     HIPCHECK(hipSetDevice(c->device));
     upload_hasher(c->stream);
     c->parts.ensure((size_t)std::max<uint32_t>(np, 1) * nr * sizeof(fe) + 16);
@@ -1402,6 +1461,7 @@
     return ZKL_E_INVALID;
   std::lock_guard<std::mutex> lk(c->mu);
   return run_guarded(c, [&] {
+    c->zero_stage.forget();
     HIPCHECK(hipSetDevice(c->device));
     upload_hasher(c->stream);
     c->parts.ensure((size_t)std::max<uint32_t>(np, 1) * nr * sizeof(fe) + 16);
@@ -1441,28 +1501,12 @@
         decode_column_scan(c->h_scan.at<uint32_t>(), nc, n, per.data());
       }
     }
-    const MontTab mi = mont_tab(c->miroots.p, c->tab_N), mr = mont_tab(c->mroots.p, c->tab_N);
-    int split = -1;
-    for (uint32_t c0 = 0; c0 < nc;) {
-      uint32_t c1 = c0;
-      const bool zero = per[c0] == 0;
-      while (c1 < nc && (per[c1] == 0) == zero) c1++;
-      fe* cf = (fe*)d_coeffs + (size_t)c0 * n;
-      fe* out = (fe*)d_lde + (size_t)c0 * N;
-      if (zero) {
-        HIPCHECK(hipMemsetAsync(cf, 0, (size_t)(c1 - c0) * n * sizeof(fe), s));
-        HIPCHECK(hipMemsetAsync(out, 0, (size_t)(c1 - c0) * N * sizeof(fe), s));
-      } else {
-        launch_intt_scaled((const fe*)d_values + (size_t)c0 * n, cf, c1 - c0, n, mi, c->tab_N, c->opow_n.f(), s);
-        const int sp = launch_lde_from_coeffs(cf, c1 - c0, n, N, mr, c->tab_N, out, s, want_split != 0);
-        if (split >= 0 && sp != split) throw std::runtime_error("internal: LDE column runs in different layouts");
-        split = sp;
-      }
-      c0 = c1;
-    }
+    const int split = trace_lde_columns(c, c->zero_stage, (const fe*)d_values, nc, n, N,
+                                        column_structure_enabled() ? per.data() : nullptr, (fe*)d_coeffs, (fe*)d_lde,
+                                        want_split != 0, nullptr, s);
     check_launch("stage entry point");
     HIPCHECK(hipStreamSynchronize(s));
-    if (split_out) *split_out = split < 0 ? 0 : split;
+    if (split_out) *split_out = split;
   });
 }
 
@@ -1498,6 +1542,7 @@
   if (!c || !d_states || engine < 0 || engine > 2) return ZKL_E_INVALID;
   std::lock_guard<std::mutex> lk(c->mu);
   return run_guarded(c, [&] {
+    c->zero_stage.forget();
     HIPCHECK(hipSetDevice(c->device));
     upload_hasher(c->stream);
     launch_permute((fe*)d_states, n_states, engine, c->stream);
@@ -1510,6 +1555,7 @@
   if (!c || n < 2 || (n & (n - 1))) return ZKL_E_INVALID;
   std::lock_guard<std::mutex> lk(c->mu);
   return run_guarded(c, [&] {
+    c->zero_stage.forget();
     HIPCHECK(hipSetDevice(c->device));
     upload_hasher(c->stream);
     HIPCHECK(hipMemcpyAsync((fe*)d_nodes + n, d_leaves, (size_t)n * sizeof(fe), hipMemcpyDeviceToDevice, c->stream));
@@ -1524,6 +1570,7 @@
   if (!c || !d_data || n < 2 || (n & (n - 1))) return ZKL_E_INVALID;
   std::lock_guard<std::mutex> lk(c->mu);
   return run_guarded(c, [&] {
+    c->zero_stage.forget();
     HIPCHECK(hipSetDevice(c->device));
     ensure_tables(c, c->tab_n ? c->tab_n : n, std::max<size_t>(n, c->tab_N));
     const MontTab t = mont_tab(inverse ? c->miroots.p : c->mroots.p, c->tab_N);
@@ -1538,6 +1585,7 @@
   if (!c || n < 2 || (n & (n - 1)) || blowup < 1 || (blowup & (blowup - 1))) return ZKL_E_INVALID;
   std::lock_guard<std::mutex> lk(c->mu);
   return run_guarded(c, [&] {
+    c->zero_stage.forget();
     HIPCHECK(hipSetDevice(c->device));
     size_t N = (size_t)n * blowup;
     ensure_tables(c, n, N);
```
